# arkworks-rs/ripp

Hardware: AMD Instinct MI355X
Metric: SIPP prover pairing-products/sec at n=2^20 BLS12-381 (higher is better)
Workload: dtype u32

## Files before the change

### include/ripp_hip.h

```cpp
#ifndef RIPP_HIP_H
#define RIPP_HIP_H
#include <stddef.h>
#include <stdint.h>
#ifdef __cplusplus
extern "C" {
#endif

typedef struct { uint64_t l[6]; } ripp_fp;
typedef struct { uint64_t l[4]; } ripp_fr;
typedef struct { ripp_fp c0, c1; } ripp_fp2;
typedef struct { ripp_fp2 c[6]; } ripp_gt;
typedef struct { ripp_fp x, y; } ripp_g1a;
typedef struct { ripp_fp x, y, z; } ripp_g1j;
typedef struct { ripp_fp2 x, y; } ripp_g2a;
typedef struct { ripp_fp2 x, y, z; } ripp_g2j;

enum { RIPP_OK = 0, RIPP_ERR_LENGTH = 1, RIPP_ERR_POW2 = 2, RIPP_ERR_DEVICE = 3, RIPP_ERR_ARG = 4 };

typedef struct {
    double total_ms, upload_ms, scale_ms, miller_lines_ms, miller_products_ms, fold_ms, normalize_ms, host_ms, hash_ms;
    double kernel_miller_lines_ms_sum, kernel_line_products_ms_sum;
    uint64_t kernel_miller_lines_launches, kernel_line_products_launches;
    uint64_t pairs_lines, pairs_products;
    double exchange_ms;
    double look_ms;
    uint64_t look_items, look_pairs;
    double statement_hash_ms, statement_hash_wait_ms;
    uint64_t chains_lines;
    uint64_t mem_tier, device_bytes;
} ripp_stats;
#define RIPP_ABI_VERSION 7
int32_t ripp_abi_version(void);
size_t  ripp_stats_size(void);

int32_t ripp_init(int32_t device_ordinal);
void    ripp_shutdown(void);
int32_t ripp_device_count(void);
int32_t ripp_release_scratch(void);
size_t  ripp_device_bytes(void);
const char* ripp_last_error(void);

typedef struct {
    uint32_t struct_size;
    uint32_t no_vm, no_precompute, no_fold_tables, no_msm_glv, lp_one_lane, no_endo, no_fq, no_xscale, scale_no_fq, agg_sequential, look_static, quiet_waits, no_share, no_fuse, fuse_tables;
    int32_t  look_eighths;
    int32_t  ranks_per_device;
    int32_t  msm_c; uint32_t msm_ch, msm_gmin;
    uint32_t no_prebuild;
    uint64_t vm_lines_max, vm_fold_max, vm_tree_max, gls_split_max, msm_vm_merge_max, fold_tab_min, fq_min, lp_fq_min, vm_joint_max, vm_scale_max,
             tail_pipe_max, ml_fq_min, fq_min_g1,
             msm_lds_sort_min,
             msm_chunk_min;
    uint64_t mem_cap_bytes;
    uint32_t hot_workers;
    uint32_t no_job_cache;
    uint32_t no_lp_karatsuba;
    uint32_t comm_timeout_ms;
    uint32_t plan_derate_pct;
    uint32_t n_devices;
} ripp_config;
int32_t ripp_config_default(ripp_config* cfg);
int32_t ripp_configure(const ripp_config* cfg);
int32_t ripp_config_get(ripp_config* cfg);

int32_t ripp_pairing_product_j(const ripp_g1j* left, size_t n_left, const ripp_g2j* right, size_t n_right, ripp_gt* out);
int32_t ripp_pairing_product_a(const ripp_g1a* a, const ripp_g2a* b, size_t n, ripp_gt* out);
int32_t ripp_pairing_product_coeffs_a(const ripp_g1a* a, const ripp_g2a* b, const ripp_fr* r, size_t n, ripp_gt* out);
int32_t ripp_msm_g1_j(const ripp_g1j* bases, size_t n_left, const ripp_fr* scalars, size_t n_right, ripp_g1j* out);
int32_t ripp_msm_g2_j(const ripp_g2j* bases, size_t n_left, const ripp_fr* scalars, size_t n_right, ripp_g2j* out);
int32_t ripp_msm_g1_a(const ripp_g1a* bases, const ripp_fr* scalars, size_t n, ripp_g1j* out);
int32_t ripp_msm_g2_a(const ripp_g2a* bases, const ripp_fr* scalars, size_t n, ripp_g2j* out);
int32_t ripp_device_slots_used(void);
int32_t ripp_scalar_inner_product(const ripp_fr* left, size_t nl, const ripp_fr* right, size_t nr, ripp_fr* out);
int32_t ripp_pairing_miller_j(const ripp_g1j* left, size_t nl, const ripp_g2j* right, size_t nr, ripp_gt* miller_value);
int32_t ripp_sum_g1_j(const ripp_g1j* pts, size_t n, ripp_g1j* out);
int32_t ripp_sum_g2_j(const ripp_g2j* pts, size_t n, ripp_g2j* out);

int32_t ripp_fold_g1_a(const ripp_g1a* hi, const ripp_g1a* lo, size_t half, const ripp_fr* s, ripp_g1a* out);
int32_t ripp_fold_g2_a(const ripp_g2a* hi, const ripp_g2a* lo, size_t half, const ripp_fr* s, ripp_g2a* out);
int32_t ripp_fold_g1_j(const ripp_g1j* hi, const ripp_g1j* lo, size_t half, const ripp_fr* s, ripp_g1j* out);
int32_t ripp_fold_g2_j(const ripp_g2j* hi, const ripp_g2j* lo, size_t half, const ripp_fr* s, ripp_g2j* out);
int32_t ripp_fold_fr(const ripp_fr* hi, const ripp_fr* lo, size_t half, const ripp_fr* s, ripp_fr* out);
int32_t ripp_scale_g1_a(const ripp_g1a* a, const ripp_fr* r, size_t n, ripp_g1a* out);
int32_t ripp_normalize_g1(const ripp_g1j* in, size_t n, ripp_g1a* out);
int32_t ripp_normalize_g2(const ripp_g2j* in, size_t n, ripp_g2a* out);

typedef struct ripp_vec ripp_vec;
enum { RIPP_VEC_G1 = 1, RIPP_VEC_G2 = 2, RIPP_VEC_FR = 3 };
int32_t ripp_vec_upload_g1a(const ripp_g1a* p, size_t n, ripp_vec** out);
int32_t ripp_vec_upload_g2a(const ripp_g2a* p, size_t n, ripp_vec** out);
int32_t ripp_vec_upload_g1j(const ripp_g1j* p, size_t n, ripp_vec** out);
int32_t ripp_vec_upload_g2j(const ripp_g2j* p, size_t n, ripp_vec** out);
int32_t ripp_vec_upload_fr(const ripp_fr* p, size_t n, ripp_vec** out);
size_t  ripp_vec_len(const ripp_vec* v);
int32_t ripp_vec_kind(const ripp_vec* v);
int32_t ripp_vec_slice(const ripp_vec* v, size_t off, size_t len, ripp_vec** view);
int32_t ripp_vec_halves(const ripp_vec* v, ripp_vec** lo, ripp_vec** hi);
int32_t ripp_vec_download(const ripp_vec* v, void* out);
void    ripp_vec_free(ripp_vec* v);
int32_t ripp_vec_pairing_product(const ripp_vec* left_g1, const ripp_vec* right_g2, ripp_gt* out);
int32_t ripp_vec_msm(const ripp_vec* bases, const ripp_vec* scalars, void* out );
int32_t ripp_vec_scalar_inner_product(const ripp_vec* left, const ripp_vec* right, ripp_fr* out);
int32_t ripp_vec_fold(const ripp_vec* hi, const ripp_vec* lo, const ripp_fr* s, ripp_vec** out);

int32_t ripp_sipp_prove(const ripp_g1a* a, const ripp_g2a* b, const ripp_fr* r, size_t n, const ripp_gt* value,
                        ripp_gt* proof, ripp_fr* challenges, ripp_stats* stats);
int32_t ripp_sipp_verify(const ripp_g1a* a, const ripp_g2a* b, const ripp_fr* r, size_t n, const ripp_gt* claimed,
                         const ripp_gt* proof, size_t proof_rounds, int32_t* accept);

typedef struct ripp_sipp_job ripp_sipp_job;
int32_t ripp_sipp_job_create(const ripp_g1a* a, const ripp_g2a* b, const ripp_fr* r, size_t n_local,
                             int32_t rank, int32_t world, ripp_sipp_job** job);
void    ripp_sipp_job_destroy(ripp_sipp_job* job);
int32_t ripp_sipp_job_prove(ripp_sipp_job* job, const ripp_gt* value, ripp_gt* proof, ripp_fr* challenges, ripp_stats* stats);
int32_t ripp_sipp_job_begin(ripp_sipp_job* job);
size_t  ripp_sipp_job_rounds_left(const ripp_sipp_job* job);
int32_t ripp_sipp_job_round_partials(ripp_sipp_job* job, ripp_gt* partials );
int32_t ripp_sipp_job_round_finish(ripp_sipp_job* job, const ripp_gt* combined , const uint8_t seed_digest[32],
                                   ripp_gt* z_l, ripp_gt* z_r, ripp_fr* x);
int32_t ripp_sipp_job_stats(const ripp_sipp_job* job, ripp_stats* stats);
size_t  ripp_sipp_job_local_len(const ripp_sipp_job* job);
int32_t ripp_sipp_job_export(ripp_sipp_job* job, ripp_g1a* a_out, ripp_g2a* b_out);
// ... 189 lines not shown
```

### ripp_amd/csrc/engine.hip

```cpp
#include <hip/hip_runtime.h>
#include <atomic>
#include <csignal>
#include <sched.h>
#include <condition_variable>
#include <deque>
#include <functional>
#include <memory>
#include <future>
#include <chrono>
#include <cmath>
#include <cstdio>
#include <cstring>
#include <cstdlib>
#include <mutex>
#include <string>
#include <thread>
#include <vector>
#ifndef RIPP_BUILD_STAMP
#define RIPP_BUILD_STAMP __DATE__ " " __TIME__
#endif
#include "../../include/ripp_hip.h"
#include "kernels.hpp"
#include "line_products.hpp"
#include "msm.hpp"
// ... 129 lines not shown
struct Engine;
thread_local Engine* t_engine = nullptr;
size_t evict_idle_scratch(Engine* e);
struct DevBuf {
    void* p = nullptr; size_t cap = 0; uint64_t epoch = 0;
    int32_t reserve(size_t bytes) {
        epoch = g_call_epoch.load(std::memory_order_relaxed);
        if (bytes <= cap) return RIPP_OK;
        release();
        hipError_t err = hipMalloc(&p, bytes);
        if (err == hipErrorOutOfMemory && t_engine) {
            (void)hipGetLastError();
            const size_t freed = evict_idle_scratch(t_engine);
            if (trace_on()) fprintf(stderr, "[ripp] out of device memory for %zu bytes: %zu bytes of idle scratch freed, retrying\n", bytes, freed);
            err = freed ? hipMalloc(&p, bytes) : err;
        }
        if (err != hipSuccess) { p = nullptr; (void)hipGetLastError(); set_err(std::string("hipMalloc(&p, bytes): ") + hipGetErrorString(err) + " (" + std::to_string(bytes) + " bytes wanted, " + std::to_string(g_dev_bytes.load()) + " held by the library)"); return RIPP_ERR_DEVICE; }
        cap = bytes; g_dev_bytes.fetch_add(bytes, std::memory_order_relaxed); return RIPP_OK;
    }
    void release() { if (p) { (void)hipFree(p); g_dev_bytes.fetch_sub(cap, std::memory_order_relaxed); } p = nullptr; cap = 0; }
    template <class T> T* as() { return reinterpret_cast<T*>(p); }
};

struct PinBuf {
    void* p = nullptr; size_t cap = 0; hipEvent_t ev = nullptr; bool pending = false;
    bool blocking = false;
    bool ev_blocking = false;
    int32_t wait() { if (pending) { HIPCHK(hipEventSynchronize(ev)); pending = false; } return RIPP_OK; }
    int32_t reserve(size_t bytes) {
        int32_t rc = wait(); if (rc) return rc;
        if (ev && ev_blocking != blocking) { (void)hipEventDestroy(ev); ev = nullptr; }
        if (!ev) { HIPCHK(hipEventCreateWithFlags(&ev, hipEventDisableTiming | (blocking ? hipEventBlockingSync : 0))); ev_blocking = blocking; }
        if (bytes <= cap) return RIPP_OK;
        if (p) { (void)hipHostFree(p); p = nullptr; cap = 0; }
        HIPCHK(hipHostMalloc(&p, bytes, hipHostMallocDefault)); cap = bytes; return RIPP_OK;
    }
    int32_t send(void* dst, size_t bytes, hipStream_t st) {
        HIPCHK(hipMemcpyAsync(dst, p, bytes, hipMemcpyHostToDevice, st)); HIPCHK(hipEventRecord(ev, st)); pending = true; return RIPP_OK;
    }
    void release() { if (pending && ev) (void)hipEventSynchronize(ev); pending = false; if (p) (void)hipHostFree(p); p = nullptr; cap = 0; if (ev) (void)hipEventDestroy(ev); ev = nullptr; }
    template <class T> T* as() { return reinterpret_cast<T*>(p); }
};

struct MsmScratch {
    DevBuf digits, hist, offs, cursor, slotoffs, spw, sorted, slots, buckets, seg, seg2, win, out;
    DevBuf ext;
    DevBuf flags;
    DevBuf nflag;
    void* host_out = nullptr;
    void release() { for (DevBuf* b : {&digits, &hist, &offs, &cursor, &slotoffs, &spw, &sorted, &slots, &buckets, &seg, &seg2, &win, &out, &ext, &flags, &nflag}) b->release(); if (host_out) (void)hipHostFree(host_out); host_out = nullptr; }
};

struct Timer {
    hipEvent_t a{}, b{};
    int32_t init() { HIPCHK(hipEventCreate(&a)); HIPCHK(hipEventCreate(&b)); return RIPP_OK; }
    void destroy() { if (a) (void)hipEventDestroy(a); if (b) (void)hipEventDestroy(b); a = b = nullptr; }
};

struct Engine {
    int device = -1;
    hipStream_t stream = nullptr, stream2 = nullptr;
    hipEvent_t ev_fork = nullptr, ev_join = nullptr, ev_join3 = nullptr;
    hipEvent_t ev_t0 = nullptr, ev_t1 = nullptr;
    int n_simd = 1024;
    DevBuf lines, partA, partB, jacG1, jacG2, tmpA, tmpB, tmpR, affG1, affG2;
    DevBuf qtab;
    MsmScratch msm_scratch[2];
    MsmScratch msm_batch; DevBuf pc_coef, pc_out, pc_yev, pc_h, pc_cin, pc_q, pc_aff;
    DevBuf tpc_m, tpc_m2, tpc_b, tpc_b2, tpc_k, tpc_k2, tpc_jac, tpc_part, tpc_out;
    uint32_t msm_batch_chunks = 0;
    void pc_release() { msm_batch.release(); for (DevBuf* b : {&pc_coef, &pc_out, &pc_yev, &pc_h, &pc_cin, &pc_q, &pc_aff, &tpc_m, &tpc_m2, &tpc_b, &tpc_b2, &tpc_k, &tpc_k2, &tpc_jac, &tpc_part, &tpc_out}) b->release(); }
    DevBuf kzg_q[2];
    PinBuf stage[4];
    DevBuf kzg_bases[2];
    hipStream_t stream3 = nullptr;
    hipStream_t stream4 = nullptr;
    hipEvent_t ev_join4 = nullptr;
    DevBuf fold_tab1, fold_mult, fold_tab, fold_jac1, fold_jac2;
    DevBuf fix_flags, scale_flags;
    const void* tab_owner = nullptr;
    struct JobBufCache { DevBuf d[15]; PinBuf p[4]; bool full = false; void release() { for (DevBuf& b : d) b.release(); for (PinBuf& b : p) b.release(); full = false; } } job_cache;
    size_t msm_chunk_min = (size_t)1 << 20;
    size_t msm_lds_sort_min = 0;
    const void* g2tab_hi = nullptr; size_t g2tab_half = 0;
    size_t vm_scale_max = (size_t)1 << 14;
    size_t vm_joint_max = (size_t)1 << 13;
    size_t lp_fq_min = 0;
    size_t ml_fq_min = 0;
    size_t fq_min_g1 = (size_t)1 << 12;
    size_t fq_min = (size_t)1 << 15;
    size_t fold_tab_min = 32768;
    size_t msm_vm_merge_max = 16384;
    hipStream_t stream5 = nullptr;
    hipEvent_t ev_join5 = nullptr;
    Fp12* pinned_rows = nullptr;
    size_t pinned_rows_cap = 0;
    std::vector<std::pair<hipEvent_t, hipEvent_t>> ev_lines, ev_prod;
    std::vector<std::pair<hipEvent_t, hipEvent_t>> ev_fold_async;
    size_t tail_pipe_max = (size_t)1 << 11;
    size_t vm_tree_max = (size_t)1 << 16;
    size_t vm_fold_max = (size_t)1 << 11;
    DevBuf vm_flag;
    size_t vm_lines_max = (size_t)1 << 15;
    size_t gls_split_max = (size_t)1 << 14;
    size_t max_pairs_per_batch = (size_t)1 << 19;
    size_t mem_cap = 0;
    int mem_tier = 0;
    bool mem_fits(size_t need, size_t held) const {
        if (need <= held) return true;
        const size_t extra = need - held;
        if (mem_cap) return g_dev_bytes.load(std::memory_order_relaxed) + extra <= mem_cap;
        size_t fr = 0, tot = 0;
        if (hipMemGetInfo(&fr, &tot) != hipSuccess) return true;
        return extra + std::max<size_t>((size_t)2 << 30, tot / 50) <= fr;
    }
    size_t pairs_cap(size_t want) {
        want = std::max<size_t>(1, std::min(want, max_pairs_per_batch));
        const size_t per = (size_t)N_LINES * LINE_CHUNKS * sizeof(uint4);
        auto bytes = [per](size_t pairs) { return ((pairs + 63) & ~(size_t)63) * per + (size_t)MAX_PRODUCTS * 64 * per; };
        if (bytes(want) <= lines.cap) return want;
        size_t w = want;
        while (w > 4096 && !mem_fits(bytes(w), lines.cap)) w = (w + 1) / 2;
        if (w < want) mem_tier |= 8;
        return w;
    }
    ripp_stats stats{};
    std::vector<Engine*> peers; bool virtual_devices = false;
    Engine* aux = nullptr;
    Engine* aux_engine() {
        if (!aux) { Engine* a = new Engine(); if (a->init(device) != RIPP_OK) { delete a; return nullptr; } aux = a; }
        aux->refresh_switches(); aux->stats = ripp_stats{};
        return aux;
    }
    struct Switches { bool no_vm = false, no_precompute = false, no_fold_tables = false, no_msm_glv = false, lp_one_lane = false, no_endo = false, no_fq = false, no_xscale = false, no_share = false, no_fuse = false, no_prebuild = false, fuse_tables = false, no_job_cache = false, no_lp_kara = false, no_msm_batch = false; } sw;
    struct Sizes { size_t vm_lines_max, vm_fold_max, vm_tree_max, gls_split_max, msm_vm_merge_max, fold_tab_min, fq_min, lp_fq_min, vm_joint_max, vm_scale_max, tail_pipe_max, ml_fq_min, fq_min_g1, msm_lds_sort_min, msm_chunk_min; } defaults{};
    MsmTune msm_tune;
    static constexpr size_t TPC_CROSS_MIN = ~(size_t)0;
    size_t tpc_cross_min = TPC_CROSS_MIN;
    double cal_ms_per_pair = 0, cal_hash_bytes_per_ms = 0;
    int look_eighths = -1; double ranks_per_device = 1.0; bool look_static = false, quiet_waits_cfg = false, agg_sequential = false, scale_no_fq = false;
    int hot_workers_cfg = 0;
    uint32_t comm_timeout_ms = 0, plan_derate_pct = 0, n_devices_cfg = 0;
    void refresh_switches() {
        msm_tune = MsmTune();
        vm_lines_max = defaults.vm_lines_max; vm_fold_max = defaults.vm_fold_max; vm_tree_max = defaults.vm_tree_max; gls_split_max = defaults.gls_split_max;
        msm_vm_merge_max = defaults.msm_vm_merge_max; fold_tab_min = defaults.fold_tab_min; fq_min = defaults.fq_min; lp_fq_min = defaults.lp_fq_min; vm_joint_max = defaults.vm_joint_max;
        vm_scale_max = defaults.vm_scale_max; tail_pipe_max = defaults.tail_pipe_max; ml_fq_min = defaults.ml_fq_min; fq_min_g1 = defaults.fq_min_g1; msm_lds_sort_min = defaults.msm_lds_sort_min; msm_chunk_min = defaults.msm_chunk_min;
        sw = Switches(); look_eighths = -1; ranks_per_device = 1.0; look_static = quiet_waits_cfg = agg_sequential = scale_no_fq = false; mem_cap = 0; hot_workers_cfg = 0; comm_timeout_ms = plan_derate_pct = n_devices_cfg = 0;
        if (g_cfg_set) {
            const ripp_config& c = g_cfg;
            sw.no_vm = c.no_vm; sw.no_precompute = c.no_precompute; sw.no_fold_tables = c.no_fold_tables; sw.no_msm_glv = c.no_msm_glv; sw.lp_one_lane = c.lp_one_lane;
            sw.no_endo = c.no_endo; sw.no_fq = c.no_fq; sw.no_xscale = c.no_xscale; sw.no_share = c.no_share; sw.no_fuse = c.no_fuse; sw.fuse_tables = c.fuse_tables; scale_no_fq = c.scale_no_fq; agg_sequential = c.agg_sequential; look_static = c.look_static; quiet_waits_cfg = c.quiet_waits;
            look_eighths = c.look_eighths; ranks_per_device = c.ranks_per_device > 1 ? (double)c.ranks_per_device : 1.0;
            msm_tune.c = c.msm_c; msm_tune.ch = c.msm_ch; msm_tune.gmin = c.msm_gmin; sw.no_prebuild = c.no_prebuild;
            mem_cap = (size_t)c.mem_cap_bytes; hot_workers_cfg = (int)c.hot_workers; sw.no_job_cache = c.no_job_cache != 0;
            sw.no_lp_kara = c.no_lp_karatsuba != 0; comm_timeout_ms = c.comm_timeout_ms; plan_derate_pct = c.plan_derate_pct; n_devices_cfg = c.n_devices;
            vm_lines_max = c.vm_lines_max; vm_fold_max = c.vm_fold_max; vm_tree_max = c.vm_tree_max; gls_split_max = c.gls_split_max; msm_vm_merge_max = c.msm_vm_merge_max; fold_tab_min = c.fold_tab_min;
            fq_min = c.fq_min; lp_fq_min = c.lp_fq_min; vm_joint_max = c.vm_joint_max; vm_scale_max = c.vm_scale_max; tail_pipe_max = c.tail_pipe_max; ml_fq_min = c.ml_fq_min; fq_min_g1 = c.fq_min_g1; msm_lds_sort_min = c.msm_lds_sort_min; msm_chunk_min = c.msm_chunk_min;
        }
        { const char* s; if ((s = std::getenv("RIPP_MSM_C"))) msm_tune.c = std::atoi(s); if ((s = std::getenv("RIPP_MSM_CH"))) msm_tune.ch = (uint32_t)std::strtoul(s, nullptr, 10); if ((s = std::getenv("RIPP_MSM_GMIN"))) msm_tune.gmin = (uint32_t)std::strtoul(s, nullptr, 10); }
        auto env_sz = [](const char* k, size_t& v) { if (const char* s = std::getenv(k)) v = (size_t)std::strtoull(s, nullptr, 10); };
        env_sz("RIPP_VM_LINES_MAX", vm_lines_max); env_sz("RIPP_VM_FOLD_MAX", vm_fold_max); env_sz("RIPP_VM_TREE_MAX", vm_tree_max);
        env_sz("RIPP_GLS_SPLIT_MAX", gls_split_max); env_sz("RIPP_MSM_VM_MERGE_MAX", msm_vm_merge_max); env_sz("RIPP_FOLD_TAB_MIN", fold_tab_min);
        env_sz("RIPP_FQ_MIN", fq_min); env_sz("RIPP_LP_FQ_MIN", lp_fq_min); env_sz("RIPP_VM_JOINT_MAX", vm_joint_max);
        env_sz("RIPP_MSM_LDS_SORT_MIN", msm_lds_sort_min); env_sz("RIPP_MSM_CHUNK_MIN", msm_chunk_min);
        env_sz("RIPP_VM_SCALE_MAX", vm_scale_max); env_sz("RIPP_TAIL_PIPE_MAX", tail_pipe_max); env_sz("RIPP_ML_FQ_MIN", ml_fq_min); env_sz("RIPP_FQ_MIN_G1", fq_min_g1);
        auto env_on = [](const char* k, bool& v) { if (std::getenv(k)) v = true; };
        env_on("RIPP_NO_VM", sw.no_vm); env_on("RIPP_NO_PRECOMPUTE", sw.no_precompute); env_on("RIPP_NO_FOLD_TABLES", sw.no_fold_tables); env_on("RIPP_NO_MSM_GLV", sw.no_msm_glv);
        env_on("RIPP_LP_ONE_LANE", sw.lp_one_lane);
        env_on("RIPP_NO_ENDO", sw.no_endo);
        env_on("RIPP_NO_XSCALE", sw.no_xscale);
        env_on("RIPP_NO_LP_KARA", sw.no_lp_kara);
        env_on("RIPP_NO_FQ", sw.no_fq);
        env_on("RIPP_FUSE_TABLES", sw.fuse_tables);
        env_on("RIPP_NO_JOB_CACHE", sw.no_job_cache);
        env_sz("RIPP_MEM_CAP_BYTES", mem_cap);
        if (const char* s = std::getenv("RIPP_HOT_WORKERS")) hot_workers_cfg = std::atoi(s) ? 1 : 2;
        { auto env_u32 = [](const char* k, uint32_t& v) { if (const char* s = std::getenv(k)) v = (uint32_t)std::strtoul(s, nullptr, 10); };
          env_u32("RIPP_COMM_TIMEOUT_MS", comm_timeout_ms); env_u32("RIPP_PLAN_DERATE_PCT", plan_derate_pct); env_u32("RIPP_N_DEVICES", n_devices_cfg);
          virtual_devices = false; if (const char* s = std::getenv("RIPP_VIRTUAL_DEVICES")) { n_devices_cfg = (uint32_t)std::strtoul(s, nullptr, 10); virtual_devices = true; } }
        tpc_cross_min = TPC_CROSS_MIN; env_sz("RIPP_TPC_CROSS_MIN", tpc_cross_min);
        env_on("RIPP_NO_MSM_BATCH", sw.no_msm_batch);
        env_on("RIPP_NO_PREBUILD", sw.no_prebuild);
        env_on("RIPP_NO_FUSE", sw.no_fuse);
        env_on("RIPP_NO_SHARE", sw.no_share);
        env_on("RIPP_SCALE_NO_FQ", scale_no_fq); env_on("RIPP_AGG_SEQUENTIAL", agg_sequential); env_on("RIPP_LOOK_STATIC", look_static); env_on("RIPP_QUIET_WAITS", quiet_waits_cfg);
        if (const char* s = std::getenv("RIPP_LOOK_ITEMS")) look_eighths = 8 * std::max(0, std::atoi(s));
        if (const char* s = std::getenv("RIPP_LOOK_EIGHTHS")) look_eighths = std::max(0, std::atoi(s));
        if (const char* s = std::getenv("RIPP_RANKS_PER_DEVICE")) ranks_per_device = std::max(1.0, std::atof(s));
#if !defined(RIPP_AB_KERNELS) || defined(RIPP_BLS12_377)
        sw.lp_one_lane = false;
#endif
    }

    int32_t init(int dev) {
        int n = 0;
        if (hipGetDeviceCount(&n) != hipSuccess || n <= 0) { set_err("no HIP device available (libripp_hip has no CPU fallback)"); return RIPP_ERR_DEVICE; }
        if (dev < 0 || dev >= n) { set_err("device ordinal out of range"); return RIPP_ERR_ARG; }
        HIPCHK(hipSetDevice(dev));
        HIPCHK(hipStreamCreateWithFlags(&stream, hipStreamNonBlocking));
        HIPCHK(hipStreamCreateWithFlags(&stream2, hipStreamNonBlocking));
        HIPCHK(hipStreamCreateWithFlags(&stream3, hipStreamNonBlocking));
        HIPCHK(hipStreamCreateWithFlags(&stream4, hipStreamNonBlocking)); HIPCHK(hipEventCreateWithFlags(&ev_join4, hipEventDisableTiming));
        HIPCHK(hipStreamCreateWithFlags(&stream5, hipStreamNonBlocking)); HIPCHK(hipEventCreateWithFlags(&ev_join5, hipEventDisableTiming));
        HIPCHK(hipEventCreateWithFlags(&ev_fork, hipEventDisableTiming)); HIPCHK(hipEventCreateWithFlags(&ev_join, hipEventDisableTiming)); HIPCHK(hipEventCreateWithFlags(&ev_join3, hipEventDisableTiming));
        HIPCHK(hipEventCreate(&ev_t0)); HIPCHK(hipEventCreate(&ev_t1));
        { hipDeviceProp_t pr; if (hipGetDeviceProperties(&pr, dev) == hipSuccess) n_simd = pr.multiProcessorCount * 4; }
        defaults = Sizes{vm_lines_max, vm_fold_max, vm_tree_max, gls_split_max, msm_vm_merge_max, fold_tab_min, fq_min, lp_fq_min, vm_joint_max, vm_scale_max, tail_pipe_max, ml_fq_min, fq_min_g1, msm_lds_sort_min, msm_chunk_min};
        refresh_switches();
        device = dev;
        return RIPP_OK;
    }
    void destroy() {
        if (aux) { aux->destroy(); delete aux; aux = nullptr; }
        for (Engine* p : peers) { (void)hipSetDevice(p->device); p->destroy(); delete p; }
        if (!peers.empty()) { peers.clear(); (void)hipSetDevice(device); }
        for (DevBuf* b : {&lines, &partA, &partB, &jacG1, &jacG2, &tmpA, &tmpB, &tmpR, &affG1, &affG2, &qtab, &vm_flag, &scale_tab, &fold_tab1, &fold_mult, &fold_tab, &fold_jac1, &fold_jac2, &fix_flags, &scale_flags}) b->release();
        msm_scratch[0].release(); msm_scratch[1].release(); kzg_q[0].release(); kzg_q[1].release(); kzg_bases[0].release(); kzg_bases[1].release(); job_cache.release(); pc_release();
        if (stream3) (void)hipStreamDestroy(stream3);
        if (stream4) (void)hipStreamDestroy(stream4); if (ev_join4) (void)hipEventDestroy(ev_join4);
        if (stream5) (void)hipStreamDestroy(stream5); if (ev_join5) (void)hipEventDestroy(ev_join5);
        if (pinned_rows) (void)hipHostFree(pinned_rows);
        for (PinBuf& b : stage) b.release();
        for (auto& e : ev_lines) { (void)hipEventDestroy(e.first); (void)hipEventDestroy(e.second); }
        for (auto& e : ev_prod) { (void)hipEventDestroy(e.first); (void)hipEventDestroy(e.second); }
        for (auto& e : ev_fold_async) { (void)hipEventDestroy(e.first); (void)hipEventDestroy(e.second); }
        if (stream) (void)hipStreamDestroy(stream);
        if (stream2) (void)hipStreamDestroy(stream2);
        if (ev_fork) (void)hipEventDestroy(ev_fork); if (ev_join) (void)hipEventDestroy(ev_join); if (ev_join3) (void)hipEventDestroy(ev_join3);
        if (ev_t0) (void)hipEventDestroy(ev_t0); if (ev_t1) (void)hipEventDestroy(ev_t1);
        if (ev_quiet) (void)hipEventDestroy(ev_quiet);
    }
    int32_t ensure_pinned_rows(size_t rows) {
        if (rows <= pinned_rows_cap) return RIPP_OK;
        if (pinned_rows) (void)hipHostFree(pinned_rows);
        HIPCHK(hipHostMalloc((void**)&pinned_rows, rows * sizeof(Fp12), hipHostMallocDefault));
        pinned_rows_cap = rows; return RIPP_OK;
    }
    bool quiet_waits = false; hipEvent_t ev_quiet = nullptr;
    int32_t sync() {
        if (quiet_waits) {
            if (!ev_quiet) HIPCHK(hipEventCreateWithFlags(&ev_quiet, hipEventDisableTiming | hipEventBlockingSync));
            HIPCHK(hipEventRecord(ev_quiet, stream)); HIPCHK(hipEventSynchronize(ev_quiet)); return RIPP_OK;
        }
        HIPCHK(hipStreamSynchronize(stream)); return RIPP_OK;
    }

    int32_t mark(std::vector<std::pair<hipEvent_t, hipEvent_t>>& v, bool begin) {
        if (begin) { hipEvent_t a, b; HIPCHK(hipEventCreate(&a)); HIPCHK(hipEventCreate(&b)); v.emplace_back(a, b); HIPCHK(hipEventRecord(a, stream)); }
        else HIPCHK(hipEventRecord(v.back().second, stream));
        return RIPP_OK;
    }
    void collect_kernel_stats() {
        auto drain = [](std::vector<std::pair<hipEvent_t, hipEvent_t>>& v, double& sum, uint64_t& cnt) {
            for (auto& e : v) { float ms = 0; if (hipEventElapsedTime(&ms, e.first, e.second) == hipSuccess) { sum += ms; ++cnt; } (void)hipEventDestroy(e.first); (void)hipEventDestroy(e.second); }
            v.clear(); };
        drain(ev_lines, stats.kernel_miller_lines_ms_sum, stats.kernel_miller_lines_launches);
        drain(ev_prod, stats.kernel_line_products_ms_sum, stats.kernel_line_products_launches);
        uint64_t nf = 0; drain(ev_fold_async, stats.fold_ms, nf);
    }

    DevBuf scale_tab;
    int32_t scale_g1_dev(const G1A* base, uint32_t base_stride, const Fr* k, size_t n, G1J* out, hipStream_t st = nullptr) {
        if (n == 0) return RIPP_OK;
        if (!st) st = stream;
        if (sw.no_endo) {
            hipLaunchKernelGGL(HIP_KERNEL_NAME(k_scale_pts<Fp>), dim3(nblk(n, 256)), dim3(256), 0, st, base, base_stride, k, (uint32_t)n, out);
            HIPCHK(hipGetLastError());
            return RIPP_OK;
        }
        if (n <= vm_scale_max && !sw.no_vm) {
            hipLaunchKernelGGL(k_vm_scale_g1, dim3(nblk(n, 4 * VM_EPW)), dim3(256), 4 * VM_EPW * VM_SCALE_SLOTS * sizeof(VmSlot), st, base, base_stride, k, (uint32_t)n, out);
            HIPCHK(hipGetLastError());
            return RIPP_OK;
        }
        int32_t rc = scale_tab.reserve((size_t)SCALE_TAB * G1J_CHUNKS * n * sizeof(uint4)); if (rc) return rc;
        if (!sw.no_fq && !scale_no_fq)
        {
            if ((rc = scale_flags.reserve(n + 16))) return rc;
            hipLaunchKernelGGL(k_scale_g1_glv_q, dim3(nblk(n, 256)), dim3(256), 0, st, base, base_stride, k, (uint32_t)n, scale_tab.as<uint4>(), out, scale_flags.as<uint8_t>());
            hipLaunchKernelGGL(k_scale_g1_fix, dim3(FIX_GRID), dim3(64), 0, st, base, base_stride, k, (uint32_t)n, out, scale_flags.as<uint8_t>());
        }
        else
        hipLaunchKernelGGL(k_scale_g1_glv, dim3(nblk(n, 256)), dim3(256), 0, st, base, base_stride, k, (uint32_t)n, scale_tab.as<uint4>(), out);
        HIPCHK(hipGetLastError());
        return RIPP_OK;
    }

    template <class F> int32_t normalize_dev(const Jac<F>* in, size_t n, Affine<F>* out, hipStream_t st = nullptr) {
        if (n == 0) return RIPP_OK;
        if (!st) st = stream;
        uint32_t K = (uint32_t)std::min<size_t>(16, std::max<size_t>(1, n / 65536));
        uint32_t T = (uint32_t)((n + K - 1) / K);
        hipLaunchKernelGGL(HIP_KERNEL_NAME(k_normalize<F>), dim3(nblk(T, 256)), dim3(256), 0, st, in, (uint32_t)n, out, T);
        HIPCHK(hipGetLastError());
        return RIPP_OK;
    }


    template <class F> int32_t msm_launch(MsmScratch& ms, hipStream_t st, const Affine<F>* bases, const Fr* scalars, size_t n, const std::function<int32_t()>* bases_arrive = nullptr) {
        if (!ms.host_out) HIPCHK(hipHostMalloc(&ms.host_out, sizeof(G2J), hipHostMallocDefault));
        if (n == 0) { *reinterpret_cast<Jac<F>*>(ms.host_out) = jac_inf<F>(); return bases_arrive ? (*bases_arrive)() : RIPP_OK; }
        const bool no_glv = sw.no_msm_glv;
        const size_t nreal = n;
        const MsmPlan p = msm_plan(nreal, no_glv ? 1 : std::is_same<F, Fp>::value ? 2 : 4, msm_tune);
        n = p.n;
        const size_t nwb = (size_t)p.nwin * p.nb;
        const uint32_t max_slots = (uint32_t)(n / p.ch + std::min<size_t>(p.nb, n) + 1);
        uint32_t nseg = (p.nb + p.seg - 1) / p.seg;
        int32_t rc;
        if ((rc = ms.digits.reserve((size_t)p.nwin * n * sizeof(uint16_t))) || (rc = ms.hist.reserve(nwb * 4)) || (rc = ms.offs.reserve(nwb * 4)) ||
            (rc = ms.cursor.reserve(nwb * 4)) || (rc = ms.slotoffs.reserve(nwb * 4)) || (rc = ms.spw.reserve(p.nwin * 4)) ||
            (rc = ms.sorted.reserve((size_t)p.nwin * n * 4)) || (rc = ms.slots.reserve((size_t)p.nwin * max_slots * sizeof(Jac<F>))) ||
// ... 195 lines not shown
        const uint4* lrows = lines.as<uint4>() + (size_t)p_lo * N_LINES * LINE_CHUNKS * stride;
#if !defined(RIPP_BLS12_377)
        const bool lp_kara = !sw.no_fq && !sw.no_lp_kara && !sw.lp_one_lane && m * (size_t)np2 >= lp_fq_min;
#else
        const bool lp_kara = false;
#endif
        const uint32_t per_wave = sw.lp_one_lane ? 64 : lp_kara ? LK_GROUPS_PER_WAVE : LP_GROUPS_PER_WAVE;
        uint32_t T = (uint32_t)std::max<size_t>(per_wave, ((size_t)n_simd * RIPP_OCC_PROD / nrows) * per_wave);
        if (T > m) T = (uint32_t)m;
        if ((rc = partA.reserve(nrows * FP12_CHUNKS * (size_t)T * sizeof(uint4))) != RIPP_OK) return rc;
        if ((rc = partB.reserve(nrows * FP12_CHUNKS * (size_t)((T + 1) / 2) * sizeof(uint4))) != RIPP_OK) return rc;
        if ((rc = mark(ev_prod, true)) != RIPP_OK) return rc;
#if defined(RIPP_AB_KERNELS) && !defined(RIPP_BLS12_377)
        if (sw.lp_one_lane)
            hipLaunchKernelGGL(k_line_products1, dim3(nblk(T, 64), (unsigned)nrows), dim3(64), 0, stream, lrows, stride, (uint32_t)m, partA.as<uint4>(), T);
        else
#endif
#if !defined(RIPP_BLS12_377)
        if (lp_kara)
            hipLaunchKernelGGL(k_line_products_k, dim3(nblk(T, LK_GROUPS_PER_WAVE), (unsigned)nrows), dim3(64), 0, stream, lrows, stride, (uint32_t)m, partA.as<uint4>(), T);
        else
#endif
        if (!sw.no_fq && m * (size_t)np2 >= lp_fq_min)
            hipLaunchKernelGGL(k_line_products_q, dim3(nblk(T, LP_GROUPS_PER_WAVE), (unsigned)nrows), dim3(64), 0, stream, lrows, stride, (uint32_t)m, partA.as<uint4>(), T);
        else
            hipLaunchKernelGGL(k_line_products, dim3(nblk(T, LP_GROUPS_PER_WAVE), (unsigned)nrows), dim3(64), 0, stream, lrows, stride, (uint32_t)m, partA.as<uint4>(), T);
        HIPCHK(hipGetLastError());
        if ((rc = mark(ev_prod, false)) != RIPP_OK) return rc;
        stats.pairs_products += m * (size_t)np2;
        uint4* cur = partA.as<uint4>(); uint4* nxt = partB.as<uint4>();
        while (T > 1) {
            const int R = ((size_t)T * nrows > (size_t)n_simd * 64) ? 4 : 2;
            const uint32_t Tout = (T + R - 1) / R;
            if (R == 2 && (size_t)Tout * nrows <= vm_tree_max && !sw.no_vm)
                hipLaunchKernelGGL(k_vm_fp12_tree, dim3(nblk(Tout, 2 * VM_EPW), (unsigned)nrows), dim3(128), 2 * VM_EPW * VM_F12_SLOTS * sizeof(VmSlot), stream, cur, T, nxt, Tout);
            else
            hipLaunchKernelGGL(k_fp12_tree, dim3(nblk(Tout, 64), (unsigned)nrows), dim3(64), 0, stream, cur, T, nxt, Tout, R);
            HIPCHK(hipGetLastError());
            std::swap(cur, nxt); T = Tout;
        }
        HIPCHK(hipMemcpyAsync(dst_pinned + (size_t)p_lo * N_LINES, cur, nrows * sizeof(Fp12), hipMemcpyDeviceToHost, stream));
        return RIPP_OK;
    }
    int32_t step_products(const G1A* const* a, const G2A* const* b, int nprod, size_t M, Fp12* rows_out) {
        const size_t nrows = (size_t)nprod * N_LINES;
        for (size_t r = 0; r < nrows; ++r) rows_out[r] = Fp12::one();
        if (M == 0) return RIPP_OK;
        int32_t rc;
        if ((rc = ensure_pinned_rows(nrows)) != RIPP_OK) return rc;
        if (nprod > MAX_PRODUCTS) return RIPP_ERR_ARG;
        const size_t batch = std::min(M, std::max<size_t>(1, pairs_cap(std::min(max_pairs_per_batch, M * (size_t)nprod)) / nprod));
        for (size_t off = 0; off < M; off += batch) {
            const size_t m = std::min(batch, M - off);
            if ((rc = enqueue_products(a, b, nprod, off, m, pinned_rows)) != RIPP_OK) return rc;
            if ((rc = sync()) != RIPP_OK) return rc;
            for (size_t r = 0; r < nrows; ++r) rows_out[r] = (off == 0) ? pinned_rows[r] : mul(rows_out[r], pinned_rows[r]);
        }
        return RIPP_OK;
    }
};

int32_t get_engine(Engine** out) {
    if (!g_engine) {
        Engine* e = new Engine();
        int32_t rc = e->init(0);
        if (rc != RIPP_OK) { delete e; return rc; }
        g_engine = e;
    }
    if (hipSetDevice(g_engine->device) != hipSuccess) { set_err("hipSetDevice failed"); return RIPP_ERR_DEVICE; }
    g_engine->refresh_switches();
    g_call_epoch.fetch_add(1, std::memory_order_relaxed); t_engine = g_engine;
    *out = g_engine; return RIPP_OK;
}

bool trace_on() { static const bool on = std::getenv("RIPP_TRACE") != nullptr; return on; }
size_t evict_idle_scratch(Engine* e) {
    const uint64_t now = g_call_epoch.load(std::memory_order_relaxed);
    (void)hipDeviceSynchronize();
    const size_t before = g_dev_bytes.load();
    bool tables = false;
    for (DevBuf* b : {&e->lines, &e->partA, &e->partB, &e->qtab, &e->scale_tab, &e->jacG1, &e->jacG2, &e->affG1, &e->affG2, &e->tmpA, &e->tmpB, &e->tmpR}) if (b->p && b->epoch != now) b->release();
    for (DevBuf* b : {&e->fold_tab1, &e->fold_mult, &e->fold_tab, &e->fold_jac1, &e->fold_jac2}) if (b->p && b->epoch != now) { b->release(); tables = true; }
    if (tables) { e->tab_owner = nullptr; e->g2tab_hi = nullptr; }
    for (int k = 0; k < 2; ++k) {
        MsmScratch& ms = e->msm_scratch[k];
        for (DevBuf* b : {&ms.digits, &ms.hist, &ms.offs, &ms.cursor, &ms.slotoffs, &ms.spw, &ms.sorted, &ms.slots, &ms.buckets, &ms.seg, &ms.seg2, &ms.win, &ms.ext, &ms.flags}) if (b->p && b->epoch != now) b->release();
        for (DevBuf* b : {&e->kzg_q[k], &e->kzg_bases[k]}) if (b->p && b->epoch != now) b->release();
    }
    if (e->job_cache.full) e->job_cache.release();
    const size_t after = g_dev_bytes.load();
    return before > after ? before - after : 0;
}

ScalarBits scalar_bits(const Fr& s_mont) {
    const Fr c = from_mont(s_mont);
    ScalarBits sb; int top = -1;
    for (int i = 0; i < 8; ++i) { sb.w[i] = c.l[i]; }
    for (int i = 255; i >= 0; --i) if ((c.l[i >> 5] >> (i & 31)) & 1u) { top = i; break; }
    sb.nbits = top + 1; return sb;
}

int naf_recode(const uint32_t* words, int nwords, int8_t* digits, int maxd) {
    uint32_t w[10] = {0};
    for (int i = 0; i < nwords; ++i) w[i] = words[i];
    auto is_zero = [&]() { for (int i = 0; i <= nwords; ++i) if (w[i]) return false; return true; };
    int n = 0;
    while (!is_zero() && n < maxd) {
        int8_t d = 0;
        if (w[0] & 1u) {
            d = (int8_t)(2 - (int)(w[0] & 3u));
            if (d > 0) { w[0] &= ~1u; }
            else { for (int i = 0; i <= nwords; ++i) { if (++w[i] != 0) break; } }
        }
        digits[n++] = d;
        for (int i = 0; i < nwords; ++i) w[i] = (w[i] >> 1) | (w[i + 1] << 31);
        w[nwords] >>= 1;
    }
    return n;
}
NafDigits naf_digits(const Fr& s_mont) {
    const Fr c = from_mont(s_mont);
    NafDigits nd; std::memset(&nd, 0, sizeof nd);
    nd.len = naf_recode(c.l, 8, nd.d, 258);
    return nd;
}
GlsDigits gls_digits(const Fr& s_mont) {
    const Fr c = from_mont(s_mont);
    uint64_t v[4] = {(uint64_t)c.l[0] | ((uint64_t)c.l[1] << 32), (uint64_t)c.l[2] | ((uint64_t)c.l[3] << 32),
                     (uint64_t)c.l[4] | ((uint64_t)c.l[5] << 32), (uint64_t)c.l[6] | ((uint64_t)c.l[7] << 32)};
    GlsDigits g; std::memset(&g, 0, sizeof g);
    int maxlen = 0;
    for (int j = 0; j < 4; ++j) {
        unsigned __int128 rem = 0;
        for (int i = 3; i >= 0; --i) { const unsigned __int128 cur = (rem << 64) | v[i]; v[i] = (uint64_t)(cur / BLS_X_ABS); rem = cur % BLS_X_ABS; }
        const uint64_t dj = (uint64_t)rem;
        const uint32_t words[2] = {(uint32_t)dj, (uint32_t)(dj >> 32)};
        const int len = naf_recode(words, 2, g.d[j], 66);
        if (len > maxlen) maxlen = len;
    }
    g.len = maxlen;
    return g;
}

void glv_split(const Fr& s_mont, uint32_t rem[9], uint32_t quo[8]) {
    const Fr c = from_mont(s_mont);
    const uint32_t lam[8] = RIPP_GLV_LAMBDA;
    for (int i = 0; i < 9; ++i) rem[i] = 0; for (int i = 0; i < 8; ++i) quo[i] = 0;
    for (int bit = 255; bit >= 0; --bit) {
        for (int i = 8; i > 0; --i) rem[i] = (rem[i] << 1) | (rem[i - 1] >> 31);
        rem[0] = (rem[0] << 1) | ((c.l[bit >> 5] >> (bit & 31)) & 1u);
        bool ge = rem[8] != 0;
        if (!ge) { ge = true; for (int i = 7; i >= 0; --i) { if (rem[i] != lam[i]) { ge = rem[i] > lam[i]; break; } } }
        if (ge) { uint32_t borrow = 0; for (int i = 0; i < 8; ++i) rem[i] = subb32(rem[i], lam[i], borrow); rem[8] -= borrow; quo[bit >> 5] |= 1u << (bit & 31); }
    }
}
GlvDigits glv_digits(const Fr& s_mont) {
    uint32_t rem[9], quo[8]; glv_split(s_mont, rem, quo);
    GlvDigits g; std::memset(&g, 0, sizeof g);
    const int l1 = naf_recode(rem, 5, g.d1, 131), l2 = naf_recode(quo, 5, g.d2, 131);
    g.len = l1 > l2 ? l1 : l2;
    return g;
}

int wnaf4_recode(uint64_t v, int8_t* digits, int maxd, int W = RIPP_FOLD_W) {
    unsigned __int128 k = v; int len = 0;
    while (k != 0 && len < maxd) {
        int d = 0;
        if ((uint64_t)k & 1u) { d = (int)((uint64_t)k & ((1u << W) - 1)); if (d >= (1 << (W - 1))) d -= 1 << W; if (d >= 0) k -= (unsigned)d; else k += (unsigned)(-d); }
        digits[len++] = (int8_t)d;
        k >>= 1;
    }
    return len;
}
Wnaf4 split32_wnaf(const Fr& s_mont, int W = RIPP_FOLD_W) {
    const Fr c = from_mont(s_mont);
    Wnaf4 g; std::memset(&g, 0, sizeof g);
    for (int t = 0; t < 4; ++t) g.len = std::max(g.len, wnaf4_recode(c.l[t], g.d[t], 35, W));
    return g;
}
int tab_width(int M) { int w = 2; while ((1 << (w - 2)) < M) ++w; return w; }
void glv_split(const Fr& s_mont, uint32_t rem[9], uint32_t quo[8]);
WnafG1x4 fused_digits_g1(const Fr& x0, const Fr& x1, int W) {
    WnafG1x4 g; std::memset(&g, 0, sizeof g);
    const Fr c0 = from_mont(x0), c1 = from_mont(x1);
    uint32_t rem[9], quo[8]; glv_split(mul(x0, x1), rem, quo);
    const uint32_t* src[4] = {c0.l, rem, quo, c1.l};
    for (int u = 0; u < 4; ++u) for (int b = 0; b < 4; ++b) g.len = std::max(g.len, wnaf4_recode(src[u][b], g.d[4 * u + b], 35, W));
    return g;
}
GlvDigits split64_digits(const Fr& s_mont) {
    const Fr c = from_mont(s_mont);
    GlvDigits g; std::memset(&g, 0, sizeof g);
    const int l1 = naf_recode(&c.l[0], 2, g.d1, 131), l2 = naf_recode(&c.l[2], 2, g.d2, 131);
    g.len = l1 > l2 ? l1 : l2;
    return g;
}
bool fits_128(const Fr& s_mont) { const Fr c = from_mont(s_mont); return (c.l[4] | c.l[5] | c.l[6] | c.l[7]) == 0; }
Gls8Digits gls8_digits(const Fr& s_mont) {
    const Fr c = from_mont(s_mont);
    uint64_t v[4] = {(uint64_t)c.l[0] | ((uint64_t)c.l[1] << 32), (uint64_t)c.l[2] | ((uint64_t)c.l[3] << 32),
                     (uint64_t)c.l[4] | ((uint64_t)c.l[5] << 32), (uint64_t)c.l[6] | ((uint64_t)c.l[7] << 32)};
    Gls8Digits g; std::memset(&g, 0, sizeof g);
    int maxlen = 0;
    for (int j = 0; j < 4; ++j) {
        unsigned __int128 rem = 0;
        for (int i = 3; i >= 0; --i) { const unsigned __int128 cur = (rem << 64) | v[i]; v[i] = (uint64_t)(cur / BLS_X_ABS); rem = cur % BLS_X_ABS; }
        const uint64_t dj = (uint64_t)rem;
        const uint32_t lo = (uint32_t)dj, hi = (uint32_t)(dj >> 32);
        const int l1 = naf_recode(&lo, 1, g.d[j], 35), l2 = naf_recode(&hi, 1, g.d[4 + j], 35);
        maxlen = std::max(maxlen, std::max(l1, l2));
    }
    g.len = maxlen;
    return g;
}

Wnaf16 gls16_wnaf(const Fr& s_mont, int W = RIPP_FOLD_W) {
    const Fr c = from_mont(s_mont);
    uint64_t v[4] = {(uint64_t)c.l[0] | ((uint64_t)c.l[1] << 32), (uint64_t)c.l[2] | ((uint64_t)c.l[3] << 32),
                     (uint64_t)c.l[4] | ((uint64_t)c.l[5] << 32), (uint64_t)c.l[6] | ((uint64_t)c.l[7] << 32)};
    Wnaf16 g; std::memset(&g, 0, sizeof g);
    for (int j = 0; j < 4; ++j) {
        unsigned __int128 rem = 0;
        for (int i = 3; i >= 0; --i) { const unsigned __int128 cur = (rem << 64) | v[i]; v[i] = (uint64_t)(cur / BLS_X_ABS); rem = cur % BLS_X_ABS; }
        const uint64_t dj = (uint64_t)rem;
        for (int b = 0; b < 4; ++b) g.len = std::max(g.len, wnaf4_recode((dj >> (16 * b)) & 0xffffu, g.d[4 * b + j], 19, W));
    }
    return g;
}
Wnaf16x3 fused_digits_g2(const Fr& x0, const Fr& x1, int W) {
    Wnaf16x3 g; g.s[0] = gls16_wnaf(mul(x0, x1), W); g.s[1] = gls16_wnaf(x0, W); g.s[2] = gls16_wnaf(x1, W);
    g.len = std::max(g.s[0].len, std::max(g.s[1].len, g.s[2].len));
    return g;
}

GlsDigits gls_wnaf(const Fr& s_mont, int W) {
    const Fr c = from_mont(s_mont);
    uint64_t v[4] = {(uint64_t)c.l[0] | ((uint64_t)c.l[1] << 32), (uint64_t)c.l[2] | ((uint64_t)c.l[3] << 32),
                     (uint64_t)c.l[4] | ((uint64_t)c.l[5] << 32), (uint64_t)c.l[6] | ((uint64_t)c.l[7] << 32)};
    GlsDigits g; std::memset(&g, 0, sizeof g);
    for (int j = 0; j < 4; ++j) {
        unsigned __int128 rem = 0;
        for (int i = 3; i >= 0; --i) { const unsigned __int128 cur = (rem << 64) | v[i]; v[i] = (uint64_t)(cur / BLS_X_ABS); rem = cur % BLS_X_ABS; }
        g.len = std::max(g.len, wnaf4_recode((uint64_t)rem, g.d[j], 66, W));
    }
    return g;
}

SplitDigits split_digits_g1(const Fr& s_mont) {
    const GlvDigits g = split64_digits(s_mont);
    SplitDigits d; std::memset(&d, 0, sizeof d);
    for (int i = 0; i < g.len && i < 68; ++i) { d.d[0][i] = g.d1[i]; d.d[1][i] = g.d2[i]; }
    d.len = g.len; return d;
}
SplitDigits split_digits_g2(const Fr& s_mont) {
    const Gls8Digits g = gls8_digits(s_mont);
    SplitDigits d; std::memset(&d, 0, sizeof d);
    for (int t = 0; t < 8; ++t) for (int i = 0; i < g.len; ++i) d.d[t][i] = g.d[t][i];
    d.len = g.len; return d;
}

SplitDigits split_digits_g1_glv(const Fr& s_mont) {
    uint32_t rem[9], quo[8]; glv_split(s_mont, rem, quo);
    SplitDigits d; std::memset(&d, 0, sizeof d);
    const int l0 = naf_recode(&rem[0], 2, d.d[0], 67), l1 = naf_recode(&quo[0], 2, d.d[1], 67), l2 = naf_recode(&rem[2], 2, d.d[2], 67), l3 = naf_recode(&quo[2], 2, d.d[3], 67);
    d.len = std::max(std::max(l0, l1), std::max(l2, l3)); return d;
}

template <class T> int32_t upload(Engine* e, DevBuf& buf, const void* host, size_t n, T** dev) {
    int32_t rc = buf.reserve(std::max<size_t>(n, 1) * sizeof(T)); if (rc != RIPP_OK) return rc;
    if (n) HIPCHK(hipMemcpyAsync(buf.p, host, n * sizeof(T), hipMemcpyHostToDevice, e->stream));
    *dev = buf.as<T>(); return RIPP_OK;
}


double g_digest_hash_ms = 0, g_digest_wait_ms = 0;
void statement_digest(const G1A* a, const G2A* b, const Fr* r, size_t n, const Fp12& value, uint8_t digest[32], std::atomic<uint64_t>* progress = nullptr) {
    fs::Blake2s h;
    g_digest_hash_ms = g_digest_wait_ms = 0;
    const uint64_t len = (uint64_t)n;
    constexpr size_t BLK = 1 << 13; constexpr int RING = 6;
    const size_t item[3] = {96, 192, 32};
    struct Seg { int kind; size_t s, e; };
    std::vector<Seg> segs;
    for (int kind = 0; kind < 3; ++kind) for (size_t s0 = 0; s0 < n; s0 += BLK) segs.push_back({kind, s0, std::min(n, s0 + BLK)});
    struct Ring { std::vector<uint8_t> b[RING]; };
    static std::mutex pool_mu; static std::vector<std::unique_ptr<Ring>> pool;
    std::unique_ptr<Ring> ring;
    { std::lock_guard<std::mutex> lk(pool_mu); if (!pool.empty()) { ring = std::move(pool.back()); pool.pop_back(); } }
    if (!ring) { ring.reset(new Ring()); for (auto& v : ring->b) v.resize(BLK * 192); }
    struct Return { std::unique_ptr<Ring>& r; std::mutex& m; std::vector<std::unique_ptr<Ring>>& p; ~Return() { std::lock_guard<std::mutex> lk(m); p.emplace_back(std::move(r)); } } give_back{ring, pool_mu, pool};
    std::vector<uint8_t>* const buf = ring->b;
    std::vector<std::future<void>> fut(segs.size());
    auto launch = [&](size_t j) {
        const Seg sg = segs[j]; uint8_t* out = buf[j % RING].data();
        fut[j] = host_pool().submit([a, b, r, sg, out]() {
            for (size_t i = sg.s; i < sg.e; ++i) {
                if (sg.kind == 0) fs::ser_g1(a[i], out + (i - sg.s) * 96);
                else if (sg.kind == 1) fs::ser_g2(b[i], out + (i - sg.s) * 192);
                else fs::ser_fr(r[i], out + (i - sg.s) * 32);
            } });
    };
    for (size_t j = 0; j < segs.size() && j < (size_t)RING - 1; ++j) launch(j);
    int cur_kind = -1;
    for (size_t j = 0; j < segs.size(); ++j) {
        if (segs[j].kind != cur_kind) {
            for (int k = cur_kind + 1; k <= segs[j].kind; ++k) h.update(reinterpret_cast<const uint8_t*>(&len), 8);
            cur_kind = segs[j].kind;
        }
        const double t0 = now_ms();
        fut[j].get();
        const double t1 = now_ms();
        h.update(buf[j % RING].data(), (segs[j].e - segs[j].s) * item[segs[j].kind]);
        if (progress) progress->fetch_add((segs[j].e - segs[j].s) * item[segs[j].kind], std::memory_order_relaxed);
        g_digest_wait_ms += t1 - t0; g_digest_hash_ms += now_ms() - t1;
        if (j + RING - 1 < segs.size()) launch(j + RING - 1);
    }
    for (int k = cur_kind + 1; k < 3; ++k) h.update(reinterpret_cast<const uint8_t*>(&len), 8);
    uint8_t gt[576]; fs::ser_gt(value, gt); h.update(gt, 576);
    h.finish(digest);
}

}

struct ripp_sipp_job {
    size_t n_local = 0, len = 0;
    int rank = 0, world = 1, world0 = 1;
    DevBuf a0, b0, r0;
    DevBuf a, b, a_next, b_next, jac1, jac2;
    size_t tab2_stride = 0; bool tab_ready = false;
    size_t tab_cnt = 0; int tab_M = FOLD_TAB_M; bool tab_fused = false;
    Fr bs = Fr::one(); bool bs_on = false; bool tab_on_lo = false; bool xs_enabled = false;
    DevBuf a_pow, b_pow; bool pre_ready = false;
    struct LookItem {
        int R = 0, side = 0, level = 0;
        size_t npairs = 0, q = 0;
        std::vector<Fp12> Z;
        std::vector<std::future<Fp12>> fe, pend;
    };
    std::vector<LookItem> look; PinBuf look_rows[2];
    double look_deadline = 0;
    std::atomic<uint64_t> hash_done{0}; uint64_t hash_total = 0; double hash_t0 = 0;
    bool no_window = false;
    size_t hash_n = 0;
    DevBuf a_pow_h, b_pow_h, parts1, parts2; bool pre_vm_ready = false, pre_vm_side = false;
    PinBuf tp_rows[2]; size_t tp_round[2] = {~(size_t)0, ~(size_t)0};
    std::vector<G1A> ha; std::vector<G2A> hb; std::vector<Fr> hr;
    const G1A* ha_ext = nullptr; const G2A* hb_ext = nullptr; const Fr* hr_ext = nullptr;
    bool hash_prestarted = false;
    fs::FiatShamirRng rng; bool seeded = false;
    std::thread hash_thread; uint8_t digest[32]; std::atomic<bool> digest_ready{false};
    double t_begin = 0;
};

namespace {

int32_t job_begin(Engine* e, ripp_sipp_job* j) {
    const size_t n = j->n_local;
    int32_t rc;
    if ((rc = j->a.reserve(n * sizeof(G1A))) != RIPP_OK) return rc;
    if ((rc = j->b.reserve(n * sizeof(G2A))) != RIPP_OK) return rc;
    if ((rc = j->a_next.reserve(std::max<size_t>(n / 2, 1) * sizeof(G1A))) != RIPP_OK) return rc;
    if ((rc = j->b_next.reserve(std::max<size_t>(n / 2, 1) * sizeof(G2A))) != RIPP_OK) return rc;
    if ((rc = j->jac1.reserve(n * sizeof(G1J))) != RIPP_OK) return rc;
    if ((rc = j->jac2.reserve(std::max<size_t>(n / 2, 1) * sizeof(G2J))) != RIPP_OK) return rc;
    e->stats = ripp_stats{};
    j->t_begin = now_ms();
    hipEvent_t t0 = e->ev_t0, t1 = e->ev_t1;
    HIPCHK(hipEventRecord(t0, e->stream));
    if ((rc = e->scale_g1_dev(j->a0.as<G1A>(), 1u, j->r0.as<Fr>(), n, j->jac1.as<G1J>())) != RIPP_OK) return rc;
    if ((rc = e->normalize_dev<Fp>(j->jac1.as<G1J>(), n, j->a.as<G1A>())) != RIPP_OK) return rc;
    HIPCHK(hipMemcpyAsync(j->b.p, j->b0.p, n * sizeof(G2A), hipMemcpyDeviceToDevice, e->stream));
    HIPCHK(hipEventRecord(t1, e->stream));
    if ((rc = e->sync()) != RIPP_OK) return rc;
    float ms = 0; (void)hipEventElapsedTime(&ms, t0, t1); e->stats.scale_ms += ms;
    j->len = n; j->seeded = false; j->world = j->world0;
    j->bs = Fr::one(); j->bs_on = false;
    j->pre_vm_ready = false; j->pre_vm_side = false; j->pre_ready = false; j->look.clear(); j->tp_round[0] = j->tp_round[1] = ~(size_t)0;
    return RIPP_OK;
}

int32_t job_round_partials(Engine* e, ripp_sipp_job* j, Fp12* rows ) {
    const size_t half = j->len / 2;
    const G1A* a = j->a.as<G1A>(); const G2A* b = j->b.as<G2A>();
    const G1A* as[2] = {a + half, a};
    const G2A* bs[2] = {b, b + half};
    const double t0 = now_ms();
    int32_t rc = e->step_products(as, bs, 2, half, rows);
    e->stats.miller_products_ms += now_ms() - t0;
    return rc;
}

bool fold_g2_table_pays(const Engine* e, size_t half) { return half >= e->fold_tab_min && half > e->gls_split_max && !e->sw.no_fold_tables; }
bool fold_g2_table_fits(const Engine* e, size_t half) {
    const size_t need = half * (5 * 4 * sizeof(G2A) + 3 * sizeof(G2J)) + 65536, held = e->fold_mult.cap + e->fold_tab.cap + e->fold_jac2.cap;
    return need <= held || e->mem_fits(need, held);
}
bool xscale_round(const Engine* e, const ripp_sipp_job* j, size_t half) {
    if (!j->xs_enabled || e->sw.no_endo || e->sw.no_xscale) return false;
    if (fold_g2_table_pays(e, half)) return true;
    return j->bs_on && half <= e->gls_split_max && 2 * half > e->vm_joint_max && half > e->vm_fold_max;
}
int32_t job_precompute_vm(Engine* e, ripp_sipp_job* j, bool side = false) {
    const size_t half = j->len / 2;
    if (half == 0 || half > e->vm_fold_max || e->sw.no_vm || e->sw.no_precompute) return RIPP_OK;
    int32_t rc;
    if ((rc = j->a_pow_h.reserve(half * sizeof(G1J))) || (rc = j->b_pow_h.reserve(half * sizeof(G2J))) || (rc = j->parts1.reserve(2 * half * sizeof(G1J))) || (rc = j->parts2.reserve(8 * half * sizeof(G2J)))) return rc;
    hipLaunchKernelGGL(HIP_KERNEL_NAME(k_vm_pow2<Fp>), dim3(nblk(half, 4 * VM_EPW)), dim3(256), 4 * VM_EPW * VmCurve<Fp>::SLOTS * sizeof(VmSlot), e->stream2, j->a.as<G1A>() + half, (uint32_t)half, 64, j->a_pow_h.as<G1J>());
    hipStream_t s2 = e->stream;
    if (side) { HIPCHK(hipStreamWaitEvent(e->stream3, e->ev_t1, 0)); s2 = e->stream3; }
    hipLaunchKernelGGL(HIP_KERNEL_NAME(k_vm_pow2<Fp2>), dim3(nblk(half, 4 * VM_EPW)), dim3(256), 4 * VM_EPW * VmCurve<Fp2>::SLOTS * sizeof(VmSlot), s2, j->b.as<G2A>() + half, (uint32_t)half, 32, j->b_pow_h.as<G2J>());
    HIPCHK(hipGetLastError());
    if (side) HIPCHK(hipEventRecord(e->ev_join3, e->stream3));
    j->pre_vm_side = side;
    j->pre_vm_ready = true;
    return RIPP_OK;
}

int32_t job_precompute_round0(Engine* e, ripp_sipp_job* j, bool fuse = false) {
    const size_t half = j->len / 2, q = j->len / 4;
    if (half < ((size_t)1 << 16) || j->digest_ready.load() || j->no_window || e->sw.no_precompute) return RIPP_OK;
    int32_t rc;
    bool tables = !e->sw.no_fold_tables;
    j->tab_ready = false; j->tab_fused = false;
    auto tab_bytes = [](size_t M, size_t cnt) { return cnt * (4 * M * (sizeof(G1A) + sizeof(G2A)) + 16 * M * sizeof(G2A) + (M - 1) * (sizeof(G1J) + sizeof(G2J)) + 4) + 65536; };
    const size_t tab_held = e->fold_tab1.cap + e->fold_mult.cap + e->fold_tab.cap + e->fold_jac1.cap + e->fold_jac2.cap + e->fix_flags.cap;
    size_t M_half = FOLD_TAB_M;
    if (tables) {
        const bool want_fuse = fuse && xscale_round(e, j, half) && !e->sw.no_fq && !e->sw.no_fuse && q >= e->fq_min;
        if (want_fuse && !e->mem_fits(tab_bytes(4, 3 * q), tab_held)) { fuse = false; e->mem_tier = std::max(e->mem_tier & 7, 1) | (e->mem_tier & 8); }
        if (!(want_fuse && fuse)) {
            if (!e->mem_fits(tab_bytes(M_half, half), tab_held)) { M_half = 4; e->mem_tier = std::max(e->mem_tier & 7, 1) | (e->mem_tier & 8); }
            if (!e->mem_fits(tab_bytes(M_half, half), tab_held)) { tables = false; e->mem_tier = std::max(e->mem_tier & 7, 2) | (e->mem_tier & 8); }
        }
        if (!tables) e->sw.no_fold_tables = true;
    }
    if (!tables && !e->mem_fits(half * (sizeof(G1A) + sizeof(G2A) + sizeof(G1J) + sizeof(G2J)), j->a_pow.cap + j->b_pow.cap + j->jac1.cap + j->jac2.cap)) {
        e->mem_tier = 3 | (e->mem_tier & 8);
        if (trace_on()) fprintf(stderr, "[ripp] round-0 precomputation skipped: the device is short of memory\n");
        return RIPP_OK;
    }
    if (trace_on() && (e->mem_tier & 7)) fprintf(stderr, "[ripp] round-0 tables: memory tier %d (%s)\n", e->mem_tier & 7, tables ? "half-vector tables" : "pre-doubled bases only");
    if ((rc = j->a_pow.reserve(half * sizeof(G1A))) || (rc = j->b_pow.reserve(half * sizeof(G2A))) || (rc = j->jac1.reserve(half * sizeof(G1J))) || (rc = j->jac2.reserve(half * sizeof(G2J)))) return rc;
    if (!tables) {
        if (!e->sw.no_fq) hipLaunchKernelGGL(k_pow2_mul_g1_q, dim3(nblk(half, 256)), dim3(256), 0, e->stream, j->a.as<G1A>() + half, (uint32_t)half, 64, j->jac1.as<G1J>());
        else hipLaunchKernelGGL(HIP_KERNEL_NAME(k_pow2_mul<Fp>), dim3(nblk(half, 256)), dim3(256), 0, e->stream, j->a.as<G1A>() + half, (uint32_t)half, 64, j->jac1.as<G1J>());
        HIPCHK(hipGetLastError());
        if ((rc = e->normalize_dev<Fp>(j->jac1.as<G1J>(), half, j->a_pow.as<G1A>()))) return rc;
        if (!e->sw.no_fq) hipLaunchKernelGGL(k_pow2_mul_g2_q, dim3(nblk(half, 64)), dim3(64), 0, e->stream, j->b.as<G2A>() + half, (uint32_t)half, 32, j->jac2.as<G2J>());
        else hipLaunchKernelGGL(HIP_KERNEL_NAME(k_pow2_mul<Fp2>), dim3(nblk(half, 256)), dim3(256), 0, e->stream, j->b.as<G2A>() + half, (uint32_t)half, 32, j->jac2.as<G2J>());
        HIPCHK(hipGetLastError());
        if ((rc = e->normalize_dev<Fp2>(j->jac2.as<G2J>(), half, j->b_pow.as<G2A>()))) return rc;
        j->pre_ready = true;
        return RIPP_OK;
    }
    j->tab_on_lo = xscale_round(e, j, half);
    fuse = fuse && j->tab_on_lo && !e->sw.no_fq && !e->sw.no_fuse && q >= e->fq_min;
    const size_t M = fuse ? 4 : M_half;
    const size_t cnt = fuse ? 3 * q : half;
    const size_t qstride = (cnt + 63) & ~(size_t)63;
    const size_t njt = (M - 1) * cnt;
    if ((rc = e->fold_tab1.reserve(4 * M * cnt * sizeof(G1A))) || (rc = e->fold_mult.reserve(4 * M * cnt * sizeof(G2A))) || (rc = e->fold_tab.reserve(16 * M * G2A_CHUNKS * qstride * sizeof(uint4))) ||
        (rc = e->fold_jac1.reserve(njt * sizeof(G1J))) || (rc = e->fold_jac2.reserve(njt * sizeof(G2J))) || (rc = e->fix_flags.reserve(4 * cnt + 16))) return rc;
    e->tab_owner = j;
    G1A* t1 = e->fold_tab1.as<G1A>(); G2A* t2 = e->fold_mult.as<G2A>();
    G1J* sj1 = e->fold_jac1.as<G1J>(); G2J* sj2 = e->fold_jac2.as<G2J>();
    HIPCHK(hipMemcpyAsync(t1, j->a.as<G1A>() + (fuse ? q : half), cnt * sizeof(G1A), hipMemcpyDeviceToDevice, e->stream));
    HIPCHK(hipMemcpyAsync(t2, j->b.as<G2A>() + (j->tab_on_lo ? 0 : half), cnt * sizeof(G2A), hipMemcpyDeviceToDevice, e->stream));
    for (int b = 0; b < 4; ++b) {
        G1A* base1 = t1 + M * b * cnt; G2A* base2 = t2 + M * b * cnt;
        if (b > 0) {
            if (!e->sw.no_fq) hipLaunchKernelGGL(k_pow2_mul_g1_q, dim3(nblk(cnt, 256)), dim3(256), 0, e->stream, base1 - M * cnt, (uint32_t)cnt, 32, sj1);
            else hipLaunchKernelGGL(HIP_KERNEL_NAME(k_pow2_mul<Fp>), dim3(nblk(cnt, 256)), dim3(256), 0, e->stream, base1 - M * cnt, (uint32_t)cnt, 32, sj1);
            HIPCHK(hipGetLastError());
            if ((rc = e->normalize_dev<Fp>(sj1, cnt, base1))) return rc;
            if (!e->sw.no_fq) hipLaunchKernelGGL(k_pow2_mul_g2_q, dim3(nblk(cnt, 64)), dim3(64), 0, e->stream, base2 - M * cnt, (uint32_t)cnt, 16, sj2);
            else hipLaunchKernelGGL(HIP_KERNEL_NAME(k_pow2_mul<Fp2>), dim3(nblk(cnt, 256)), dim3(256), 0, e->stream, base2 - M * cnt, (uint32_t)cnt, 16, sj2);
            HIPCHK(hipGetLastError());
            if ((rc = e->normalize_dev<Fp2>(sj2, cnt, base2))) return rc;
        }
        hipLaunchKernelGGL(HIP_KERNEL_NAME(k_odd_multiples<Fp>), dim3(nblk(cnt, 64)), dim3(64), 0, e->stream, base1, (uint32_t)cnt, (int)M, sj1);
        HIPCHK(hipGetLastError());
        if ((rc = e->normalize_dev<Fp>(sj1, njt, base1 + cnt))) return rc;
        if (!e->sw.no_fq) {
            hipLaunchKernelGGL(k_odd_multiples_q, dim3(nblk(cnt, 64)), dim3(64), 0, e->stream, base2, (uint32_t)cnt, (int)M, sj2, e->fix_flags.as<uint8_t>());
#if !defined(RIPP_INLINE_FALLBACK)
            hipLaunchKernelGGL(k_odd_multiples_fix, dim3(FIX_GRID), dim3(64), 0, e->stream, base2, (uint32_t)cnt, (int)M, sj2, e->fix_flags.as<uint8_t>());
#endif
        }
        else hipLaunchKernelGGL(HIP_KERNEL_NAME(k_odd_multiples<Fp2>), dim3(nblk(cnt, 64)), dim3(64), 0, e->stream, base2, (uint32_t)cnt, (int)M, sj2);
        HIPCHK(hipGetLastError());
        if ((rc = e->normalize_dev<Fp2>(sj2, njt, base2 + cnt))) return rc;
    }
    hipLaunchKernelGGL(k_g2_tab_images, dim3(nblk(cnt, 64), 4 * M), dim3(64), 0, e->stream, e->fold_mult.as<G2A>(), (uint32_t)cnt, (int)M, e->fold_tab.as<uint4>(), qstride);
    HIPCHK(hipGetLastError());
    j->tab2_stride = qstride; j->tab_cnt = cnt; j->tab_M = (int)M; j->tab_fused = fuse; j->tab_ready = true;
    return RIPP_OK;
}

int32_t fold_g2_table_build(Engine* e, hipStream_t st, const G2A* hi, size_t half) {
    constexpr int M = 4;
    const size_t qstride = (half + 63) & ~(size_t)63;
    int32_t rc;
    e->g2tab_hi = nullptr;
    if ((rc = e->fold_mult.reserve((size_t)M * half * sizeof(G2A))) || (rc = e->fold_tab.reserve((size_t)4 * M * G2A_CHUNKS * qstride * sizeof(uint4))) ||
        (rc = e->fold_jac2.reserve((size_t)(M - 1) * half * sizeof(G2J))) || (rc = e->fix_flags.reserve(4 * half + 16))) return rc;
    e->tab_owner = nullptr;
    G2A* mult = e->fold_mult.as<G2A>();
    HIPCHK(hipMemcpyAsync(mult, hi, half * sizeof(G2A), hipMemcpyDeviceToDevice, st));
    if (!e->sw.no_fq) {
        hipLaunchKernelGGL(k_odd_multiples_q, dim3(nblk(half, 64)), dim3(64), 0, st, hi, (uint32_t)half, M, e->fold_jac2.as<G2J>(), e->fix_flags.as<uint8_t>());
#if !defined(RIPP_INLINE_FALLBACK)
        hipLaunchKernelGGL(k_odd_multiples_fix, dim3(FIX_GRID), dim3(64), 0, st, hi, (uint32_t)half, M, e->fold_jac2.as<G2J>(), e->fix_flags.as<uint8_t>());
#endif
    }
    else hipLaunchKernelGGL(HIP_KERNEL_NAME(k_odd_multiples<Fp2>), dim3(nblk(half, 64)), dim3(64), 0, st, hi, (uint32_t)half, M, e->fold_jac2.as<G2J>());
    HIPCHK(hipGetLastError());
    if ((rc = e->normalize_dev<Fp2>(e->fold_jac2.as<G2J>(), (size_t)(M - 1) * half, mult + half, st)) != RIPP_OK) return rc;
    hipLaunchKernelGGL(k_g2_tab_images, dim3(nblk(half, 64), M), dim3(64), 0, st, mult, (uint32_t)half, M, e->fold_tab.as<uint4>(), qstride);
    HIPCHK(hipGetLastError());
    e->g2tab_hi = hi; e->g2tab_half = half;
    return RIPP_OK;
}
int32_t fold_g2_table(Engine* e, hipStream_t st, const G2A* hi, const G2A* lo, size_t half, const Fr& s, DevBuf& jac) {
    constexpr int M = 4;
    const size_t qstride = (half + 63) & ~(size_t)63;
    int32_t rc;
    const bool built = e->g2tab_hi == hi && e->g2tab_half == half && e->tab_owner == nullptr;
    if (!built && (rc = fold_g2_table_build(e, st, hi, half))) return rc;
    e->g2tab_hi = nullptr;
    if ((rc = jac.reserve(half * sizeof(G2J))) || (rc = e->fix_flags.reserve(4 * half + 16))) return rc;
    if (!e->sw.no_fq && half >= e->fq_min)
    {
        hipLaunchKernelGGL(HIP_KERNEL_NAME(k_fold_g2_tab_q<GlsDigits, 4>), dim3(nblk(half, 64)), dim3(64), 0, st, e->fold_tab.as<uint4>(), qstride, M, lo, (uint32_t)half, gls_wnaf(s, 4), jac.as<G2J>(), e->fix_flags.as<uint8_t>());
#if !defined(RIPP_INLINE_FALLBACK)
        hipLaunchKernelGGL(HIP_KERNEL_NAME(k_fold_g2_tab_fix<GlsDigits, 4>), dim3(FIX_GRID), dim3(64), 0, st, e->fold_tab.as<uint4>(), qstride, M, lo, (uint32_t)half, gls_wnaf(s, 4), jac.as<G2J>(), e->fix_flags.as<uint8_t>());
#endif
    }
    else
        hipLaunchKernelGGL(HIP_KERNEL_NAME(k_fold_g2_tab<GlsDigits, 4>), dim3(nblk(half, 64)), dim3(64), 0, st, e->fold_tab.as<uint4>(), qstride, M, lo, (uint32_t)half, gls_wnaf(s, 4), jac.as<G2J>());
    HIPCHK(hipGetLastError());
    return RIPP_OK;
}

int32_t job_prebuild_g2_tables(Engine* e, ripp_sipp_job* j) {
    const size_t half = j->len / 2;
    e->g2tab_hi = nullptr;
    if (e->sw.no_prebuild || e->sw.no_endo || half < 1) return RIPP_OK;
    const bool vm_form = (half <= e->vm_fold_max || half <= e->vm_joint_max) && !e->sw.no_vm;
    if (vm_form || j->pre_ready || j->pre_vm_ready || (j->tab_ready && e->tab_owner == j) || !fold_g2_table_pays(e, half)) return RIPP_OK;
    const bool xs = xscale_round(e, j, half);
    if (j->bs_on && !xs) return RIPP_OK;
    if (!fold_g2_table_fits(e, half)) return RIPP_OK;
    const G2A* b = j->b.as<G2A>();
    return fold_g2_table_build(e, e->stream, xs ? b : b + half, half);
}

int32_t job_fold(Engine* e, ripp_sipp_job* j, const Fr& x, bool allow_vm = true, bool async = false) {
    const size_t half = j->len / 2;
    int32_t rc;
    const Fr x_inv = inv(x);
    hipEvent_t t0 = e->ev_t0, t1 = e->ev_t1;
    HIPCHK(hipEventRecord(t0, e->stream));
    if (async) { hipEvent_t fa, fb; HIPCHK(hipEventCreate(&fa)); HIPCHK(hipEventCreate(&fb)); e->ev_fold_async.emplace_back(fa, fb); HIPCHK(hipEventRecord(fa, e->stream)); }
    G1A* a = j->a.as<G1A>(); G2A* b = j->b.as<G2A>();
    const size_t qstride = (half + 63) & ~(size_t)63;
    if ((rc = e->qtab.reserve(4 * G2A_CHUNKS * qstride * sizeof(uint4))) != RIPP_OK) return rc;
    const bool use_vm = allow_vm && half <= e->vm_fold_max && !e->sw.no_vm;
    const bool mid_vm = allow_vm && !use_vm && half <= e->vm_joint_max && !e->sw.no_vm && !e->sw.no_endo;
    if ((rc = e->vm_flag.reserve(sizeof(uint32_t))) != RIPP_OK) return rc;
    const bool pre = j->pre_ready && fits_128(x); j->pre_ready = false;
    const bool pre_vm = j->pre_vm_ready && fits_128(x) && allow_vm; j->pre_vm_ready = false;
    const hipStream_t g1s = e->stream2;
    HIPCHK(hipEventRecord(e->ev_fork, e->stream));
    HIPCHK(hipStreamWaitEvent(e->stream2, e->ev_fork, 0));
    const bool tab = j->tab_ready && e->tab_owner == j && fits_128(x); j->tab_ready = false;
    const int tabW = tab_width(j->tab_M);
    const G1A* tab1 = e->fold_tab1.as<G1A>() + (j->tab_fused ? half / 2 : 0);
    if (tab && !e->sw.no_fq && half >= e->fq_min)
        hipLaunchKernelGGL(k_fold_g1_tab_q, dim3(nblk(half, 256)), dim3(256), 0, g1s, tab1, j->tab_cnt, j->tab_M, a, (uint32_t)half, split32_wnaf(x, tabW), j->jac1.as<G1J>());
    else if (tab)
        hipLaunchKernelGGL(k_fold_g1_tab, dim3(nblk(half, 256)), dim3(256), 0, g1s, tab1, j->tab_cnt, j->tab_M, a, (uint32_t)half, split32_wnaf(x, tabW), j->jac1.as<G1J>());
    else if (pre)
        hipLaunchKernelGGL(k_fold_g1_two, dim3(nblk(half, 256)), dim3(256), 0, g1s, a + half, j->a_pow.as<G1A>(), a, (uint32_t)half, split64_digits(x), j->jac1.as<G1J>());
    else if (pre_vm) {
        hipLaunchKernelGGL(HIP_KERNEL_NAME(k_vm_fold_split2<Fp>), dim3(nblk(half, 4 * VM_EPW), 2), dim3(256), 4 * VM_EPW * VmCurve<Fp>::SLOTS * sizeof(VmSlot), g1s, a + half, j->a_pow_h.as<G1J>(), (uint32_t)half, split_digits_g1(x), 1, j->parts1.as<G1J>());
        hipLaunchKernelGGL(HIP_KERNEL_NAME(k_vm_combine<Fp>), dim3(nblk(half, 4 * VM_EPW)), dim3(256), 4 * VM_EPW * VmCurve<Fp>::SLOTS * sizeof(VmSlot), g1s, j->parts1.as<G1J>(), 2, a, (uint32_t)half, j->jac1.as<G1J>());
    }
    else if (use_vm || mid_vm)
        hipLaunchKernelGGL(k_vm_fold_g1, dim3(nblk(half, 4 * VM_EPW)), dim3(256), 4 * VM_EPW * VM_G1_SLOTS * sizeof(VmSlot), g1s, a + half, a, (uint32_t)half, naf_digits(x), j->jac1.as<G1J>(), e->vm_flag.as<uint32_t>());
    else if (!e->sw.no_fq && half >= e->fq_min_g1)
        hipLaunchKernelGGL(k_fold_g1_naf_q, dim3(nblk(half, 256)), dim3(256), 0, g1s, a + half, a, (uint32_t)half, naf_digits(x), j->jac1.as<G1J>());
    else
        hipLaunchKernelGGL(HIP_KERNEL_NAME(k_fold_affine_naf<Fp>), dim3(nblk(half, 256)), dim3(256), 0, g1s, a + half, a, (uint32_t)half, naf_digits(x), j->jac1.as<G1J>());
    HIPCHK(hipGetLastError());
    if ((rc = e->normalize_dev<Fp>(j->jac1.as<G1J>(), half, j->a_next.as<G1A>(), g1s)) != RIPP_OK) return rc;
    HIPCHK(hipEventRecord(e->ev_join, g1s));
    const bool xs = xscale_round(e, j, half) && fits_128(x) && (!tab || j->tab_on_lo);
    const bool unscale = j->bs_on && !xs;
    if (tab && j->tab_on_lo != xs) return (set_err("fold tables were built for the other half"), RIPP_ERR_ARG);
    const G2A* g2_hi = xs ? b : b + half; const G2A* g2_lo = xs ? b + half : b;
    const Fr g2_s = xs ? x : x_inv;
    if (unscale) {
        const Fr s_inv = inv(j->bs), sx_inv = mul(s_inv, x_inv);
        if (mid_vm) {
            GlsDigits2 d2; d2.a = gls_digits(s_inv); d2.b = gls_digits(sx_inv);
            hipLaunchKernelGGL(k_vm_fold_g2_joint2, dim3(nblk(half, 4 * VM_EPW)), dim3(256), 4 * VM_EPW * VM_G2_SLOTS * sizeof(VmSlot), e->stream, b, b + half, (uint32_t)half, d2, j->jac2.as<G2J>());
        } else {
        if ((rc = e->qtab.reserve(8 * half * sizeof(G2J))) != RIPP_OK || (rc = e->fix_flags.reserve(8 * half + 32)) != RIPP_OK) return rc;
        HIPCHK(hipStreamWaitEvent(e->stream3, e->ev_fork, 0));
        for (int t = 0; t < 2; ++t) {
            hipStream_t st2 = t ? e->stream3 : e->stream; const G2A* src = t ? b + half : b; const GlsDigits dg2 = gls_digits(t ? sx_inv : s_inv);
            G2J* parts = e->qtab.as<G2J>() + (size_t)t * 4 * half; uint8_t* flags = e->fix_flags.as<uint8_t>() + (size_t)t * ((4 * half + 15) & ~(size_t)15);
            if (!e->sw.no_fq) {
                hipLaunchKernelGGL(k_fold_g2_gls_split_q, dim3(nblk(half, 64), 4), dim3(64), 0, st2, src, (uint32_t)half, dg2, parts, flags);
#if !defined(RIPP_INLINE_FALLBACK)
                hipLaunchKernelGGL(k_fold_g2_gls_split_fix, dim3(FIX_GRID), dim3(64), 0, st2, src, (uint32_t)half, dg2, parts, flags);
#endif
            } else hipLaunchKernelGGL(k_fold_g2_gls_split, dim3(nblk(half, 64), 4), dim3(64), 0, st2, src, (uint32_t)half, dg2, parts);
        }
        HIPCHK(hipEventRecord(e->ev_join3, e->stream3)); HIPCHK(hipStreamWaitEvent(e->stream, e->ev_join3, 0));
        hipLaunchKernelGGL(k_fold_g2_combine8, dim3(nblk(half, 64)), dim3(64), 0, e->stream, e->qtab.as<G2J>(), (uint32_t)half, j->jac2.as<G2J>());
        }
        j->bs = Fr::one(); j->bs_on = false;
    } else
    if (pre_vm) {
        if (j->pre_vm_side) { HIPCHK(hipStreamWaitEvent(e->stream, e->ev_join3, 0)); j->pre_vm_side = false; }
        hipLaunchKernelGGL(HIP_KERNEL_NAME(k_vm_fold_split2<Fp2>), dim3(nblk(half, 4 * VM_EPW), 8), dim3(256), 4 * VM_EPW * VmCurve<Fp2>::SLOTS * sizeof(VmSlot), e->stream, b + half, j->b_pow_h.as<G2J>(), (uint32_t)half, split_digits_g2(x_inv), 4, j->parts2.as<G2J>());
        hipLaunchKernelGGL(HIP_KERNEL_NAME(k_vm_combine<Fp2>), dim3(nblk(half, 4 * VM_EPW)), dim3(256), 4 * VM_EPW * VmCurve<Fp2>::SLOTS * sizeof(VmSlot), e->stream, j->parts2.as<G2J>(), 8, b, (uint32_t)half, j->jac2.as<G2J>());
    } else
    if (tab && !e->sw.no_fq && half >= e->fq_min) {
        if ((rc = e->fix_flags.reserve(4 * half + 16))) return rc;
        hipLaunchKernelGGL(HIP_KERNEL_NAME(k_fold_g2_tab_q<Wnaf16, 16>), dim3(nblk(half, 64)), dim3(64), 0, e->stream, e->fold_tab.as<uint4>(), j->tab2_stride, j->tab_M, g2_lo, (uint32_t)half, gls16_wnaf(g2_s, tabW), j->jac2.as<G2J>(), e->fix_flags.as<uint8_t>());
#if !defined(RIPP_INLINE_FALLBACK)
        hipLaunchKernelGGL(HIP_KERNEL_NAME(k_fold_g2_tab_fix<Wnaf16, 16>), dim3(FIX_GRID), dim3(64), 0, e->stream, e->fold_tab.as<uint4>(), j->tab2_stride, j->tab_M, g2_lo, (uint32_t)half, gls16_wnaf(g2_s, tabW), j->jac2.as<G2J>(), e->fix_flags.as<uint8_t>());
#endif
    } else
    if (tab) {
        hipLaunchKernelGGL(HIP_KERNEL_NAME(k_fold_g2_tab<Wnaf16, 16>), dim3(nblk(half, 64)), dim3(64), 0, e->stream, e->fold_tab.as<uint4>(), j->tab2_stride, j->tab_M, g2_lo, (uint32_t)half, gls16_wnaf(g2_s, tabW), j->jac2.as<G2J>());
    } else
    if (pre) {
        if ((rc = e->qtab.reserve(8 * G2A_CHUNKS * qstride * sizeof(uint4))) != RIPP_OK) return rc;
        hipLaunchKernelGGL(k_fold_g2_gls8, dim3(nblk(half, 64)), dim3(64), 0, e->stream, b + half, j->b_pow.as<G2A>(), b, (uint32_t)half, gls8_digits(x_inv), e->qtab.as<uint4>(), qstride, j->jac2.as<G2J>());
    } else
    if (mid_vm) {
        hipLaunchKernelGGL(k_vm_fold_g2_joint, dim3(nblk(half, 4 * VM_EPW)), dim3(256), 4 * VM_EPW * VM_G2_SLOTS * sizeof(VmSlot), e->stream, g2_hi, g2_lo, (uint32_t)half, gls_digits(g2_s), j->jac2.as<G2J>());
    } else
    if (use_vm) {
        if ((rc = e->qtab.reserve(std::max<size_t>(4 * G2A_CHUNKS * qstride * sizeof(uint4), 4 * half * sizeof(G2J)))) != RIPP_OK) return rc;
        hipLaunchKernelGGL(k_vm_fold_g2_split, dim3(nblk(half, 4 * VM_EPW), 4), dim3(256), 4 * VM_EPW * VM_G2_SLOTS * sizeof(VmSlot), e->stream, b + half, (uint32_t)half, gls_digits(x_inv), e->qtab.as<G2J>(), e->vm_flag.as<uint32_t>());
        hipLaunchKernelGGL(k_vm_combine_g2, dim3(nblk(half, 4 * VM_EPW)), dim3(256), 4 * VM_EPW * VM_G2_SLOTS * sizeof(VmSlot), e->stream, e->qtab.as<G2J>(), b, (uint32_t)half, j->jac2.as<G2J>());
    } else
    if (e->sw.no_endo) {
        hipLaunchKernelGGL(HIP_KERNEL_NAME(k_fold_affine_naf<Fp2>), dim3(nblk(half, 256)), dim3(256), 0, e->stream, b + half, b, (uint32_t)half, naf_digits(x_inv), j->jac2.as<G2J>());
    } else
    if (half <= e->gls_split_max || (fold_g2_table_pays(e, half) && !(e->g2tab_hi && e->g2tab_half == half) && !fold_g2_table_fits(e, half) && ((e->mem_tier |= 16), true))) {
        if ((rc = e->qtab.reserve(std::max<size_t>(4 * G2A_CHUNKS * qstride * sizeof(uint4), 4 * half * sizeof(G2J)))) != RIPP_OK) return rc;
        if (!e->sw.no_fq) {
            if ((rc = e->fix_flags.reserve(4 * half + 16))) return rc;
            hipLaunchKernelGGL(k_fold_g2_gls_split_q, dim3(nblk(half, 64), 4), dim3(64), 0, e->stream, g2_hi, (uint32_t)half, gls_digits(g2_s), e->qtab.as<G2J>(), e->fix_flags.as<uint8_t>());
#if !defined(RIPP_INLINE_FALLBACK)
            hipLaunchKernelGGL(k_fold_g2_gls_split_fix, dim3(FIX_GRID), dim3(64), 0, e->stream, g2_hi, (uint32_t)half, gls_digits(g2_s), e->qtab.as<G2J>(), e->fix_flags.as<uint8_t>());
#endif
        }
        else hipLaunchKernelGGL(k_fold_g2_gls_split, dim3(nblk(half, 64), 4), dim3(64), 0, e->stream, g2_hi, (uint32_t)half, gls_digits(g2_s), e->qtab.as<G2J>());
        hipLaunchKernelGGL(k_fold_g2_combine, dim3(nblk(half, 64)), dim3(64), 0, e->stream, e->qtab.as<G2J>(), g2_lo, (uint32_t)half, j->jac2.as<G2J>());
    } else if (fold_g2_table_pays(e, half)) {
        if ((rc = fold_g2_table(e, e->stream, g2_hi, g2_lo, half, g2_s, j->jac2)) != RIPP_OK) return rc;
    } else {
        hipLaunchKernelGGL(k_fold_g2_gls, dim3(nblk(half, 64)), dim3(64), 0, e->stream, b + half, b, (uint32_t)half, gls_digits(x_inv), e->qtab.as<uint4>(), qstride, j->jac2.as<G2J>());
    }
    HIPCHK(hipGetLastError());
    if (xs) { j->bs = j->bs_on ? mul(j->bs, x) : x; j->bs_on = true; }
    if ((rc = e->normalize_dev<Fp2>(j->jac2.as<G2J>(), half, j->b_next.as<G2A>())) != RIPP_OK) return rc;
    HIPCHK(hipStreamWaitEvent(e->stream, e->ev_join, 0));
    HIPCHK(hipEventRecord(t1, e->stream));
    if (!async) {
        if ((rc = e->sync()) != RIPP_OK) return rc;
        float ms = 0; (void)hipEventElapsedTime(&ms, t0, t1); e->stats.fold_ms += ms;
    } else HIPCHK(hipEventRecord(e->ev_fold_async.back().second, e->stream));
    std::swap(j->a, j->a_next); std::swap(j->b, j->b_next);
    j->len = half;
    return RIPP_OK;
}

int32_t job_fold_fused(Engine* e, ripp_sipp_job* j, const Fr& x0, const Fr& x1, bool async) {
    const size_t q = j->len / 4;
    int32_t rc;
    if (!(j->tab_ready && j->tab_fused && e->tab_owner == j && j->tab_on_lo && !j->bs_on && fits_128(x0) && fits_128(x1))) { set_err("fused fold: the three-quarter tables of this job are not in place"); return RIPP_ERR_ARG; }
    j->tab_ready = false; j->pre_ready = false; j->pre_vm_ready = false;
    hipEvent_t t0 = e->ev_t0, t1 = e->ev_t1;
    HIPCHK(hipEventRecord(t0, e->stream));
    if (async) { hipEvent_t fa, fb; HIPCHK(hipEventCreate(&fa)); HIPCHK(hipEventCreate(&fb)); e->ev_fold_async.emplace_back(fa, fb); HIPCHK(hipEventRecord(fa, e->stream)); }
    if ((rc = j->jac1.reserve(q * sizeof(G1J))) || (rc = j->jac2.reserve(q * sizeof(G2J))) || (rc = e->fix_flags.reserve(2 * ((q + 15) & ~(size_t)15) + 32))) return rc;
    const int W = tab_width(j->tab_M);
    G1A* a = j->a.as<G1A>(); G2A* b = j->b.as<G2A>();
    uint8_t* flag1 = e->fix_flags.as<uint8_t>(); uint8_t* flag2 = flag1 + ((q + 15) & ~(size_t)15) + 16;
    HIPCHK(hipEventRecord(e->ev_fork, e->stream));
    HIPCHK(hipStreamWaitEvent(e->stream2, e->ev_fork, 0));
    const hipStream_t g1s = e->stream2;
    const WnafG1x4 d1 = fused_digits_g1(x0, x1, W);
    hipLaunchKernelGGL(k_fold_g1_fused_q, dim3(nblk(q, 256)), dim3(256), 0, g1s, e->fold_tab1.as<G1A>(), j->tab_cnt, j->tab_M, a, (uint32_t)q, d1, j->jac1.as<G1J>(), flag1);
    hipLaunchKernelGGL(k_fold_g1_fused_fix, dim3(FIX_GRID), dim3(64), 0, g1s, e->fold_tab1.as<G1A>(), j->tab_cnt, j->tab_M, a, (uint32_t)q, d1, j->jac1.as<G1J>(), flag1);
    HIPCHK(hipGetLastError());
    if ((rc = e->normalize_dev<Fp>(j->jac1.as<G1J>(), q, j->a_next.as<G1A>(), g1s)) != RIPP_OK) return rc;
    HIPCHK(hipEventRecord(e->ev_join, g1s));
    const Wnaf16x3 d2 = fused_digits_g2(x0, x1, W);
    hipLaunchKernelGGL(k_fold_g2_fused_q, dim3(nblk(q, 64)), dim3(64), 0, e->stream, e->fold_tab.as<uint4>(), j->tab2_stride, j->tab_M, b + 3 * q, (uint32_t)q, d2, j->jac2.as<G2J>(), flag2);
    hipLaunchKernelGGL(k_fold_g2_fused_fix, dim3(FIX_GRID), dim3(64), 0, e->stream, e->fold_tab.as<uint4>(), j->tab2_stride, j->tab_M, b + 3 * q, (uint32_t)q, d2, j->jac2.as<G2J>(), flag2);
    HIPCHK(hipGetLastError());
    j->bs = mul(x0, x1); j->bs_on = true;
    if ((rc = e->normalize_dev<Fp2>(j->jac2.as<G2J>(), q, j->b_next.as<G2A>())) != RIPP_OK) return rc;
    HIPCHK(hipStreamWaitEvent(e->stream, e->ev_join, 0));
    HIPCHK(hipEventRecord(t1, e->stream));
    if (!async) {
        if ((rc = e->sync()) != RIPP_OK) return rc;
        float ms = 0; (void)hipEventElapsedTime(&ms, t0, t1); e->stats.fold_ms += ms;
    } else HIPCHK(hipEventRecord(e->ev_fold_async.back().second, e->stream));
    std::swap(j->a, j->a_next); std::swap(j->b, j->b_next);
    j->len = q;
    return RIPP_OK;
}

void job_start_hash(ripp_sipp_job* j, const Fp12& value) {
    if (j->hash_prestarted) { j->hash_prestarted = false; return; }
    if (j->hash_thread.joinable()) j->hash_thread.join();
    j->digest_ready = false;
    const G1A* pa = j->ha_ext ? j->ha_ext : j->ha.data(); const G2A* pb = j->ha_ext ? j->hb_ext : j->hb.data(); const Fr* pr = j->ha_ext ? j->hr_ext : j->hr.data();
    const size_t pn = j->ha_ext ? j->hash_n : j->ha.size();
    j->hash_done = 0; j->hash_total = (uint64_t)pn * (96 + 192 + 32); j->hash_t0 = now_ms();
    j->hash_thread = std::thread([j, value, pa, pb, pr, pn]() { statement_digest(pa, pb, pr, pn, value, j->digest, &j->hash_done); j->digest_ready = true; });
}

}

extern "C" {

#define API __attribute__((visibility("default")))
#define LOCK std::lock_guard<std::mutex> lk_(g_mu)
#define ENGINE Engine* e; { int32_t rc_ = get_engine(&e); if (rc_ != RIPP_OK) return rc_; }

API const char* ripp_last_error(void) { return g_err.c_str(); }
static_assert(sizeof(ripp_stats) == 24 * 8, "ripp_stats changed: bump RIPP_ABI_VERSION (include/ripp_hip.h) and the bindings (ripp_amd/_lib.py, rust/ripp-hip/src/ffi.rs)");
API int32_t ripp_abi_version(void) { return RIPP_ABI_VERSION; }
API size_t ripp_stats_size(void) { return sizeof(ripp_stats); }
API void ripp_statement_hash_times(double* hash_ms, double* wait_ms) { if (hash_ms) *hash_ms = g_digest_hash_ms; if (wait_ms) *wait_ms = g_digest_wait_ms; }
API int32_t ripp_device_count(void) { int n = 0; if (hipGetDeviceCount(&n) != hipSuccess) return 0; return n; }
extern "C++" { static void vec_caches_release(); }
API int32_t ripp_init(int32_t dev) {
    LOCK;
    if (g_engine) {
        if (g_engine->device == dev) return RIPP_OK;
        if (g_live_handles.load() > 0) { set_err("ripp_init: " + std::to_string(g_live_handles.load()) + " job / SRS handle(s) are alive on device " + std::to_string(g_engine->device) + "; destroy them before re-binding the engine"); return RIPP_ERR_ARG; }
        vec_caches_release();
        g_engine->destroy(); delete g_engine; g_engine = nullptr;
    }
    Engine* e = new Engine(); int32_t rc = e->init(dev);
    if (rc != RIPP_OK) { delete e; return rc; }
    g_engine = e; return RIPP_OK;
}
API void ripp_shutdown(void) {
    LOCK; if (!g_engine) return;
    if (g_live_handles.load() > 0) { set_err("ripp_shutdown: " + std::to_string(g_live_handles.load()) + " job / SRS / vector handle(s) are still alive; destroy them first"); fprintf(stderr, "[ripp] %s\n", g_err.c_str()); return; }
    vec_caches_release();
    g_engine->destroy(); delete g_engine; g_engine = nullptr;
}
API int32_t ripp_release_scratch(void) {
    LOCK; if (!g_engine) return RIPP_OK;
    Engine* e = g_engine;
    if (hipSetDevice(e->device) != hipSuccess || hipDeviceSynchronize() != hipSuccess) { set_err("ripp_release_scratch: device synchronisation failed"); return RIPP_ERR_DEVICE; }
    for (DevBuf* b : {&e->lines, &e->partA, &e->partB, &e->jacG1, &e->jacG2, &e->tmpA, &e->tmpB, &e->tmpR, &e->affG1, &e->affG2, &e->qtab, &e->scale_tab, &e->fold_tab1, &e->fold_mult, &e->fold_tab, &e->fold_jac1, &e->fold_jac2, &e->fix_flags, &e->scale_flags}) b->release();
    e->msm_scratch[0].release(); e->msm_scratch[1].release(); e->kzg_q[0].release(); e->kzg_q[1].release(); e->kzg_bases[0].release(); e->kzg_bases[1].release(); e->pc_release();
    for (PinBuf& pb : e->stage) pb.release();
    e->tab_owner = nullptr; e->g2tab_hi = nullptr; e->job_cache.release(); vec_caches_release();
    if (e->aux) { e->aux->destroy(); delete e->aux; e->aux = nullptr; }
    for (Engine* p : e->peers) { (void)hipSetDevice(p->device); p->destroy(); delete p; }
    if (!e->peers.empty()) { e->peers.clear(); (void)hipSetDevice(e->device); }
    return RIPP_OK;
}

API size_t ripp_device_bytes(void) { return g_dev_bytes.load(std::memory_order_relaxed); }

API int32_t ripp_normalize_g1(const ripp_g1j* in, size_t n, ripp_g1a* out) {
    LOCK; ENGINE; if (n == 0) return RIPP_OK; if (!in || !out) return RIPP_ERR_ARG;
    G1J* d; int32_t rc = upload<G1J>(e, e->jacG1, in, n, &d); if (rc) return rc;
    if ((rc = e->affG1.reserve(n * sizeof(G1A)))) return rc;
    if ((rc = e->normalize_dev<Fp>(d, n, e->affG1.as<G1A>()))) return rc;
    HIPCHK(hipMemcpyAsync(out, e->affG1.p, n * sizeof(G1A), hipMemcpyDeviceToHost, e->stream));
    return e->sync();
}
API int32_t ripp_normalize_g2(const ripp_g2j* in, size_t n, ripp_g2a* out) {
    LOCK; ENGINE; if (n == 0) return RIPP_OK; if (!in || !out) return RIPP_ERR_ARG;
    G2J* d; int32_t rc = upload<G2J>(e, e->jacG2, in, n, &d); if (rc) return rc;
    if ((rc = e->affG2.reserve(n * sizeof(G2A)))) return rc;
    if ((rc = e->normalize_dev<Fp2>(d, n, e->affG2.as<G2A>()))) return rc;
    HIPCHK(hipMemcpyAsync(out, e->affG2.p, n * sizeof(G2A), hipMemcpyDeviceToHost, e->stream));
    return e->sync();
}
API int32_t ripp_scale_g1_a(const ripp_g1a* a, const ripp_fr* r, size_t n, ripp_g1a* out) {
    LOCK; ENGINE; if (n == 0) return RIPP_OK; if (!a || !r || !out) return RIPP_ERR_ARG;
    G1A* da; Fr* dr; int32_t rc;
    if ((rc = upload<G1A>(e, e->tmpA, a, n, &da))) return rc;
    if ((rc = upload<Fr>(e, e->tmpR, r, n, &dr))) return rc;
    if ((rc = e->jacG1.reserve(n * sizeof(G1J)))) return rc;
    if ((rc = e->affG1.reserve(n * sizeof(G1A)))) return rc;
    if ((rc = e->scale_g1_dev(da, 1u, dr, n, e->jacG1.as<G1J>()))) return rc;
    if ((rc = e->normalize_dev<Fp>(e->jacG1.as<G1J>(), n, e->affG1.as<G1A>()))) return rc;
    HIPCHK(hipMemcpyAsync(out, e->affG1.p, n * sizeof(G1A), hipMemcpyDeviceToHost, e->stream));
    return e->sync();
}

extern "C++" {
template <class F, bool JAC_IN, bool AFF_OUT, class IN, class OUT>
static int32_t fold_impl(const IN* hi, const IN* lo, size_t half, const ripp_fr* s, OUT* out) {
    LOCK; ENGINE; if (half == 0) return RIPP_OK; if (!hi || !lo || !s || !out) return RIPP_ERR_ARG;
    Fr sm; std::memcpy(&sm, s, sizeof(Fr));
    const ScalarBits sb = scalar_bits(sm);
    int32_t rc;
    DevBuf& jac = std::is_same<F, Fp>::value ? e->jacG1 : e->jacG2;
    DevBuf& aff = std::is_same<F, Fp>::value ? e->affG1 : e->affG2;
    if ((rc = jac.reserve(half * sizeof(Jac<F>)))) return rc;
    if (JAC_IN) {
        Jac<F>*dh, *dl;
        if ((rc = upload<Jac<F>>(e, e->tmpA, hi, half, &dh))) return rc;
        if ((rc = upload<Jac<F>>(e, e->tmpB, lo, half, &dl))) return rc;
        hipLaunchKernelGGL(HIP_KERNEL_NAME(k_fold_jac<F>), dim3(nblk(half, 64)), dim3(64), 0, e->stream, dh, dl, (uint32_t)half, sb, jac.as<Jac<F>>());
    } else {
        Affine<F>*dh, *dl;
        if ((rc = upload<Affine<F>>(e, e->tmpA, hi, half, &dh))) return rc;
        if ((rc = upload<Affine<F>>(e, e->tmpB, lo, half, &dl))) return rc;
        if (std::is_same<F, Fp2>::value && !e->sw.no_endo) {
            const size_t qstride = (half + 63) & ~(size_t)63;
            if ((rc = e->qtab.reserve(4 * G2A_CHUNKS * qstride * sizeof(uint4)))) return rc;
            hipLaunchKernelGGL(k_fold_g2_gls, dim3(nblk(half, 64)), dim3(64), 0, e->stream, reinterpret_cast<const G2A*>(dh), reinterpret_cast<const G2A*>(dl), (uint32_t)half,
                               gls_digits(sm), e->qtab.as<uint4>(), qstride, reinterpret_cast<G2J*>(jac.p));
        } else {
            hipLaunchKernelGGL(HIP_KERNEL_NAME(k_fold_affine_naf<F>), dim3(nblk(half, 256)), dim3(256), 0, e->stream, dh, dl, (uint32_t)half, naf_digits(sm), jac.as<Jac<F>>());
        }
    }
    HIPCHK(hipGetLastError());
    if (AFF_OUT) {
        if ((rc = aff.reserve(half * sizeof(Affine<F>)))) return rc;
        if ((rc = e->normalize_dev<F>(jac.as<Jac<F>>(), half, aff.as<Affine<F>>()))) return rc;
        HIPCHK(hipMemcpyAsync(out, aff.p, half * sizeof(Affine<F>), hipMemcpyDeviceToHost, e->stream));
    } else {
        HIPCHK(hipMemcpyAsync(out, jac.p, half * sizeof(Jac<F>), hipMemcpyDeviceToHost, e->stream));
    }
    return e->sync();
}
}
API int32_t ripp_fold_g1_a(const ripp_g1a* hi, const ripp_g1a* lo, size_t half, const ripp_fr* s, ripp_g1a* out) { return fold_impl<Fp, false, true>(hi, lo, half, s, out); }
API int32_t ripp_fold_g2_a(const ripp_g2a* hi, const ripp_g2a* lo, size_t half, const ripp_fr* s, ripp_g2a* out) { return fold_impl<Fp2, false, true>(hi, lo, half, s, out); }
API int32_t ripp_fold_g1_j(const ripp_g1j* hi, const ripp_g1j* lo, size_t half, const ripp_fr* s, ripp_g1j* out) { return fold_impl<Fp, true, false>(hi, lo, half, s, out); }
API int32_t ripp_fold_g2_j(const ripp_g2j* hi, const ripp_g2j* lo, size_t half, const ripp_fr* s, ripp_g2j* out) { return fold_impl<Fp2, true, false>(hi, lo, half, s, out); }

API int32_t ripp_fold_fr(const ripp_fr* hi, const ripp_fr* lo, size_t half, const ripp_fr* s, ripp_fr* out) {
    LOCK; ENGINE; if (half == 0) return RIPP_OK; if (!hi || !lo || !s || !out) return RIPP_ERR_ARG;
    Fr sm; std::memcpy(&sm, s, sizeof sm);
    Fr *dh, *dl; int32_t rc;
    if ((rc = upload<Fr>(e, e->tmpA, hi, half, &dh)) || (rc = upload<Fr>(e, e->tmpB, lo, half, &dl)) || (rc = e->tmpR.reserve(half * sizeof(Fr)))) return rc;
    hipLaunchKernelGGL(k_fold_fr, dim3(nblk(half, 256)), dim3(256), 0, e->stream, dh, dl, (uint32_t)half, sm, e->tmpR.as<Fr>());
    HIPCHK(hipGetLastError());
    HIPCHK(hipMemcpyAsync(out, e->tmpR.p, half * sizeof(Fr), hipMemcpyDeviceToHost, e->stream));
    return e->sync();
}

extern "C++" {
static std::atomic<int32_t> g_last_slots{1};
struct DevSlot { Engine* e; size_t off, cnt; };
static int32_t device_slots(Engine* e, size_t n, size_t min_units, std::vector<DevSlot>* out) {
    size_t D = e->n_devices_cfg > 1 ? e->n_devices_cfg : 1;
    if (min_units && D > n / min_units) D = std::max<size_t>(1, n / min_units);
    out->clear();
    if (D > 1) {
        int count = 0; (void)hipGetDeviceCount(&count);
        for (size_t d = 1; d < D; ++d) {
            const int phys = e->virtual_devices ? e->device : e->device + (int)d;
            if (phys >= count) { set_err("n_devices = " + std::to_string(e->n_devices_cfg) + ": device " + std::to_string(phys) + " does not exist (" + std::to_string(count) + " visible)"); (void)hipSetDevice(e->device); return RIPP_ERR_ARG; }
            if (e->peers.size() < d) {
                Engine* p = new Engine(); const int32_t rc = p->init(phys);
                (void)hipSetDevice(e->device);
                if (rc != RIPP_OK) { delete p; return rc; }
                e->peers.push_back(p);
            } else if (e->peers[d - 1]->device != phys) { set_err("n_devices: the device mapping changed under live peer engines (ripp_release_scratch first)"); return RIPP_ERR_ARG; }
            e->peers[d - 1]->refresh_switches(); e->peers[d - 1]->stats = ripp_stats{};
        }
    }
    for (size_t d = 0; d < D; ++d) { const size_t lo = n * d / D, hi = n * (d + 1) / D; out->push_back({d == 0 ? e : e->peers[d - 1], lo, hi - lo}); }
    g_last_slots = (int32_t)D;
    return RIPP_OK;
}
template <class FN> static int32_t run_on_devices(Engine* e, const std::vector<DevSlot>& sl, FN fn) {
    if (sl.size() == 1) return fn(sl[0].e, sl[0].off, sl[0].cnt, 0);
    std::vector<int32_t> rcs(sl.size(), RIPP_OK); std::vector<std::string> errs(sl.size());
    std::vector<std::thread> th;
    for (size_t d = 1; d < sl.size(); ++d)
        th.emplace_back([&, d]() {
            if (hipSetDevice(sl[d].e->device) != hipSuccess) { rcs[d] = RIPP_ERR_DEVICE; errs[d] = "hipSetDevice failed"; return; }
            t_engine = sl[d].e;
            rcs[d] = fn(sl[d].e, sl[d].off, sl[d].cnt, (int)d);
            if (rcs[d]) errs[d] = g_err;
        });
    rcs[0] = fn(sl[0].e, sl[0].off, sl[0].cnt, 0); if (rcs[0]) errs[0] = g_err;
    for (std::thread& t : th) t.join();
    (void)hipSetDevice(e->device);
    for (size_t d = 0; d < sl.size(); ++d) if (rcs[d]) { set_err("device slot " + std::to_string(d) + " of " + std::to_string(sl.size()) + ": " + errs[d]); return rcs[d]; }
    return RIPP_OK;
}
constexpr size_t PAIRS_PER_DEVICE_MIN = 4096, MSM_TERMS_PER_DEVICE_MIN = (size_t)1 << 15;
}
API int32_t ripp_device_slots_used(void) { return g_last_slots.load(); }

static int32_t pairing_product_dev(Engine* e, const G1A* da, const G2A* db, size_t n, ripp_gt* out) {
// ... 559 lines not shown
            auto rows = std::make_shared<std::vector<Fp12>>(grows.begin() + (size_t)g * N_LINES, grows.begin() + (size_t)(g + 1) * N_LINES);
            li.fe.push_back(look_pool().submit([rows]() { return final_exponentiation(miller_combine(rows->data())); }));
        }
        ++e->stats.look_items;
    }
    e->stats.look_ms += now_ms() - t0;
    if (trace_on()) fprintf(stderr, "[ripp] look-ahead: %zu of %d (round, side) values pre-evaluated in the hash window, %.1f ms (hash %s)\n", j->look.size(), items, now_ms() - t0, j->digest_ready.load() ? "already done" : "still running");
    return RIPP_OK;
}
static void look_finish_level(ripp_sipp_job::LookItem& it) {
    if (it.pend.empty()) return;
    const size_t S = it.Z.size() / 3;
    std::vector<Fp12> Zn(S);
    for (size_t r = 0; r < S; ++r) { const Fp12 lo = mul(it.pend[3 * r].get(), it.pend[3 * r + 1].get()); Zn[r] = mul(mul(lo, it.Z[S + r]), it.pend[3 * r + 2].get()); }
    it.pend.clear(); it.Z.swap(Zn); ++it.level;
}
static void look_start_level(ripp_sipp_job::LookItem& it, const GlsDigits& gx, const GlsDigits& gxi) {
    if (!it.fe.empty()) { it.Z.resize(it.fe.size()); for (size_t i = 0; i < it.fe.size(); ++i) it.Z[i] = it.fe[i].get(); it.fe.clear(); }
    const size_t S = it.Z.size() / 3;
    for (size_t r = 0; r < S; ++r) {
        const Fp12 zm = it.Z[r], zp = it.Z[2 * S + r];
        it.pend.push_back(host_pool().submit([zm, gxi]() { return gt_pow_gls_strings(zm, gxi, 3u); }));
        it.pend.push_back(host_pool().submit([zm, gxi]() { return gt_pow_gls_strings(zm, gxi, 12u); }));
        it.pend.push_back(host_pool().submit([zp, gx]() { return gt_pow_gls_strings(zp, gx, 15u); }));
    }
}
static void look_apply(ripp_sipp_job* j, size_t t, const Fr& x) {
    bool any = false; for (auto& it : j->look) any = any || (size_t)it.R > t;
    if (!any) return;
    const GlsDigits gx = gls_digits(x), gxi = gls_digits(inv(x));
    for (int pass = 0; pass < 2; ++pass) for (auto& it : j->look) {
        if ((size_t)it.R <= t || ((size_t)it.R == t + 1) != (pass == 0)) continue;
        look_finish_level(it);
        look_start_level(it, gx, gxi);
    }
}
static ripp_sipp_job::LookItem* look_find(ripp_sipp_job* j, size_t round, int side) { for (auto& it : j->look) if ((size_t)it.R == round && it.side == side) return &it; return nullptr; }
static bool look_full(ripp_sipp_job* j, size_t round) { const auto* l = look_find(j, round, 0); const auto* r = look_find(j, round, 1); return l && r && l->npairs == l->q && r->npairs == r->q; }

static int32_t job_round0_shared(Engine* e, ripp_sipp_job* j, Fp12* rows) {
    const size_t q = j->len / 4;
    const G1A* a = j->a.as<G1A>(); const G2A* b = j->b.as<G2A>();
    const G1A* as[8] = {a + 2 * q, a + q, a + 3 * q,   a, a + q, a + 3 * q,   a + 3 * q,   a + q};
    const G2A* bs[8] = {b, b, b,   b + 2 * q, b + 2 * q, b + 2 * q,   b + q,   b + 3 * q};
    std::vector<Fp12> all((size_t)8 * N_LINES);
    const double t0 = now_ms();
    int32_t rc = e->step_products(as, bs, 8, q, all.data());
    e->stats.miller_products_ms += now_ms() - t0;
    if (rc) return rc;
    auto row = [&](int p) { return all.data() + (size_t)p * N_LINES; };
    for (int s2 = 0; s2 < N_LINES; ++s2) { rows[s2] = mul(row(0)[s2], row(6)[s2]); rows[N_LINES + s2] = mul(row(3)[s2], row(7)[s2]); }
    j->look.clear();
    j->look.emplace_back();
    ripp_sipp_job::LookItem& li = j->look.back();
    li.R = 1; li.side = 0; li.level = 0; li.npairs = q; li.q = q;
    for (int g = 0; g < 3; ++g) {
        auto grows = std::make_shared<std::vector<Fp12>>((size_t)N_LINES);
        for (int s2 = 0; s2 < N_LINES; ++s2) (*grows)[s2] = g == 0 ? row(4)[s2] : g == 1 ? mul(row(1)[s2], row(5)[s2]) : row(2)[s2];
        li.fe.push_back(look_pool().submit([grows]() { return final_exponentiation(miller_combine(grows->data())); }));
    }
    ++e->stats.look_items; e->stats.look_pairs += 4 * q;
    return RIPP_OK;
}

static std::atomic<int> g_fail_rank{-1}, g_fail_round{-1};
static bool test_fail_hit(int rank, size_t round) {
    if (g_fail_rank.load(std::memory_order_relaxed) == rank && g_fail_round.load(std::memory_order_relaxed) == 1000 + (int)round) raise(SIGKILL);
    if (g_fail_rank.load(std::memory_order_relaxed) != rank || g_fail_round.load(std::memory_order_relaxed) != (int)round) return false;
    g_fail_rank = -1; g_fail_round = -1;
    set_err("injected failure (ripp_test_inject_failure) in the fold of round " + std::to_string(round) + " on rank " + std::to_string(rank));
    return true;
}
struct SippPlanMsg { uint64_t n_local; int32_t world, rank, look_items, window, rc, pad; double hash_left_ms; };
struct SippRoundMsg { Fp12 z[2]; uint8_t digest[32]; int32_t rc, pad[3]; };
struct SippTailMsg { G1A a; G2A b; int32_t rc, pad[3]; };
static int32_t sipp_prove_core(Engine* e, ripp_sipp_job* j, const Fp12& val, const uint8_t* seed_digest, ripp_gt* proof, ripp_fr* challenges, ripp_stats* st) {
    const int world0 = j->world0, rank = j->rank;
    const double t_start = now_ms();
    double exchange_ms = 0;
    comm_mark_proof();
    e->mem_tier = 0;
    struct Quiesce { Engine* e; ripp_sipp_job* j; ~Quiesce() {
        (void)hipStreamSynchronize(e->stream); (void)hipStreamSynchronize(e->stream2); (void)hipStreamSynchronize(e->stream3);
        j->tp_round[0] = j->tp_round[1] = ~(size_t)0; j->pre_vm_ready = false; j->pre_vm_side = false; j->pre_ready = false; j->tab_ready = false; j->look.clear();
        e->g2tab_hi = nullptr;
        if (j->hash_thread.joinable()) j->hash_thread.join();
        j->ha_ext = nullptr; j->hb_ext = nullptr; j->hr_ext = nullptr; j->hash_prestarted = false; } } quiesce{e, j};
    const bool window = rank == 0 && !seed_digest;
    if (rank == 0) {
        if (seed_digest) { if (j->hash_thread.joinable()) j->hash_thread.join(); std::memcpy(j->digest, seed_digest, 32); j->digest_ready = true; j->hash_prestarted = false; }
        else job_start_hash(j, val);
    }
    const bool look_forced = e->look_eighths >= 0;
    int look_items = (rank == 0 || look_forced) ? look_plan(e, j->n_local, world0, window || look_forced) : 0;
    j->no_window = !window; j->look_deadline = 0;
    if (world0 > 1) {
        double hash_left = 0;
        if (window && j->hash_total > 0) hash_left = std::max(0.0, (double)j->hash_total / (e->cal_hash_bytes_per_ms > 0 ? e->cal_hash_bytes_per_ms : 1.17e6) - (now_ms() - j->hash_t0));
        SippPlanMsg mine{(uint64_t)j->n_local, world0, rank, look_items, window ? 1 : 0, RIPP_OK, 0, hash_left};
        std::vector<SippPlanMsg> all((size_t)world0);
        const double tx = now_ms();
        t_ex_kind = EX_PLAN;
        int32_t rc = comm_allgather(e, &mine, all.data(), sizeof mine); if (rc) return rc;
        exchange_ms += now_ms() - tx;
        for (int w = 0; w < world0; ++w) {
            if (all[w].rc) { set_err("sharded SIPP proof: rank " + std::to_string(w) + " failed before the proof started (status " + std::to_string(all[w].rc) + ")"); return RIPP_ERR_DEVICE; }
            if (all[w].n_local != (uint64_t)j->n_local || all[w].world != world0 || all[w].rank != w) { set_err("sharded SIPP proof: the ranks disagree on the shard size / world size / rank order"); return RIPP_ERR_ARG; }
        }
        look_items = all[0].look_items; j->no_window = !all[0].window;
        if (rank != 0 && all[0].window && all[0].hash_left_ms > 0) j->look_deadline = now_ms() + all[0].hash_left_ms;
    }
    struct HotOff { ~HotOff() { host_pool().set_hot(false); } } hot_off;
    struct QuietOff { Engine* e; ~QuietOff() { e->quiet_waits = false; } } quiet_off{e};
    e->quiet_waits = window && e->quiet_waits_cfg;
    j->look_rows[0].blocking = j->look_rows[1].blocking = e->quiet_waits;
    struct XsOff { ripp_sipp_job* j; ~XsOff() { j->xs_enabled = false; } } xs_off{j};
    j->xs_enabled = true; j->seeded = false;
    int32_t lrc = job_begin(e, j);
    if (lrc && world0 == 1) return lrc;
    e->stats.look_items = 0; e->stats.look_pairs = 0; e->stats.look_ms = 0;
    if (trace_on()) fprintf(stderr, "[ripp] scale+normalize done at t=%.1f ms\n", now_ms() - t_start);
    size_t len = j->n_local;
    bool sharded = world0 > 1, digest_sent = world0 == 1;
    size_t round = 0;
    Fr x_prev = Fr::zero();
    bool fuse_pending = false; Fr x0_saved = Fr::zero();
    j->tp_round[0] = j->tp_round[1] = ~(size_t)0;
    while ((sharded ? len * (size_t)world0 : len) > 1) {
        if (sharded && len == 1) {
            SippTailMsg mine; std::memset((void*)&mine, 0, sizeof mine);
            if (!lrc) {
                auto grab = [&]() -> int32_t {
                    HIPCHK(hipStreamSynchronize(e->stream2)); HIPCHK(hipStreamSynchronize(e->stream3));
                    HIPCHK(hipMemcpyAsync(&mine.a, j->a.p, sizeof(G1A), hipMemcpyDeviceToHost, e->stream));
                    HIPCHK(hipMemcpyAsync(&mine.b, j->b.p, sizeof(G2A), hipMemcpyDeviceToHost, e->stream));
                    return e->sync(); };
                lrc = grab();
            }
            mine.rc = lrc;
            std::vector<SippTailMsg> all((size_t)world0);
            const double tx = now_ms();
            int32_t rc = comm_allgather(e, &mine, all.data(), sizeof mine); if (rc) return rc;
            exchange_ms += now_ms() - tx;
            for (int w = 0; w < world0; ++w) if (all[w].rc) { if (!lrc) set_err("sharded SIPP proof: rank " + std::to_string(w) + " failed (status " + std::to_string(all[w].rc) + ")"); return lrc ? lrc : RIPP_ERR_DEVICE; }
            const size_t L = (size_t)world0;
            if ((rc = j->a.reserve(L * sizeof(G1A))) || (rc = j->b.reserve(L * sizeof(G2A))) || (rc = j->a_next.reserve(L * sizeof(G1A))) ||
                (rc = j->b_next.reserve(L * sizeof(G2A))) || (rc = j->jac1.reserve(L * sizeof(G1J))) || (rc = j->jac2.reserve(L * sizeof(G2J))) || (rc = e->stage[3].reserve(L * (sizeof(G1A) + sizeof(G2A))))) return rc;
            G1A* ha = e->stage[3].as<G1A>(); G2A* hb = reinterpret_cast<G2A*>(ha + L);
            for (size_t w = 0; w < L; ++w) { ha[w] = all[w].a; hb[w] = all[w].b; }
            if (j->bs_on) { set_err("sharded SIPP proof: the G2 vector is still x-scaled at the tail gather"); return RIPP_ERR_ARG; }
            HIPCHK(hipMemcpyAsync(j->a.p, ha, L * sizeof(G1A), hipMemcpyHostToDevice, e->stream));
            HIPCHK(hipMemcpyAsync(j->b.p, hb, L * sizeof(G2A), hipMemcpyHostToDevice, e->stream));
            if ((rc = e->sync())) return rc;
            j->len = len = L; j->world = 1; sharded = false;
            j->pre_vm_ready = false;
            continue;
        }
        Fp12 rows[2 * N_LINES];
        const double tr0 = now_ms();
        ripp_sipp_job::LookItem* lk_l = lrc ? nullptr : look_find(j, round, 0);
        ripp_sipp_job::LookItem* lk_r = lrc ? nullptr : look_find(j, round, 1);
        const bool tp_round = !lrc && j->tp_round[round & 1] == round;
        double t0 = tr0;
        double round0_ms_per_pair = 7.7e-5;
        bool shared_r0 = false;
        Fp12 zl = Fp12::one(), zr = Fp12::one();
        auto local_values = [&]() -> int32_t {
            int32_t rc;
            const size_t half = fuse_pending ? j->len / 4 : j->len / 2;
            const size_t start[2] = {lk_l ? std::min(lk_l->npairs, half) : 0, lk_r ? std::min(lk_r->npairs, half) : 0};
            const bool dev[2] = {!tp_round && start[0] < half, !tp_round && start[1] < half};
            if (dev[0] && dev[1] && start[0] == 0 && start[1] == 0) {
                const double tp = now_ms();
                shared_r0 = round == 0 && !j->seeded && look_items >= 8 && j->len >= 4 && !e->sw.no_share && !e->sw.no_precompute && (look_forced || !j->digest_ready.load());
                if (shared_r0) { if ((rc = job_round0_shared(e, j, rows))) return rc; }
                else if ((rc = job_round_partials(e, j, rows))) return rc;
                if (round == 0 && j->len >= ((size_t)1 << 16)) {
                    round0_ms_per_pair = (now_ms() - tp) / (double)(shared_r0 ? 2 * j->len : j->len);
                    if (e->ranks_per_device <= 1.0) e->cal_ms_per_pair = round0_ms_per_pair;
                }
            }
            else for (int sd = 0; sd < 2; ++sd) {
                if (!dev[sd]) continue;
                const G1A* as[1] = {j->a.as<G1A>() + (sd == 0 ? half : 0) + start[sd]}; const G2A* bs[1] = {j->b.as<G2A>() + (sd == 0 ? 0 : half) + start[sd]};
                const double tp = now_ms();
                if ((rc = e->step_products(as, bs, 1, half - start[sd], rows + sd * N_LINES))) return rc;
                e->stats.miller_products_ms += now_ms() - tp;
            }
            if (round >= 1 && !fuse_pending && !tp_round && (rc = job_prebuild_g2_tables(e, j))) return rc;
            const bool plan_fuse = look_forced ? look_items >= 16 : look_items >= 12;
            if (round == 0 && !j->seeded && (rc = job_precompute_round0(e, j, (plan_fuse || e->sw.fuse_tables) && j->len >= 4))) return rc;
            if (!j->pre_vm_ready && (rc = job_precompute_vm(e, j))) return rc;
            const bool next_known = round == 0 ? (plan_fuse && j->len >= 4 && (look_forced || !j->digest_ready.load())) : look_full(j, round + 1);
            if (!tp_round && !next_known && tail_pipe_ok(e, j) && (rc = job_tail_enqueue(e, j, round + 1))) return rc;
            t0 = now_ms();
            if (tp_round) { if ((rc = job_tail_values(j, round, x_prev, &zl, &zr))) return rc; }
            else {
                Fp12 zd[2] = {Fp12::one(), Fp12::one()};
                if (dev[0] && dev[1]) pairing_values(rows, 2, zd);
                else if (dev[0]) pairing_values(rows, 1, &zd[0]);
                else if (dev[1]) pairing_values(rows + N_LINES, 1, &zd[1]);
                if (j->bs_on && (dev[0] || dev[1])) {
                    const GlsDigits gsi = gls_digits(inv(j->bs));
                    if (host_pool().size() >= 11) {
                        Fp12 part[8];
                        host_pool().parallel(8, [&](int t) { if (!dev[t >> 2]) return; part[t] = gt_pow_gls_strings(zd[t >> 2], gsi, 1u << (t & 3)); });
                        for (int k = 0; k < 2; ++k) if (dev[k]) zd[k] = mul(mul(part[4 * k], part[4 * k + 1]), mul(part[4 * k + 2], part[4 * k + 3]));
                    } else {
                    Fp12 part[4];
                    host_pool().parallel(4, [&](int t) { if (!dev[t >> 1]) return; part[t] = gt_pow_gls_strings(zd[t >> 1], gsi, (t & 1) ? 12u : 3u); });
                    for (int k = 0; k < 2; ++k) if (dev[k]) zd[k] = mul(part[2 * k], part[2 * k + 1]);
                    }
                }
                zl = zd[0]; zr = zd[1];
                if (lk_l) { look_finish_level(*lk_l); zl = dev[0] ? mul(lk_l->Z[0], zd[0]) : lk_l->Z[0]; }
                if (lk_r) { look_finish_level(*lk_r); zr = dev[1] ? mul(lk_r->Z[0], zd[1]) : lk_r->Z[0]; }
            }
            if (round == 0 && !j->seeded && (rc = job_lookahead(e, j, look_items, look_forced, round0_ms_per_pair, shared_r0 ? 1 : 0))) return rc;
            return RIPP_OK;
        };
        if (!lrc) lrc = local_values();
        if (lrc && !sharded) return lrc;
        if (!j->seeded && rank == 0) {
            const double th = now_ms();
            if (j->hash_thread.joinable()) j->hash_thread.join();
            e->stats.hash_ms += now_ms() - th;
        }
        if (sharded || !digest_sent) {
            SippRoundMsg mine; std::memset((void*)&mine, 0, sizeof mine);
            mine.z[0] = zl; mine.z[1] = zr; mine.rc = lrc;
            if (rank == 0) std::memcpy(mine.digest, j->digest, 32);
            std::vector<SippRoundMsg> all((size_t)world0);
            const double tx = now_ms();
            int32_t rc = comm_allgather(e, &mine, all.data(), sizeof mine); if (rc) return rc;
            exchange_ms += now_ms() - tx;
            for (int w = 0; w < world0; ++w) if (all[w].rc) { if (!lrc) set_err("sharded SIPP proof: rank " + std::to_string(w) + " failed (status " + std::to_string(all[w].rc) + ")"); return lrc ? lrc : RIPP_ERR_DEVICE; }
            if (sharded) { zl = all[0].z[0]; zr = all[0].z[1]; for (int w = 1; w < world0; ++w) { zl = mul(zl, all[w].z[0]); zr = mul(zr, all[w].z[1]); } }
            if (!digest_sent) { std::memcpy(j->digest, all[0].digest, 32); digest_sent = true; }
        }
        if (!j->seeded) {
            j->rng.from_digest(j->digest); j->seeded = true;
            e->quiet_waits = false;
            host_pool().set_hot(e->hot_workers_cfg ? (e->hot_workers_cfg == 1 && effective_cpus() >= (int)host_pool().size() + 2) : hot_workers_pay(world0));
        }
        const Fr x = fs::sipp_challenge(j->rng, zl, zr);
        x_prev = x;
        look_apply(j, round, x);
        e->stats.host_ms += now_ms() - t0;
        std::memcpy(&proof[2 * round], &zl, sizeof(Fp12)); std::memcpy(&proof[2 * round + 1], &zr, sizeof(Fp12));
        if (challenges) std::memcpy(&challenges[round], &x, sizeof(Fr));
        const double tf0 = now_ms();
        const bool pipelined = j->tp_round[(round + 1) & 1] == round + 1;
        const bool known = look_full(j, round + 1);
        if (!sharded && len == 2) { j->len = 0; j->pre_vm_ready = false; }
        else {
            if (!lrc && test_fail_hit(rank, round)) lrc = RIPP_ERR_DEVICE;
            if (!lrc && fuse_pending) { lrc = job_fold_fused(e, j, x0_saved, x, pipelined || known); fuse_pending = false; }
            else if (!lrc && round == 0 && known && j->tab_ready && j->tab_fused && e->tab_owner == j && !j->bs_on) { fuse_pending = true; x0_saved = x; }
            else
            if (!lrc) lrc = job_fold(e, j, x, true, pipelined || known);
            if (!lrc && pipelined) {
                if (!j->pre_vm_ready) lrc = job_precompute_vm(e, j, true);
                if (!lrc && tail_pipe_ok(e, j)) lrc = job_tail_enqueue(e, j, round + 2);
            }
            if (lrc && !sharded) return lrc;
        }
        len /= 2;
        if (trace_on()) fprintf(stderr, "[ripp] round %2zu len %8zu: products %.2f ms, host %.2f ms, fold %.2f ms%s (t=%.1f)\n", round, len * 2, t0 - tr0, tf0 - t0, now_ms() - tf0, (pipelined || known) ? " (enqueued)" : "", now_ms() - t_start);
        ++round;
    }
    if (j->hash_thread.joinable()) j->hash_thread.join();
    host_pool().set_hot(false);
    if (lrc) return lrc;
    int32_t rc;
    if ((rc = e->sync())) return rc; HIPCHK(hipStreamSynchronize(e->stream2)); HIPCHK(hipStreamSynchronize(e->stream3));
    e->collect_kernel_stats();
    e->stats.exchange_ms = exchange_ms;
    e->stats.mem_tier = (uint64_t)e->mem_tier; e->stats.device_bytes = g_dev_bytes.load();
    e->stats.statement_hash_ms = window ? g_digest_hash_ms : 0; e->stats.statement_hash_wait_ms = window ? g_digest_wait_ms : 0;
    if (window && j->hash_total >= ((uint64_t)336 << 16) && g_digest_hash_ms + g_digest_wait_ms > 1.0) e->cal_hash_bytes_per_ms = (double)j->hash_total / (g_digest_hash_ms + g_digest_wait_ms);
    e->stats.total_ms = now_ms() - t_start;
    if (st) *st = e->stats;
    return RIPP_OK;
}

static void config_from_engine(const Engine* e, ripp_config* c) {
    std::memset(c, 0, sizeof *c); c->struct_size = (uint32_t)sizeof *c;
    c->no_vm = e->sw.no_vm; c->no_precompute = e->sw.no_precompute; c->no_fold_tables = e->sw.no_fold_tables; c->no_msm_glv = e->sw.no_msm_glv; c->lp_one_lane = e->sw.lp_one_lane;
    c->no_endo = e->sw.no_endo; c->no_fq = e->sw.no_fq; c->no_xscale = e->sw.no_xscale; c->no_share = e->sw.no_share; c->no_fuse = e->sw.no_fuse; c->fuse_tables = e->sw.fuse_tables; c->scale_no_fq = e->scale_no_fq; c->agg_sequential = e->agg_sequential; c->look_static = e->look_static; c->quiet_waits = e->quiet_waits_cfg;
    c->look_eighths = e->look_eighths; c->ranks_per_device = (int32_t)e->ranks_per_device; c->msm_c = e->msm_tune.c; c->msm_ch = e->msm_tune.ch; c->msm_gmin = e->msm_tune.gmin; c->no_prebuild = e->sw.no_prebuild;
    c->vm_lines_max = e->vm_lines_max; c->vm_fold_max = e->vm_fold_max; c->vm_tree_max = e->vm_tree_max; c->gls_split_max = e->gls_split_max; c->msm_vm_merge_max = e->msm_vm_merge_max; c->fold_tab_min = e->fold_tab_min;
    c->fq_min = e->fq_min; c->lp_fq_min = e->lp_fq_min; c->vm_joint_max = e->vm_joint_max; c->vm_scale_max = e->vm_scale_max; c->tail_pipe_max = e->tail_pipe_max; c->ml_fq_min = e->ml_fq_min; c->fq_min_g1 = e->fq_min_g1; c->msm_lds_sort_min = e->msm_lds_sort_min; c->msm_chunk_min = e->msm_chunk_min;
    c->mem_cap_bytes = e->mem_cap; c->hot_workers = (uint32_t)e->hot_workers_cfg; c->no_job_cache = e->sw.no_job_cache;
    c->no_lp_karatsuba = e->sw.no_lp_kara; c->comm_timeout_ms = e->comm_timeout_ms; c->plan_derate_pct = e->plan_derate_pct; c->n_devices = e->n_devices_cfg;
}
API int32_t ripp_config_default(ripp_config* cfg) {
    if (!cfg) return RIPP_ERR_ARG;
    Engine tmp; tmp.defaults = Engine::Sizes{tmp.vm_lines_max, tmp.vm_fold_max, tmp.vm_tree_max, tmp.gls_split_max, tmp.msm_vm_merge_max, tmp.fold_tab_min, tmp.fq_min, tmp.lp_fq_min, tmp.vm_joint_max, tmp.vm_scale_max, tmp.tail_pipe_max, tmp.ml_fq_min, tmp.fq_min_g1, tmp.msm_lds_sort_min, tmp.msm_chunk_min};
    config_from_engine(&tmp, cfg); cfg->look_eighths = -1; cfg->ranks_per_device = 1;
    return RIPP_OK;
}
API int32_t ripp_configure(const ripp_config* cfg) {
    LOCK;
    if (!cfg) { g_cfg_set = false; return RIPP_OK; }
    if (cfg->struct_size != sizeof(ripp_config)) { set_err("ripp_configure: struct_size does not match this library's ripp_config (fill the struct with ripp_config_default first)"); return RIPP_ERR_ARG; }
    g_cfg = *cfg; g_cfg_set = true;
    return RIPP_OK;
}
API int32_t ripp_config_get(ripp_config* cfg) {
    if (!cfg) return RIPP_ERR_ARG;
    LOCK; ENGINE;
    config_from_engine(e, cfg);
    return RIPP_OK;
}

API void ripp_test_inject_failure(int32_t rank, int32_t round) { g_fail_rank = rank; g_fail_round = round; }

API int32_t ripp_sipp_job_prove(ripp_sipp_job* j, const ripp_gt* value, ripp_gt* proof, ripp_fr* challenges, ripp_stats* st) {
    LOCK; ENGINE; if (!j || !value || !proof || j->world0 != 1) return RIPP_ERR_ARG;
    Fp12 val; std::memcpy(&val, value, sizeof(Fp12));
    return sipp_prove_core(e, j, val, nullptr, proof, challenges, st);
}

extern "C++" {
static int32_t sipp_prove_devices(Engine* e, std::vector<DevSlot>& sl, const ripp_g1a* a, const ripp_g2a* b, const ripp_fr* r, size_t n, const ripp_gt* value,
                                  ripp_gt* proof, ripp_fr* challenges, ripp_stats* st) {
    const size_t D = sl.size(), nl = n / D; size_t rounds = 0; while (((size_t)1 << rounds) < n) ++rounds;
    LocalComm lc; lc.world = (int)D;
    Fp12 val; std::memcpy(&val, value, sizeof val);
    struct Out { std::vector<ripp_gt> proof; std::vector<ripp_fr> ch; ripp_stats st; };
    std::vector<Out> outs(D);
    const bool virt = e->virtual_devices;
    int32_t rc = run_on_devices(e, sl, [&](Engine* ee, size_t, size_t, int d) -> int32_t {
        t_lcomm = &lc; t_lrank = d;
        struct Unbind { ~Unbind() { t_lcomm = nullptr; t_lrank = 0; } } unbind;
        if (virt) ee->ranks_per_device = (double)D;
        std::vector<G1A> sa(nl); std::vector<G2A> sb(nl); std::vector<Fr> sr(nl);
        for (size_t i = 0; i < nl; ++i) { std::memcpy(&sa[i], &a[i * D + (size_t)d], sizeof(G1A)); std::memcpy(&sb[i], &b[i * D + (size_t)d], sizeof(G2A)); std::memcpy(&sr[i], &r[i * D + (size_t)d], sizeof(Fr)); }
        ripp_sipp_job* j = nullptr;
        int32_t r2 = sipp_job_create_on(ee, reinterpret_cast<const ripp_g1a*>(sa.data()), reinterpret_cast<const ripp_g2a*>(sb.data()), reinterpret_cast<const ripp_fr*>(sr.data()), nl, d, (int32_t)D,
                                        d == 0 ? value : nullptr, &j, d == 0 ? a : nullptr, d == 0 ? b : nullptr, d == 0 ? r : nullptr, n, true);
        if (r2) { lc.fail(); return r2; }
        if (d == 0 && !j->hash_prestarted) {
// ... 119 lines not shown
```

### ripp_amd/csrc/fq_curve.hpp

```cpp
#pragma once
#include "fq28.hpp"
#include "kernels.hpp"

namespace ripp {

#if defined(__HIP_DEVICE_COMPILE__)
using FqC = Fq<FQ_LN, 4>;

template <uint64_t LM, int VB>
__device__ __forceinline__ Fqn fq_reduce(const Fq<LM, VB>& a) {
    using namespace fq28;
    static_assert((uint64_t)VB * (P_TOP + 1) < ((uint64_t)1 << 31), "top limb must stay a positive int");
    const Fq<FQ_LN, VB> n = fq_norm(a);
    constexpr float INV = (1.0f - 1.0f / 1048576.0f) / (float)(P_TOP + 1);
    const int q = (int)((float)n.l[NL - 1] * INV);
    Fqn r; int64_t carry = 0;
#pragma unroll
    for (int i = 0; i < NL - 1; ++i) { const int64_t t = (int64_t)n.l[i] - (int64_t)q * (int32_t)P28.l[i] + carry; r.l[i] = (uint32_t)t & MASK; carry = t >> W; }
    r.l[NL - 1] = (uint32_t)((int64_t)n.l[NL - 1] - (int64_t)q * (int32_t)P28.l[NL - 1] + carry);
    return r;
}
__device__ __forceinline__ bool fq_is_zero(const Fqn& a) {
    uint32_t z = 0, e = 0;
#pragma unroll
// ... 174 lines not shown
            a2 = dbl(a2);
#pragma unroll 1
            for (int t = 0; t < 4; ++t) { const int d = dg.d[t][pos]; if (d != 0) { G1A q = tab[(size_t)(M * t + ((d < 0 ? -d : d) >> 1)) * tstride + i]; if (d < 0) q.y = neg(q.y); a2 = add_mixed(a2, q); } }
        }
        out[i] = add_mixed(a2, l);
    } else out[i] = jacq_to_g1j(acc);
#endif
}

struct WnafG1x4 { int8_t d[16][36]; int len; };
__device__ __noinline__ inline G1J fold_g1_fused_complete(const G1A* __restrict__ tab, size_t tstride, int M, const G1A& l, uint32_t q, uint32_t i, const WnafG1x4& dg) {
    G1J a2 = jac_inf<Fp>();
#pragma unroll 1
    for (int pos = dg.len - 1; pos >= 0; --pos) {
        a2 = dbl(a2);
#pragma unroll 1
        for (int t = 0; t < 16; ++t) {
            const int d = dg.d[t][pos]; if (d == 0) continue;
            const int u = t >> 2; const uint32_t el = (u == 0 ? q : u == 3 ? 0u : 2 * q) + i;
            G1A p = tab[(size_t)(M * (t & 3) + ((d < 0 ? -d : d) >> 1)) * tstride + el];
            if (u == 2) p.x = fmul(p.x, fp_const(RIPP_GLV_BETA));
            if (d < 0) p.y = neg(p.y);
            a2 = add_mixed(a2, p);
        }
    }
    return add_mixed(a2, l);
}
__global__ void __launch_bounds__(256, 2) k_fold_g1_fused_q(const G1A* __restrict__ tab, size_t tstride, int M, const G1A* __restrict__ lo, uint32_t q, WnafG1x4 dg, G1J* __restrict__ out, uint8_t* __restrict__ flag) {
    const uint32_t i = blockIdx.x * blockDim.x + threadIdx.x;
    if (i >= q) return;
#if defined(__HIP_DEVICE_COMPILE__)
    constexpr uint32_t betaw[12] = RIPP_GLV_BETA; constexpr fq28::Limbs BETA = fq28::from_mont384(betaw);
    JacQ acc; jq_set_identity(acc);
    bool inf = true, bad = false;
#pragma unroll 1
    for (int pos = dg.len - 1; pos >= 0; --pos) {
        if (!inf) jdbl_q(acc);
#pragma unroll 1
        for (int t = 0; t < 16; ++t) {
            const int d = dg.d[t][pos];
            if (d == 0) continue;
            const int u = t >> 2;
            uint32_t el = i; asm volatile("" : "+v"(el));
            el += u == 0 ? q : u == 3 ? 0u : 2 * q;
            const G1A qa = tab[(size_t)(M * (t & 3) + ((d < 0 ? -d : d) >> 1)) * tstride + el];
            bad |= is_inf(qa);
            if (inf) {
                AffQ p = affq_from(qa);
                if (u == 2) p.x = fq_mul(p.x, fq_const<FQ_LN, 1>(BETA));
                if (d < 0) p.y = fq_reduce(fq_neg(p.y));
                jq_set(acc, p.x, p.y, fq_one()); inf = false;
            } else {
                FqTab px = fq_tab(qa.x);
                if (u == 2) px = fq_widen<FQ_LN, 256>(fq_mul(px, fq_const<FQ_LN, 1>(BETA)));
                bad |= jmadd_q(acc, px, fq_tab_y(qa.y, d < 0));
            }
        }
    }
    const G1A l = lo[i];
    if (inf) { out[i] = to_jac(l); flag[i] = 0; return; }
    if (!is_inf(l)) { const AffQ lq = affq_from(l); bad |= jmadd_q(acc, lq.x, lq.y); }
    flag[i] = bad;
    if (!bad) out[i] = jacq_to_g1j(acc);
#endif
}
__global__ void __launch_bounds__(64) k_fold_g1_fused_fix(const G1A* __restrict__ tab, size_t tstride, int M, const G1A* __restrict__ lo, uint32_t q, WnafG1x4 dg, G1J* __restrict__ out, const uint8_t* __restrict__ flag) {
    for_flagged(flag, q, [&](uint32_t i) { out[i] = fold_g1_fused_complete(tab, tstride, M, lo[i], q, i, dg); });
}

__global__ void __launch_bounds__(256, 2) k_pow2_mul_g1_q(const G1A* __restrict__ in, uint32_t n, int k, G1J* __restrict__ out) {
    const uint32_t i = blockIdx.x * blockDim.x + threadIdx.x;
    if (i >= n) return;
#if defined(__HIP_DEVICE_COMPILE__)
    const G1A p = in[i];
    if (is_inf(p)) { out[i] = jac_inf<Fp>(); return; }
    const AffQ q = affq_from(p);
    JacQ acc; jq_set(acc, q.x, q.y, fq_one());
#pragma unroll 1
    for (int t = 0; t < k; ++t) jdbl_q(acc);
    out[i] = jacq_to_g1j(acc);
#endif
}

}
```

### ripp_amd/csrc/fq_curve2.hpp

```cpp
#pragma once
#include "fq_curve.hpp"

namespace ripp {

#if defined(__HIP_DEVICE_COMPILE__)
#if defined(RIPP_BLS12_377)
constexpr int FQ2_BETA = 5;
#else
constexpr int FQ2_BETA = 1;
#endif
template <uint64_t L1, int V1> __device__ __forceinline__ auto fq_mul_beta(const Fq<L1, V1>& a) {
    if constexpr (FQ2_BETA == 1) return a;
    else { static_assert(FQ2_BETA == 5, "FQ2_BETA"); return fq_add(fq_dbl(fq_dbl(a)), a); }
}
template <uint64_t LM = FQ_LN, int VB = 2> struct Fq2T { Fq<LM, VB> c0, c1; };
using Fq2n = Fq2T<FQ_LN, 2>;
using Fq2C = Fq2T<FQ_LN, 4>;

template <uint64_t L1, int V1, uint64_t L2, int V2> __device__ __forceinline__ auto f2_add(const Fq2T<L1, V1>& a, const Fq2T<L2, V2>& b) { return Fq2T<L1 + L2 - 1, V1 + V2>{fq_add(a.c0, b.c0), fq_add(a.c1, b.c1)}; }
template <uint64_t L1, int V1, uint64_t L2, int V2> __device__ __forceinline__ auto f2_sub(const Fq2T<L1, V1>& a, const Fq2T<L2, V2>& b) { return Fq2T<fq28::sub_lm(L1, L2), V1 + V2 + 1>{fq_sub(a.c0, b.c0), fq_sub(a.c1, b.c1)}; }
template <uint64_t L1, int V1> __device__ __forceinline__ auto f2_dbl(const Fq2T<L1, V1>& a) { return Fq2T<2 * L1 - 1, 2 * V1>{fq_dbl(a.c0), fq_dbl(a.c1)}; }
template <uint64_t L1, int V1> __device__ __forceinline__ auto f2_norm(const Fq2T<L1, V1>& a) { return Fq2T<FQ_LN, V1>{fq_norm(a.c0), fq_norm(a.c1)}; }
template <uint64_t L1, int V1> __device__ __forceinline__ Fq2n f2_reduce(const Fq2T<L1, V1>& a) { return {fq_reduce(a.c0), fq_reduce(a.c1)}; }
template <uint64_t L1, int V1> __device__ __forceinline__ Fq2C f2_coord(const Fq2T<L1, V1>& a) { return {fq_coord(a.c0), fq_coord(a.c1)}; }
// ... 320 lines not shown
    if (M < 2) return;
    for_flagged(flag, n, [&](uint32_t i) { odd_multiples_complete<Fp2>(base, n, M, i, out); });
}

__device__ __noinline__ inline G2J fold_g2_gls_split_complete(const G2A& q, const GlsDigits& dg, int j) {
    G2J acc = jac_inf<Fp2>();
#pragma unroll 1
    for (int pos = dg.len - 1; pos >= 0; --pos) {
        acc = dbl(acc);
        const int d = dg.d[j][pos];
        if (d != 0) { G2A t = q; if (d < 0) t.y = neg(t.y); acc = add_mixed(acc, t); }
    }
    return acc;
}
__global__ void __launch_bounds__(64, 2) k_fold_g2_gls_split_q(const G2A* __restrict__ hi, uint32_t half, GlsDigits dg, G2J* __restrict__ parts , uint8_t* __restrict__ flag ) {
    __shared__ uint4 park_[21 * 64];
    const uint32_t i = blockIdx.x * blockDim.x + threadIdx.x;
    if (i >= half) return;
    const int j = blockIdx.y;
#if defined(__HIP_DEVICE_COMPILE__)
    uint4* park = park_ + threadIdx.x;
    uint4* qpark = park + 7 * 64;
    auto st7 = [](uint4* dst, const Fq2n& v) { uint32_t w[28];
#pragma unroll
        for (int k = 0; k < 14; ++k) { w[k] = v.c0.l[k]; w[14 + k] = v.c1.l[k]; }
        const uint4* src = reinterpret_cast<const uint4*>(w);
#pragma unroll
        for (int k = 0; k < 7; ++k) dst[k * 64] = src[k]; };
    auto ld7 = [](const uint4* src) { uint4 q[7];
#pragma unroll
        for (int k = 0; k < 7; ++k) q[k] = src[k * 64];
        const uint32_t* w = reinterpret_cast<const uint32_t*>(q);
        Fq2n v;
#pragma unroll
        for (int k = 0; k < 14; ++k) { v.c0.l[k] = w[k]; v.c1.l[k] = w[14 + k]; }
        return v; };
    bool bad;
    {
        const G2A q = gls_image(hi[i], j);
        bad = is_inf(q);
        st7(qpark, f2_from(q.x)); st7(qpark + 7 * 64, f2_from(q.y));
    }
    JacQ2 acc; j2_set_identity(acc);
    bool inf = true;
#pragma unroll 1
    for (int pos = dg.len - 1; pos >= 0; --pos) {
        if (!inf) jdbl2_q(acc);
        const int d = dg.d[j][pos];
        if (d == 0) continue;
        auto loadx = [&]() { return ld7(qpark); };
        auto loady = [&]() { const Fq2n y = ld7(qpark + 7 * 64); if (d > 0) return y; return Fq2n{fq_reduce(fq_neg(y.c0)), fq_reduce(fq_neg(y.c1))}; };
        if (inf) { j2_set(acc, loadx(), loady(), Fq2n{fq_one(), fq_zero()}); f2_pin(acc.z); inf = false; }
        else bad |= jmadd2_q(acc, loadx, loady, park);
    }
#if !defined(RIPP_INLINE_FALLBACK)
    flag[(size_t)j * half + i] = bad;
    if (bad) return;
#else
    if (bad) { parts[(size_t)j * half + i] = fold_g2_gls_split_complete(gls_image(hi[i], j), dg, j); return; }
#endif
    if (inf) parts[(size_t)j * half + i] = jac_inf<Fp2>();
    else parts[(size_t)j * half + i] = G2J{f2_to(acc.x), f2_to(acc.y), f2_to(acc.z)};
#endif
}
__global__ void __launch_bounds__(64) k_fold_g2_gls_split_fix(const G2A* __restrict__ hi, uint32_t half, GlsDigits dg, G2J* __restrict__ parts, const uint8_t* __restrict__ flag) {
    for_flagged(flag, 4 * half, [&](uint32_t f) { const int j = (int)(f / half); const uint32_t i = f - (uint32_t)j * half; parts[f] = fold_g2_gls_split_complete(gls_image(hi[i], j), dg, j); });
}

__global__ void __launch_bounds__(64, 2) k_pow2_mul_g2_q(const G2A* __restrict__ in, uint32_t n, int k, G2J* __restrict__ out) {
    const uint32_t i = blockIdx.x * blockDim.x + threadIdx.x;
    if (i >= n) return;
#if defined(__HIP_DEVICE_COMPILE__)
    const G2A* bp = in + i;
    bool inf; { const G2A b = *bp; inf = is_inf(b); }
    if (inf) { out[i] = jac_inf<Fp2>(); return; }
    JacQ2 d; j2_set(d, f2_from(opaque(bp)->x), f2_from(opaque(bp)->y), Fq2n{fq_one(), fq_zero()});
    f2_pin(d.z);
#pragma unroll 1
    for (int t = 0; t < k; ++t) jdbl2_q(d);
    out[i] = G2J{f2_to(d.x), f2_to(d.y), f2_to(d.z)};
#endif
}

}
```

### rust/ripp-hip/src/ffi.rs

```rust
#![allow(non_camel_case_types)]
use core::ffi::c_void;

#[repr(C)] #[derive(Copy, Clone, Default)] pub struct RippFp { pub l: [u64; 6] }
#[repr(C)] #[derive(Copy, Clone, Default)] pub struct RippFr { pub l: [u64; 4] }
#[repr(C)] #[derive(Copy, Clone, Default)] pub struct RippFp2 { pub c0: RippFp, pub c1: RippFp }
#[repr(C)] #[derive(Copy, Clone, Default)] pub struct RippGt { pub c: [RippFp2; 6] }
#[repr(C)] #[derive(Copy, Clone, Default)] pub struct RippG1A { pub x: RippFp, pub y: RippFp }
#[repr(C)] #[derive(Copy, Clone, Default)] pub struct RippG1J { pub x: RippFp, pub y: RippFp, pub z: RippFp }
#[repr(C)] #[derive(Copy, Clone, Default)] pub struct RippG2A { pub x: RippFp2, pub y: RippFp2 }
#[repr(C)] #[derive(Copy, Clone, Default)] pub struct RippG2J { pub x: RippFp2, pub y: RippFp2, pub z: RippFp2 }

#[repr(C)] pub struct RippVec { _private: [u8; 0] }
#[repr(C)] pub struct RippSippJob { _private: [u8; 0] }
#[repr(C)] pub struct RippSrs { _private: [u8; 0] }
#[repr(C)] pub struct RippPcSrs { _private: [u8; 0] }
#[repr(C)] pub struct RippTpcCk { _private: [u8; 0] }
pub type RippAllgatherFn = Option<unsafe extern "C" fn(user: *mut c_void, send: *const c_void, recv: *mut c_void, bytes: usize) -> i32>;
#[repr(C)] #[derive(Copy, Clone)]
pub struct RippAggregateProof {
    pub com_a: RippGt, pub com_b: RippGt, pub com_c: RippGt, pub ip_ab: RippGt,
    pub agg_c: RippG1J,
    pub r: RippFr,
    pub ab_com_steps: *mut RippGt,
    pub ab_transcript: *mut RippFr,
    pub ab_base_a: RippG1J, pub ab_base_b: RippG2J,
    pub ab_final_ck_a: RippG2J, pub ab_final_ck_b: RippG1J,
    pub ab_opening_a: RippG2J, pub ab_opening_b: RippG1J,
    pub ab_kzg_c: RippFr,
    pub c_com_gt: *mut RippGt,
    pub c_com_g1: *mut RippG1J,
    pub c_transcript: *mut RippFr,
    pub c_base_a: RippG1J, pub c_base_b: RippFr,
    pub c_final_ck_a: RippG2J, pub c_opening_a: RippG2J,
    pub c_kzg_c: RippFr,
}
#[repr(C)] #[derive(Copy, Clone)]
pub struct RippPcOpening {
    pub com_gt: *mut RippGt,
    pub com_g1: *mut RippG1J,
    pub transcript: *mut RippFr,
    pub base_a: RippG1J, pub base_b: RippFr,
    pub final_ck_a: RippG2J, pub opening_a: RippG2J,
    pub kzg_challenge: RippFr,
    pub y_eval_comm: RippG1J, pub kzg_proof: RippG1J,
}
#[repr(C)] #[derive(Copy, Clone)]
pub struct RippTpcOpening {
    pub s_com_gt: *mut RippGt,
    pub s_com_g1: *mut RippG1J,
    pub s_transcript: *mut RippFr,
    pub s_base_a: RippG1J, pub s_base_b: RippFr,
    pub y_eval_comm: RippG1J,
    pub f_com_g1: *mut RippG1J,
    pub f_com_fr: *mut RippFr,
    pub f_transcript: *mut RippFr,
    pub f_base_a: RippFr, pub f_base_b: RippFr,
}
#[repr(C)] #[derive(Copy, Clone, Default)]
pub struct RippVerifierSrs { pub g: RippG1J, pub h: RippG2J, pub g_beta: RippG1J, pub h_alpha: RippG2J }
#[repr(C)] #[derive(Copy, Clone)]
pub struct RippGroth16Vk { pub alpha_g1: RippG1A, pub beta_g2: RippG2A, pub gamma_g2: RippG2A, pub delta_g2: RippG2A, pub gamma_abc_g1: *const RippG1A, pub gamma_abc_len: usize }

pub const RIPP_OK: i32 = 0;
pub const RIPP_ERR_LENGTH: i32 = 1;
pub const RIPP_ERR_POW2: i32 = 2;
pub const RIPP_ERR_DEVICE: i32 = 3;
pub const RIPP_ERR_ARG: i32 = 4;
pub const RIPP_VEC_G1: i32 = 1;
pub const RIPP_VEC_G2: i32 = 2;
pub const RIPP_VEC_FR: i32 = 3;

#[repr(C)] #[derive(Copy, Clone, Default, Debug)]
pub struct RippStats {
    pub total_ms: f64, pub upload_ms: f64, pub scale_ms: f64, pub miller_lines_ms: f64, pub miller_products_ms: f64,
    pub fold_ms: f64, pub normalize_ms: f64, pub host_ms: f64, pub hash_ms: f64,
    pub kernel_miller_lines_ms_sum: f64, pub kernel_line_products_ms_sum: f64,
    pub kernel_miller_lines_launches: u64, pub kernel_line_products_launches: u64,
    pub pairs_lines: u64, pub pairs_products: u64,
    pub exchange_ms: f64, pub look_ms: f64, pub look_items: u64, pub look_pairs: u64,
    pub statement_hash_ms: f64, pub statement_hash_wait_ms: f64,
    pub chains_lines: u64,
    pub mem_tier: u64, pub device_bytes: u64,
}
#[repr(C)] #[derive(Copy, Clone, Default, Debug)]
pub struct RippConfig {
    pub struct_size: u32,
    pub no_vm: u32, pub no_precompute: u32, pub no_fold_tables: u32, pub no_msm_glv: u32, pub lp_one_lane: u32, pub no_endo: u32, pub no_fq: u32,
    pub no_xscale: u32, pub scale_no_fq: u32, pub agg_sequential: u32, pub look_static: u32, pub quiet_waits: u32, pub no_share: u32, pub no_fuse: u32, pub fuse_tables: u32,
    pub look_eighths: i32, pub ranks_per_device: i32, pub msm_c: i32, pub msm_ch: u32, pub msm_gmin: u32, pub no_prebuild: u32,
    pub vm_lines_max: u64, pub vm_fold_max: u64, pub vm_tree_max: u64, pub gls_split_max: u64, pub msm_vm_merge_max: u64, pub fold_tab_min: u64,
    pub fq_min: u64, pub lp_fq_min: u64, pub vm_joint_max: u64, pub vm_scale_max: u64, pub tail_pipe_max: u64, pub ml_fq_min: u64, pub fq_min_g1: u64, pub msm_lds_sort_min: u64, pub msm_chunk_min: u64,
    pub mem_cap_bytes: u64, pub hot_workers: u32, pub no_job_cache: u32,
    pub no_lp_karatsuba: u32, pub comm_timeout_ms: u32, pub plan_derate_pct: u32, pub n_devices: u32,
}
pub const RIPP_ABI_VERSION: i32 = 7;
#[cfg(feature = "ffi")]
pub fn abi_check() -> bool { unsafe { ripp_abi_version() == RIPP_ABI_VERSION && ripp_stats_size() == core::mem::size_of::<RippStats>() } }

#[cfg(feature = "ffi")]
extern "C" {
    pub fn ripp_abi_version() -> i32;
    pub fn ripp_stats_size() -> usize;
    pub fn ripp_init(device_ordinal: i32) -> i32;
    pub fn ripp_shutdown();
    pub fn ripp_device_count() -> i32;
    pub fn ripp_release_scratch() -> i32;
    pub fn ripp_device_bytes() -> usize;
    pub fn ripp_last_error() -> *const core::ffi::c_char;
    pub fn ripp_config_default(cfg: *mut RippConfig) -> i32;
    pub fn ripp_configure(cfg: *const RippConfig) -> i32;
    pub fn ripp_config_get(cfg: *mut RippConfig) -> i32;
    pub fn ripp_pairing_product_j(left: *const RippG1J, n_left: usize, right: *const RippG2J, n_right: usize, out: *mut RippGt) -> i32;
    pub fn ripp_pairing_product_a(a: *const RippG1A, b: *const RippG2A, n: usize, out: *mut RippGt) -> i32;
    pub fn ripp_pairing_product_coeffs_a(a: *const RippG1A, b: *const RippG2A, r: *const RippFr, n: usize, out: *mut RippGt) -> i32;
    pub fn ripp_msm_g1_j(bases: *const RippG1J, n_left: usize, scalars: *const RippFr, n_right: usize, out: *mut RippG1J) -> i32;
    pub fn ripp_msm_g2_j(bases: *const RippG2J, n_left: usize, scalars: *const RippFr, n_right: usize, out: *mut RippG2J) -> i32;
    pub fn ripp_msm_g1_a(bases: *const RippG1A, scalars: *const RippFr, n: usize, out: *mut RippG1J) -> i32;
    pub fn ripp_msm_g2_a(bases: *const RippG2A, scalars: *const RippFr, n: usize, out: *mut RippG2J) -> i32;
    pub fn ripp_device_slots_used() -> i32;
    pub fn ripp_scalar_inner_product(left: *const RippFr, nl: usize, right: *const RippFr, nr: usize, out: *mut RippFr) -> i32;
    pub fn ripp_pairing_miller_j(left: *const RippG1J, nl: usize, right: *const RippG2J, nr: usize, miller_value: *mut RippGt) -> i32;
    pub fn ripp_sum_g1_j(pts: *const RippG1J, n: usize, out: *mut RippG1J) -> i32;
    pub fn ripp_sum_g2_j(pts: *const RippG2J, n: usize, out: *mut RippG2J) -> i32;
    pub fn ripp_fold_g1_a(hi: *const RippG1A, lo: *const RippG1A, half: usize, s: *const RippFr, out: *mut RippG1A) -> i32;
    pub fn ripp_fold_g2_a(hi: *const RippG2A, lo: *const RippG2A, half: usize, s: *const RippFr, out: *mut RippG2A) -> i32;
    pub fn ripp_fold_g1_j(hi: *const RippG1J, lo: *const RippG1J, half: usize, s: *const RippFr, out: *mut RippG1J) -> i32;
    pub fn ripp_fold_g2_j(hi: *const RippG2J, lo: *const RippG2J, half: usize, s: *const RippFr, out: *mut RippG2J) -> i32;
    pub fn ripp_fold_fr(hi: *const RippFr, lo: *const RippFr, half: usize, s: *const RippFr, out: *mut RippFr) -> i32;
    pub fn ripp_scale_g1_a(a: *const RippG1A, r: *const RippFr, n: usize, out: *mut RippG1A) -> i32;
    pub fn ripp_normalize_g1(in_: *const RippG1J, n: usize, out: *mut RippG1A) -> i32;
    pub fn ripp_normalize_g2(in_: *const RippG2J, n: usize, out: *mut RippG2A) -> i32;
    pub fn ripp_vec_upload_g1a(p: *const RippG1A, n: usize, out: *mut *mut RippVec) -> i32;
    pub fn ripp_vec_upload_g2a(p: *const RippG2A, n: usize, out: *mut *mut RippVec) -> i32;
    pub fn ripp_vec_upload_g1j(p: *const RippG1J, n: usize, out: *mut *mut RippVec) -> i32;
    pub fn ripp_vec_upload_g2j(p: *const RippG2J, n: usize, out: *mut *mut RippVec) -> i32;
    pub fn ripp_vec_upload_fr(p: *const RippFr, n: usize, out: *mut *mut RippVec) -> i32;
    pub fn ripp_vec_len(v: *const RippVec) -> usize;
    pub fn ripp_vec_kind(v: *const RippVec) -> i32;
    pub fn ripp_vec_slice(v: *const RippVec, off: usize, len: usize, view: *mut *mut RippVec) -> i32;
    pub fn ripp_vec_halves(v: *const RippVec, lo: *mut *mut RippVec, hi: *mut *mut RippVec) -> i32;
    pub fn ripp_vec_download(v: *const RippVec, out: *mut c_void) -> i32;
    pub fn ripp_vec_free(v: *mut RippVec);
    pub fn ripp_vec_pairing_product(left_g1: *const RippVec, right_g2: *const RippVec, out: *mut RippGt) -> i32;
    pub fn ripp_vec_msm(bases: *const RippVec, scalars: *const RippVec, out: *mut c_void) -> i32;
    pub fn ripp_vec_scalar_inner_product(left: *const RippVec, right: *const RippVec, out: *mut RippFr) -> i32;
    pub fn ripp_vec_fold(hi: *const RippVec, lo: *const RippVec, s: *const RippFr, out: *mut *mut RippVec) -> i32;
    pub fn ripp_sipp_prove(a: *const RippG1A, b: *const RippG2A, r: *const RippFr, n: usize, value: *const RippGt, proof: *mut RippGt, challenges: *mut RippFr, stats: *mut RippStats) -> i32;
    pub fn ripp_sipp_verify(a: *const RippG1A, b: *const RippG2A, r: *const RippFr, n: usize, claimed: *const RippGt, proof: *const RippGt, proof_rounds: usize, accept: *mut i32) -> i32;
    pub fn ripp_sipp_job_create(a: *const RippG1A, b: *const RippG2A, r: *const RippFr, n_local: usize, rank: i32, world: i32, job: *mut *mut RippSippJob) -> i32;
    pub fn ripp_sipp_job_destroy(job: *mut RippSippJob);
    pub fn ripp_sipp_job_prove(job: *mut RippSippJob, value: *const RippGt, proof: *mut RippGt, challenges: *mut RippFr, stats: *mut RippStats) -> i32;
    pub fn ripp_sipp_job_begin(job: *mut RippSippJob) -> i32;
    pub fn ripp_sipp_job_rounds_left(job: *const RippSippJob) -> usize;
    pub fn ripp_sipp_job_round_partials(job: *mut RippSippJob, partials: *mut RippGt) -> i32;
    pub fn ripp_sipp_job_round_finish(job: *mut RippSippJob, combined: *const RippGt, seed_digest: *const u8, z_l: *mut RippGt, z_r: *mut RippGt, x: *mut RippFr) -> i32;
    pub fn ripp_sipp_job_stats(job: *const RippSippJob, stats: *mut RippStats) -> i32;
    pub fn ripp_sipp_job_local_len(job: *const RippSippJob) -> usize;
    pub fn ripp_sipp_job_export(job: *mut RippSippJob, a_out: *mut RippG1A, b_out: *mut RippG2A) -> i32;
    pub fn ripp_sipp_job_import(job: *mut RippSippJob, a: *const RippG1A, b: *const RippG2A, len: usize) -> i32;
    pub fn ripp_combine_partials(gathered: *const RippGt, world: i32, count: usize, out: *mut RippGt) -> i32;
    pub fn ripp_sipp_seed_digest(a: *const RippG1A, b: *const RippG2A, r: *const RippFr, n: usize, value: *const RippGt, digest: *mut u8) -> i32;
    pub fn ripp_statement_hash_times(hash_ms: *mut f64, wait_ms: *mut f64);
    pub fn ripp_comm_unique_id(id: *mut u8) -> i32;
    pub fn ripp_comm_init(id: *const u8, rank: i32, world: i32) -> i32;
    pub fn ripp_comm_init_callback(rank: i32, world: i32, allgather: RippAllgatherFn, user: *mut c_void) -> i32;
    pub fn ripp_comm_destroy();
    pub fn ripp_comm_rank() -> i32;
    pub fn ripp_comm_world() -> i32;
    pub fn ripp_comm_allgather(send: *const c_void, recv: *mut c_void, bytes: usize) -> i32;
    pub fn ripp_comm_record(on: i32) -> i32;
    pub fn ripp_comm_recording_save(path: *const core::ffi::c_char) -> i32;
    pub fn ripp_comm_init_replay(rank: i32, world: i32, path: *const core::ffi::c_char, latency_us: f64) -> i32;
    pub fn ripp_comm_replay_info(served: *mut u64, own_differs: *mut u64, waited_ms: *mut f64) -> i32;
    pub fn ripp_comm_replay_check(differing: *mut u64, mismatches: *mut u64) -> i32;
    pub fn ripp_pairing_product_sharded_j(left: *const RippG1J, nl: usize, right: *const RippG2J, nr: usize, out: *mut RippGt) -> i32;
    pub fn ripp_msm_g1_sharded_j(bases: *const RippG1J, nl: usize, scalars: *const RippFr, nr: usize, out: *mut RippG1J) -> i32;
    pub fn ripp_msm_g2_sharded_j(bases: *const RippG2J, nl: usize, scalars: *const RippFr, nr: usize, out: *mut RippG2J) -> i32;
    pub fn ripp_sipp_prove_sharded(a: *const RippG1A, b: *const RippG2A, r: *const RippFr, n_local: usize, value: *const RippGt, full_a: *const RippG1A, full_b: *const RippG2A, full_r: *const RippFr, seed_digest: *const u8, proof: *mut RippGt, challenges: *mut RippFr, stats: *mut RippStats) -> i32;
    pub fn ripp_sipp_job_prove_sharded(job: *mut RippSippJob, value: *const RippGt, full_a: *const RippG1A, full_b: *const RippG2A, full_r: *const RippFr, seed_digest: *const u8, proof: *mut RippGt, challenges: *mut RippFr, stats: *mut RippStats) -> i32;
    pub fn ripp_test_inject_failure(rank: i32, round: i32);
    pub fn ripp_gipa_tipp_prove(m_a: *const RippG1J, m_b: *const RippG2J, ck_a: *const RippG2J, ck_b: *const RippG1J, n: usize, com_steps: *mut RippGt, transcript: *mut RippFr, base_a: *mut RippG1J, base_b: *mut RippG2J, ck_base_a: *mut RippG2J, ck_base_b: *mut RippG1J, stats: *mut RippStats) -> i32;
    pub fn ripp_srs_create(g_alpha_powers: *const RippG1J, h_beta_powers: *const RippG2J, num: usize, srs: *mut *mut RippSrs) -> i32;
    pub fn ripp_srs_destroy(srs: *mut RippSrs);
    pub fn ripp_srs_powers_g1(s: *const RippFr, num: usize, out: *mut RippG1J) -> i32;
    pub fn ripp_srs_powers_g2(s: *const RippFr, num: usize, out: *mut RippG2J) -> i32;
    pub fn ripp_srs_commitment_keys(srs: *const RippSrs, ck_1: *mut RippG2J, ck_2: *mut RippG1J) -> i32;
    pub fn ripp_tipa_tipp_prove(srs: *const RippSrs, m_a: *const RippG1J, m_b: *const RippG2J, ck_a: *const RippG2J, ck_b: *const RippG1J, n: usize, r_shift: *const RippFr, com_steps: *mut RippGt, transcript: *mut RippFr, base_a: *mut RippG1J, base_b: *mut RippG2J, final_ck_a: *mut RippG2J, final_ck_b: *mut RippG1J, opening_a: *mut RippG2J, opening_b: *mut RippG1J, kzg_challenge: *mut RippFr, stats: *mut RippStats) -> i32;
    pub fn ripp_tipa_ssm_prove(srs: *const RippSrs, m_a: *const RippG1J, m_b: *const RippFr, ck_a: *const RippG2J, n: usize, com_gt: *mut RippGt, com_g1: *mut RippG1J, transcript: *mut RippFr, base_a: *mut RippG1J, base_b: *mut RippFr, final_ck_a: *mut RippG2J, opening_a: *mut RippG2J, kzg_challenge: *mut RippFr, stats: *mut RippStats) -> i32;
    pub fn ripp_aggregate_proofs(srs: *const RippSrs, a: *const RippG1A, b: *const RippG2A, c: *const RippG1A, n: usize, out: *mut RippAggregateProof, stats: *mut RippStats) -> i32;
    pub fn ripp_aggregate_proofs_sharded(srs: *const RippSrs, a: *const RippG1A, b: *const RippG2A, c: *const RippG1A, n_local: usize, out: *mut RippAggregateProof, stats: *mut RippStats) -> i32;
// ... 63 lines not shown
```

Measured before the change: 2.644 million.

## Add precomputed doubling-ladder fold path for mid-sized SIPP rounds

```diff
diff --git a/include/ripp_hip.h b/include/ripp_hip.h
--- a/include/ripp_hip.h
+++ b/include/ripp_hip.h
@@ -38,6 +38,7 @@
 int32_t ripp_device_count(void);
 int32_t ripp_release_scratch(void);
 size_t  ripp_device_bytes(void);
+int32_t ripp_fold_ladder_terms(const ripp_fr* s, int32_t group, uint32_t* terms, size_t cap, int32_t* n_terms);
 const char* ripp_last_error(void);
 
 typedef struct {
diff --git a/ripp_amd/csrc/engine.hip b/ripp_amd/csrc/engine.hip
--- a/ripp_amd/csrc/engine.hip
+++ b/ripp_amd/csrc/engine.hip
@@ -235,6 +235,11 @@
     struct JobBufCache { DevBuf d[15]; PinBuf p[4]; bool full = false; void release() { for (DevBuf& b : d) b.release(); for (PinBuf& b : p) b.release(); full = false; } } job_cache;
     size_t msm_chunk_min = (size_t)1 << 20;
     size_t msm_lds_sort_min = 0;
+    DevBuf lad_jac1, lad_aff1, lad_jac2, lad_aff2, lad_parts1, lad_parts2, lad_flags;
+    hipEvent_t ev_lad = nullptr, ev_lad1 = nullptr, ev_lad2 = nullptr;
+    static constexpr size_t FOLD_LADDER_MIN = ((size_t)1 << 12) + 1, FOLD_LADDER_MAX = (size_t)1 << 15;
+    size_t fold_ladder_min = FOLD_LADDER_MIN, fold_ladder_max = FOLD_LADDER_MAX;
+    int fold_ladder_L = 8;
     const void* g2tab_hi = nullptr; size_t g2tab_half = 0;
     size_t vm_scale_max = (size_t)1 << 14;
     size_t vm_joint_max = (size_t)1 << 13;
@@ -285,7 +290,7 @@
         aux->refresh_switches(); aux->stats = ripp_stats{};
         return aux;
     }
-    struct Switches { bool no_vm = false, no_precompute = false, no_fold_tables = false, no_msm_glv = false, lp_one_lane = false, no_endo = false, no_fq = false, no_xscale = false, no_share = false, no_fuse = false, no_prebuild = false, fuse_tables = false, no_job_cache = false, no_lp_kara = false, no_msm_batch = false; } sw;
+    struct Switches { bool no_vm = false, no_precompute = false, no_fold_tables = false, no_msm_glv = false, lp_one_lane = false, no_endo = false, no_fq = false, no_xscale = false, no_share = false, no_fuse = false, no_prebuild = false, fuse_tables = false, no_job_cache = false, no_lp_kara = false, no_msm_batch = false, no_fold_ladder = false; } sw;
     struct Sizes { size_t vm_lines_max, vm_fold_max, vm_tree_max, gls_split_max, msm_vm_merge_max, fold_tab_min, fq_min, lp_fq_min, vm_joint_max, vm_scale_max, tail_pipe_max, ml_fq_min, fq_min_g1, msm_lds_sort_min, msm_chunk_min; } defaults{};
     MsmTune msm_tune;
     static constexpr size_t TPC_CROSS_MIN = ~(size_t)0;
@@ -299,6 +304,7 @@
         vm_lines_max = defaults.vm_lines_max; vm_fold_max = defaults.vm_fold_max; vm_tree_max = defaults.vm_tree_max; gls_split_max = defaults.gls_split_max;
         msm_vm_merge_max = defaults.msm_vm_merge_max; fold_tab_min = defaults.fold_tab_min; fq_min = defaults.fq_min; lp_fq_min = defaults.lp_fq_min; vm_joint_max = defaults.vm_joint_max;
         vm_scale_max = defaults.vm_scale_max; tail_pipe_max = defaults.tail_pipe_max; ml_fq_min = defaults.ml_fq_min; fq_min_g1 = defaults.fq_min_g1; msm_lds_sort_min = defaults.msm_lds_sort_min; msm_chunk_min = defaults.msm_chunk_min;
+        fold_ladder_min = FOLD_LADDER_MIN; fold_ladder_max = FOLD_LADDER_MAX; fold_ladder_L = 8;
         sw = Switches(); look_eighths = -1; ranks_per_device = 1.0; look_static = quiet_waits_cfg = agg_sequential = scale_no_fq = false; mem_cap = 0; hot_workers_cfg = 0; comm_timeout_ms = plan_derate_pct = n_devices_cfg = 0;
         if (g_cfg_set) {
             const ripp_config& c = g_cfg;
@@ -334,6 +340,9 @@
           virtual_devices = false; if (const char* s = std::getenv("RIPP_VIRTUAL_DEVICES")) { n_devices_cfg = (uint32_t)std::strtoul(s, nullptr, 10); virtual_devices = true; } }
         tpc_cross_min = TPC_CROSS_MIN; env_sz("RIPP_TPC_CROSS_MIN", tpc_cross_min);
         env_on("RIPP_NO_MSM_BATCH", sw.no_msm_batch);
+        env_on("RIPP_NO_FOLD_LADDER", sw.no_fold_ladder);
+        env_sz("RIPP_FOLD_LADDER_MIN", fold_ladder_min); env_sz("RIPP_FOLD_LADDER_MAX", fold_ladder_max);
+        if (const char* s = std::getenv("RIPP_FOLD_LADDER_L")) fold_ladder_L = std::min(16, std::max(1, std::atoi(s)));
         env_on("RIPP_NO_PREBUILD", sw.no_prebuild);
         env_on("RIPP_NO_FUSE", sw.no_fuse);
         env_on("RIPP_NO_SHARE", sw.no_share);
@@ -358,6 +367,7 @@
         HIPCHK(hipStreamCreateWithFlags(&stream5, hipStreamNonBlocking)); HIPCHK(hipEventCreateWithFlags(&ev_join5, hipEventDisableTiming));
         HIPCHK(hipEventCreateWithFlags(&ev_fork, hipEventDisableTiming)); HIPCHK(hipEventCreateWithFlags(&ev_join, hipEventDisableTiming)); HIPCHK(hipEventCreateWithFlags(&ev_join3, hipEventDisableTiming));
         HIPCHK(hipEventCreate(&ev_t0)); HIPCHK(hipEventCreate(&ev_t1));
+        HIPCHK(hipEventCreateWithFlags(&ev_lad, hipEventDisableTiming)); HIPCHK(hipEventCreateWithFlags(&ev_lad1, hipEventDisableTiming)); HIPCHK(hipEventCreateWithFlags(&ev_lad2, hipEventDisableTiming));
         { hipDeviceProp_t pr; if (hipGetDeviceProperties(&pr, dev) == hipSuccess) n_simd = pr.multiProcessorCount * 4; }
         defaults = Sizes{vm_lines_max, vm_fold_max, vm_tree_max, gls_split_max, msm_vm_merge_max, fold_tab_min, fq_min, lp_fq_min, vm_joint_max, vm_scale_max, tail_pipe_max, ml_fq_min, fq_min_g1, msm_lds_sort_min, msm_chunk_min};
         refresh_switches();
@@ -368,7 +378,7 @@
         if (aux) { aux->destroy(); delete aux; aux = nullptr; }
         for (Engine* p : peers) { (void)hipSetDevice(p->device); p->destroy(); delete p; }
         if (!peers.empty()) { peers.clear(); (void)hipSetDevice(device); }
-        for (DevBuf* b : {&lines, &partA, &partB, &jacG1, &jacG2, &tmpA, &tmpB, &tmpR, &affG1, &affG2, &qtab, &vm_flag, &scale_tab, &fold_tab1, &fold_mult, &fold_tab, &fold_jac1, &fold_jac2, &fix_flags, &scale_flags}) b->release();
+        for (DevBuf* b : {&lines, &partA, &partB, &jacG1, &jacG2, &tmpA, &tmpB, &tmpR, &affG1, &affG2, &qtab, &vm_flag, &scale_tab, &fold_tab1, &fold_mult, &fold_tab, &fold_jac1, &fold_jac2, &fix_flags, &scale_flags, &lad_jac1, &lad_aff1, &lad_jac2, &lad_aff2, &lad_parts1, &lad_parts2, &lad_flags}) b->release();
         msm_scratch[0].release(); msm_scratch[1].release(); kzg_q[0].release(); kzg_q[1].release(); kzg_bases[0].release(); kzg_bases[1].release(); job_cache.release(); pc_release();
         if (stream3) (void)hipStreamDestroy(stream3);
         if (stream4) (void)hipStreamDestroy(stream4); if (ev_join4) (void)hipEventDestroy(ev_join4);
@@ -382,6 +392,7 @@
         if (stream2) (void)hipStreamDestroy(stream2);
         if (ev_fork) (void)hipEventDestroy(ev_fork); if (ev_join) (void)hipEventDestroy(ev_join); if (ev_join3) (void)hipEventDestroy(ev_join3);
         if (ev_t0) (void)hipEventDestroy(ev_t0); if (ev_t1) (void)hipEventDestroy(ev_t1);
+        if (ev_lad) (void)hipEventDestroy(ev_lad); if (ev_lad1) (void)hipEventDestroy(ev_lad1); if (ev_lad2) (void)hipEventDestroy(ev_lad2);
         if (ev_quiet) (void)hipEventDestroy(ev_quiet);
     }
     int32_t ensure_pinned_rows(size_t rows) {
@@ -743,6 +754,7 @@
     for (DevBuf* b : {&e->lines, &e->partA, &e->partB, &e->qtab, &e->scale_tab, &e->jacG1, &e->jacG2, &e->affG1, &e->affG2, &e->tmpA, &e->tmpB, &e->tmpR}) if (b->p && b->epoch != now) b->release();
     for (DevBuf* b : {&e->fold_tab1, &e->fold_mult, &e->fold_tab, &e->fold_jac1, &e->fold_jac2}) if (b->p && b->epoch != now) { b->release(); tables = true; }
     if (tables) { e->tab_owner = nullptr; e->g2tab_hi = nullptr; }
+    for (DevBuf* b : {&e->lad_jac1, &e->lad_aff1, &e->lad_jac2, &e->lad_aff2, &e->lad_parts1, &e->lad_parts2, &e->lad_flags}) if (b->p && b->epoch != now) b->release();
     for (int k = 0; k < 2; ++k) {
         MsmScratch& ms = e->msm_scratch[k];
         for (DevBuf* b : {&ms.digits, &ms.hist, &ms.offs, &ms.cursor, &ms.slotoffs, &ms.spw, &ms.sorted, &ms.slots, &ms.buckets, &ms.seg, &ms.seg2, &ms.win, &ms.ext, &ms.flags}) if (b->p && b->epoch != now) b->release();
@@ -855,6 +867,28 @@
     const int l1 = naf_recode(&c.l[0], 2, g.d1, 131), l2 = naf_recode(&c.l[2], 2, g.d2, 131);
     g.len = l1 > l2 ? l1 : l2;
     return g;
+}
+LadderTerms ladder_terms_g1(const Fr& s_mont) {
+    LadderTerms tm; std::memset(&tm, 0, sizeof tm);
+    const Fr c = from_mont(s_mont);
+    if ((c.l[4] | c.l[5] | c.l[6] | c.l[7]) != 0) { tm.n = -1; return tm; }
+    const NafDigits nd = naf_digits(s_mont);
+    for (int k = 0; k < nd.len; ++k) {
+        if (nd.d[k] == 0) continue;
+        if (k >= LADDER_ROWS_G1 || tm.n >= LADDER_MAX_TERMS) { tm.n = -1; return tm; }
+        tm.t[tm.n++] = (uint16_t)(k | (nd.d[k] < 0 ? 1 << 10 : 0));
+    }
+    return tm;
+}
+LadderTerms ladder_terms_g2(const Fr& s_mont) {
+    LadderTerms tm; std::memset(&tm, 0, sizeof tm);
+    const GlsDigits g = gls_digits(s_mont);
+    for (int j = 0; j < 4; ++j) for (int k = 0; k < g.len; ++k) {
+        if (g.d[j][k] == 0) continue;
+        if (k >= LADDER_ROWS_G2 || tm.n >= LADDER_MAX_TERMS) { tm.n = -1; return tm; }
+        tm.t[tm.n++] = (uint16_t)(k | (j << 8) | (g.d[j][k] < 0 ? 1 << 10 : 0));
+    }
+    return tm;
 }
 bool fits_128(const Fr& s_mont) { const Fr c = from_mont(s_mont); return (c.l[4] | c.l[5] | c.l[6] | c.l[7]) == 0; }
 Gls8Digits gls8_digits(const Fr& s_mont) {
@@ -1003,6 +1037,7 @@
     std::atomic<uint64_t> hash_done{0}; uint64_t hash_total = 0; double hash_t0 = 0;
     bool no_window = false;
     size_t hash_n = 0;
+    bool lad_ready = false, lad_on_lo = false; size_t lad_half = 0;
     DevBuf a_pow_h, b_pow_h, parts1, parts2; bool pre_vm_ready = false, pre_vm_side = false;
     PinBuf tp_rows[2]; size_t tp_round[2] = {~(size_t)0, ~(size_t)0};
     std::vector<G1A> ha; std::vector<G2A> hb; std::vector<Fr> hr;
@@ -1036,7 +1071,7 @@
     float ms = 0; (void)hipEventElapsedTime(&ms, t0, t1); e->stats.scale_ms += ms;
     j->len = n; j->seeded = false; j->world = j->world0;
     j->bs = Fr::one(); j->bs_on = false;
-    j->pre_vm_ready = false; j->pre_vm_side = false; j->pre_ready = false; j->look.clear(); j->tp_round[0] = j->tp_round[1] = ~(size_t)0;
+    j->pre_vm_ready = false; j->pre_vm_side = false; j->pre_ready = false; j->lad_ready = false; j->look.clear(); j->tp_round[0] = j->tp_round[1] = ~(size_t)0;
     return RIPP_OK;
 }
 
@@ -1063,7 +1098,7 @@
 }
 int32_t job_precompute_vm(Engine* e, ripp_sipp_job* j, bool side = false) {
     const size_t half = j->len / 2;
-    if (half == 0 || half > e->vm_fold_max || e->sw.no_vm || e->sw.no_precompute) return RIPP_OK;
+    if (half == 0 || half > e->vm_fold_max || e->sw.no_vm || e->sw.no_precompute || j->lad_ready) return RIPP_OK;
     int32_t rc;
     if ((rc = j->a_pow_h.reserve(half * sizeof(G1J))) || (rc = j->b_pow_h.reserve(half * sizeof(G2J))) || (rc = j->parts1.reserve(2 * half * sizeof(G1J))) || (rc = j->parts2.reserve(8 * half * sizeof(G2J)))) return rc;
     hipLaunchKernelGGL(HIP_KERNEL_NAME(k_vm_pow2<Fp>), dim3(nblk(half, 4 * VM_EPW)), dim3(256), 4 * VM_EPW * VmCurve<Fp>::SLOTS * sizeof(VmSlot), e->stream2, j->a.as<G1A>() + half, (uint32_t)half, 64, j->a_pow_h.as<G1J>());
@@ -1203,12 +1238,81 @@
     return RIPP_OK;
 }
 
+bool fold_ladder_pays(const Engine* e, size_t half) {
+#if defined(RIPP_BLS12_377)
+    (void)e; (void)half; return false;
+#else
+    return !e->sw.no_fold_ladder && !e->sw.no_fq && !e->sw.no_endo && !e->sw.no_precompute && half >= 1 && half >= e->fold_ladder_min && half <= e->fold_ladder_max;
+#endif
+}
+size_t fold_ladder_bytes(const Engine* e, size_t half, bool g1, bool g2) {
+    const size_t L = (size_t)e->fold_ladder_L;
+    return (g1 ? half * ((size_t)LADDER_ROWS_G1 * (sizeof(G1J) + sizeof(G1A)) + L * sizeof(G1J)) : 0) +
+           (g2 ? half * ((size_t)LADDER_ROWS_G2 * (sizeof(G2J) + sizeof(G2A)) + L * sizeof(G2J) + L) + 64 : 0);
+}
+bool fold_ladder_fits(const Engine* e, size_t half, bool g1, bool g2) {
+    const size_t held = (g1 ? e->lad_jac1.cap + e->lad_aff1.cap + e->lad_parts1.cap : 0) + (g2 ? e->lad_jac2.cap + e->lad_aff2.cap + e->lad_parts2.cap + e->lad_flags.cap : 0);
+    return e->mem_fits(fold_ladder_bytes(e, half, g1, g2), held);
+}
+int32_t fold_ladder_reserve(Engine* e, size_t half, bool g1, bool g2) {
+    const size_t L = (size_t)e->fold_ladder_L;
+    int32_t rc;
+    if (g1 && ((rc = e->lad_jac1.reserve((size_t)LADDER_ROWS_G1 * half * sizeof(G1J))) || (rc = e->lad_aff1.reserve((size_t)LADDER_ROWS_G1 * half * sizeof(G1A))) || (rc = e->lad_parts1.reserve(L * half * sizeof(G1J))))) return rc;
+    if (g2 && ((rc = e->lad_jac2.reserve((size_t)LADDER_ROWS_G2 * half * sizeof(G2J))) || (rc = e->lad_aff2.reserve((size_t)LADDER_ROWS_G2 * half * sizeof(G2A))) || (rc = e->lad_parts2.reserve(L * half * sizeof(G2J))) ||
+               (rc = e->lad_flags.reserve(L * half + 64)))) return rc;
+    return RIPP_OK;
+}
+int32_t fold_ladder_build_g1(Engine* e, hipStream_t st, const G1A* hi, size_t half) {
+    hipLaunchKernelGGL(k_ladder_g1_q, dim3(nblk(half, 64)), dim3(64), 0, st, hi, (uint32_t)half, LADDER_ROWS_G1, e->lad_jac1.as<G1J>());
+    HIPCHK(hipGetLastError());
+    return e->normalize_dev<Fp>(e->lad_jac1.as<G1J>(), (size_t)LADDER_ROWS_G1 * half, e->lad_aff1.as<G1A>(), st);
+}
+int32_t fold_ladder_build_g2(Engine* e, hipStream_t st, const G2A* hi, size_t half) {
+    hipLaunchKernelGGL(k_ladder_g2_q, dim3(nblk(half, 64)), dim3(64), 0, st, hi, (uint32_t)half, LADDER_ROWS_G2, e->lad_jac2.as<G2J>());
+    HIPCHK(hipGetLastError());
+    return e->normalize_dev<Fp2>(e->lad_jac2.as<G2J>(), (size_t)LADDER_ROWS_G2 * half, e->lad_aff2.as<G2A>(), st);
+}
+int32_t fold_ladder_g1(Engine* e, hipStream_t st, const G1A* lo, size_t half, const LadderTerms& tm, G1J* out) {
+    const int L = e->fold_ladder_L;
+    hipLaunchKernelGGL(k_fold_g1_ladder_q, dim3(nblk(half, 64), L), dim3(64), 0, st, e->lad_aff1.as<G1A>(), (uint32_t)half, tm, L, e->lad_parts1.as<G1J>());
+    hipLaunchKernelGGL(HIP_KERNEL_NAME(k_fold_combine_n<Fp>), dim3(nblk(half, 64)), dim3(64), 0, st, e->lad_parts1.as<G1J>(), L, lo, (uint32_t)half, out);
+    HIPCHK(hipGetLastError());
+    return RIPP_OK;
+}
+int32_t fold_ladder_g2(Engine* e, hipStream_t st, const G2A* lo, size_t half, const LadderTerms& tm, G2J* out) {
+    const int L = e->fold_ladder_L;
+    hipLaunchKernelGGL(k_fold_g2_ladder_q, dim3(nblk(half, 64), L), dim3(64), 0, st, e->lad_aff2.as<G2A>(), (uint32_t)half, tm, L, e->lad_parts2.as<G2J>(), e->lad_flags.as<uint8_t>());
+    hipLaunchKernelGGL(k_fold_g2_ladder_fix, dim3(FIX_GRID), dim3(64), 0, st, e->lad_aff2.as<G2A>(), (uint32_t)half, tm, L, e->lad_parts2.as<G2J>(), e->lad_flags.as<uint8_t>());
+    hipLaunchKernelGGL(HIP_KERNEL_NAME(k_fold_combine_n<Fp2>), dim3(nblk(half, 64)), dim3(64), 0, st, e->lad_parts2.as<G2J>(), L, lo, (uint32_t)half, out);
+    HIPCHK(hipGetLastError());
+    return RIPP_OK;
+}
+int32_t job_ladder_enqueue(Engine* e, ripp_sipp_job* j) {
+    const size_t half = j->len / 2;
+    j->lad_ready = false;
+    if (half == 0 || !fold_ladder_pays(e, half)) return RIPP_OK;
+    if (j->pre_ready || j->pre_vm_ready || (j->tab_ready && e->tab_owner == j) || (e->g2tab_hi && e->g2tab_half == half)) return RIPP_OK;
+    const bool xs = xscale_round(e, j, half);
+    if (j->bs_on && !xs) return RIPP_OK;
+    if (!fold_ladder_fits(e, half, true, true)) { e->mem_tier |= 32; return RIPP_OK; }
+    int32_t rc;
+    if ((rc = fold_ladder_reserve(e, half, true, true))) return rc;
+    HIPCHK(hipEventRecord(e->ev_lad, e->stream));
+    HIPCHK(hipStreamWaitEvent(e->stream2, e->ev_lad, 0)); HIPCHK(hipStreamWaitEvent(e->stream3, e->ev_lad, 0));
+    if ((rc = fold_ladder_build_g1(e, e->stream2, j->a.as<G1A>() + half, half))) return rc;
+    HIPCHK(hipEventRecord(e->ev_lad1, e->stream2));
+    if ((rc = fold_ladder_build_g2(e, e->stream3, xs ? j->b.as<G2A>() : j->b.as<G2A>() + half, half))) return rc;
+    HIPCHK(hipEventRecord(e->ev_lad2, e->stream3));
+    j->lad_ready = true; j->lad_half = half; j->lad_on_lo = xs;
+    return RIPP_OK;
+}
+
 int32_t job_prebuild_g2_tables(Engine* e, ripp_sipp_job* j) {
     const size_t half = j->len / 2;
     e->g2tab_hi = nullptr;
     if (e->sw.no_prebuild || e->sw.no_endo || half < 1) return RIPP_OK;
     const bool vm_form = (half <= e->vm_fold_max || half <= e->vm_joint_max) && !e->sw.no_vm;
-    if (vm_form || j->pre_ready || j->pre_vm_ready || (j->tab_ready && e->tab_owner == j) || !fold_g2_table_pays(e, half)) return RIPP_OK;
+    if (vm_form || j->pre_ready || j->pre_vm_ready || j->lad_ready || (j->tab_ready && e->tab_owner == j) || !fold_g2_table_pays(e, half)) return RIPP_OK;
     const bool xs = xscale_round(e, j, half);
     if (j->bs_on && !xs) return RIPP_OK;
     if (!fold_g2_table_fits(e, half)) return RIPP_OK;
@@ -1236,8 +1340,16 @@
     HIPCHK(hipStreamWaitEvent(e->stream2, e->ev_fork, 0));
     const bool tab = j->tab_ready && e->tab_owner == j && fits_128(x); j->tab_ready = false;
     const int tabW = tab_width(j->tab_M);
+    const bool xs_now = xscale_round(e, j, half) && fits_128(x) && (!tab || j->tab_on_lo);
+    LadderTerms lt1, lt2; lt1.n = lt2.n = -1;
+    if (j->lad_ready && j->lad_half == half && !tab && !pre && j->lad_on_lo == xs_now && !(j->bs_on && !xs_now)) { lt1 = ladder_terms_g1(x); lt2 = ladder_terms_g2(xs_now ? x : x_inv); }
+    const bool lad = lt1.n >= 0 && lt2.n >= 0; j->lad_ready = false;
     const G1A* tab1 = e->fold_tab1.as<G1A>() + (j->tab_fused ? half / 2 : 0);
-    if (tab && !e->sw.no_fq && half >= e->fq_min)
+    if (lad) {
+        HIPCHK(hipStreamWaitEvent(g1s, e->ev_lad1, 0));
+        if ((rc = fold_ladder_g1(e, g1s, a, half, lt1, j->jac1.as<G1J>()))) return rc;
+    }
+    else if (tab && !e->sw.no_fq && half >= e->fq_min)
         hipLaunchKernelGGL(k_fold_g1_tab_q, dim3(nblk(half, 256)), dim3(256), 0, g1s, tab1, j->tab_cnt, j->tab_M, a, (uint32_t)half, split32_wnaf(x, tabW), j->jac1.as<G1J>());
     else if (tab)
         hipLaunchKernelGGL(k_fold_g1_tab, dim3(nblk(half, 256)), dim3(256), 0, g1s, tab1, j->tab_cnt, j->tab_M, a, (uint32_t)half, split32_wnaf(x, tabW), j->jac1.as<G1J>());
@@ -1283,6 +1395,10 @@
         hipLaunchKernelGGL(k_fold_g2_combine8, dim3(nblk(half, 64)), dim3(64), 0, e->stream, e->qtab.as<G2J>(), (uint32_t)half, j->jac2.as<G2J>());
         }
         j->bs = Fr::one(); j->bs_on = false;
+    } else
+    if (lad) {
+        HIPCHK(hipStreamWaitEvent(e->stream, e->ev_lad2, 0));
+        if ((rc = fold_ladder_g2(e, e->stream, g2_lo, half, lt2, j->jac2.as<G2J>()))) return rc;
     } else
     if (pre_vm) {
         if (j->pre_vm_side) { HIPCHK(hipStreamWaitEvent(e->stream, e->ev_join3, 0)); j->pre_vm_side = false; }
@@ -1429,7 +1545,8 @@
     LOCK; if (!g_engine) return RIPP_OK;
     Engine* e = g_engine;
     if (hipSetDevice(e->device) != hipSuccess || hipDeviceSynchronize() != hipSuccess) { set_err("ripp_release_scratch: device synchronisation failed"); return RIPP_ERR_DEVICE; }
-    for (DevBuf* b : {&e->lines, &e->partA, &e->partB, &e->jacG1, &e->jacG2, &e->tmpA, &e->tmpB, &e->tmpR, &e->affG1, &e->affG2, &e->qtab, &e->scale_tab, &e->fold_tab1, &e->fold_mult, &e->fold_tab, &e->fold_jac1, &e->fold_jac2, &e->fix_flags, &e->scale_flags}) b->release();
+    for (DevBuf* b : {&e->lines, &e->partA, &e->partB, &e->jacG1, &e->jacG2, &e->tmpA, &e->tmpB, &e->tmpR, &e->affG1, &e->affG2, &e->qtab, &e->scale_tab, &e->fold_tab1, &e->fold_mult, &e->fold_tab, &e->fold_jac1, &e->fold_jac2, &e->fix_flags, &e->scale_flags,
+                     &e->lad_jac1, &e->lad_aff1, &e->lad_jac2, &e->lad_aff2, &e->lad_parts1, &e->lad_parts2, &e->lad_flags}) b->release();
     e->msm_scratch[0].release(); e->msm_scratch[1].release(); e->kzg_q[0].release(); e->kzg_q[1].release(); e->kzg_bases[0].release(); e->kzg_bases[1].release(); e->pc_release();
     for (PinBuf& pb : e->stage) pb.release();
     e->tab_owner = nullptr; e->g2tab_hi = nullptr; e->job_cache.release(); vec_caches_release();
@@ -1440,6 +1557,15 @@
 }
 
 API size_t ripp_device_bytes(void) { return g_dev_bytes.load(std::memory_order_relaxed); }
+API int32_t ripp_fold_ladder_terms(const ripp_fr* s, int32_t group, uint32_t* terms, size_t cap, int32_t* n_terms) {
+    if (!s || !n_terms || (group != 1 && group != 2) || (cap && !terms)) return RIPP_ERR_ARG;
+    Fr sm; std::memcpy(&sm, s, sizeof(Fr));
+    const LadderTerms tm = group == 1 ? ladder_terms_g1(sm) : ladder_terms_g2(sm);
+    *n_terms = tm.n;
+    if (tm.n > 0 && (size_t)tm.n > cap) return RIPP_ERR_LENGTH;
+    for (int t = 0; t < tm.n; ++t) terms[t] = tm.t[t];
+    return RIPP_OK;
+}
 
 API int32_t ripp_normalize_g1(const ripp_g1j* in, size_t n, ripp_g1a* out) {
     LOCK; ENGINE; if (n == 0) return RIPP_OK; if (!in || !out) return RIPP_ERR_ARG;
@@ -1489,6 +1615,15 @@
         Affine<F>*dh, *dl;
         if ((rc = upload<Affine<F>>(e, e->tmpA, hi, half, &dh))) return rc;
         if ((rc = upload<Affine<F>>(e, e->tmpB, lo, half, &dl))) return rc;
+        constexpr bool G1 = std::is_same<F, Fp>::value;
+        LadderTerms lt; lt.n = -1;
+        if (fold_ladder_pays(e, half) && fits_128(sm)) lt = G1 ? ladder_terms_g1(sm) : ladder_terms_g2(sm);
+        if (lt.n >= 0 && !fold_ladder_fits(e, half, G1, !G1)) { e->mem_tier |= 32; lt.n = -1; }
+        if (lt.n >= 0) {
+            if ((rc = fold_ladder_reserve(e, half, G1, !G1))) return rc;
+            if constexpr (G1) { if ((rc = fold_ladder_build_g1(e, e->stream, dh, half)) || (rc = fold_ladder_g1(e, e->stream, dl, half, lt, jac.as<G1J>()))) return rc; }
+            else { if ((rc = fold_ladder_build_g2(e, e->stream, dh, half)) || (rc = fold_ladder_g2(e, e->stream, dl, half, lt, jac.as<G2J>()))) return rc; }
+        } else
         if (std::is_same<F, Fp2>::value && !e->sw.no_endo) {
             const size_t qstride = (half + 63) & ~(size_t)63;
             if ((rc = e->qtab.reserve(4 * G2A_CHUNKS * qstride * sizeof(uint4)))) return rc;
@@ -2214,7 +2349,7 @@
     e->mem_tier = 0;
     struct Quiesce { Engine* e; ripp_sipp_job* j; ~Quiesce() {
         (void)hipStreamSynchronize(e->stream); (void)hipStreamSynchronize(e->stream2); (void)hipStreamSynchronize(e->stream3);
-        j->tp_round[0] = j->tp_round[1] = ~(size_t)0; j->pre_vm_ready = false; j->pre_vm_side = false; j->pre_ready = false; j->tab_ready = false; j->look.clear();
+        j->tp_round[0] = j->tp_round[1] = ~(size_t)0; j->pre_vm_ready = false; j->pre_vm_side = false; j->pre_ready = false; j->tab_ready = false; j->lad_ready = false; j->look.clear();
         e->g2tab_hi = nullptr;
         if (j->hash_thread.joinable()) j->hash_thread.join();
         j->ha_ext = nullptr; j->hb_ext = nullptr; j->hr_ext = nullptr; j->hash_prestarted = false; } } quiesce{e, j};
@@ -2285,7 +2420,7 @@
             HIPCHK(hipMemcpyAsync(j->b.p, hb, L * sizeof(G2A), hipMemcpyHostToDevice, e->stream));
             if ((rc = e->sync())) return rc;
             j->len = len = L; j->world = 1; sharded = false;
-            j->pre_vm_ready = false;
+            j->pre_vm_ready = false; j->lad_ready = false;
             continue;
         }
         Fp12 rows[2 * N_LINES];
@@ -2319,6 +2454,7 @@
                 if ((rc = e->step_products(as, bs, 1, half - start[sd], rows + sd * N_LINES))) return rc;
                 e->stats.miller_products_ms += now_ms() - tp;
             }
+            if (!j->lad_ready && !fuse_pending && !(!sharded && j->len == 2) && (rc = job_ladder_enqueue(e, j))) return rc;
             if (round >= 1 && !fuse_pending && !tp_round && (rc = job_prebuild_g2_tables(e, j))) return rc;
             const bool plan_fuse = look_forced ? look_items >= 16 : look_items >= 12;
             if (round == 0 && !j->seeded && (rc = job_precompute_round0(e, j, (plan_fuse || e->sw.fuse_tables) && j->len >= 4))) return rc;
@@ -2391,6 +2527,7 @@
             else if (!lrc && round == 0 && known && j->tab_ready && j->tab_fused && e->tab_owner == j && !j->bs_on) { fuse_pending = true; x0_saved = x; }
             else
             if (!lrc) lrc = job_fold(e, j, x, true, pipelined || known);
+            if (!lrc && !fuse_pending && !(!sharded && j->len == 2)) lrc = job_ladder_enqueue(e, j);
             if (!lrc && pipelined) {
                 if (!j->pre_vm_ready) lrc = job_precompute_vm(e, j, true);
                 if (!lrc && tail_pipe_ok(e, j)) lrc = job_tail_enqueue(e, j, round + 2);
diff --git a/ripp_amd/csrc/fq_curve.hpp b/ripp_amd/csrc/fq_curve.hpp
--- a/ripp_amd/csrc/fq_curve.hpp
+++ b/ripp_amd/csrc/fq_curve.hpp
@@ -280,4 +280,68 @@
 #endif
 }
 
-}
+constexpr int LADDER_ROWS_G1 = 129;
+constexpr int LADDER_ROWS_G2 = 65;
+constexpr int LADDER_MAX_TERMS = 136;
+struct LadderTerms { uint16_t t[LADDER_MAX_TERMS]; int n; };
+__global__ void __launch_bounds__(64, 2) k_ladder_g1_q(const G1A* __restrict__ in, uint32_t n, int rows, G1J* __restrict__ out ) {
+    const uint32_t i = blockIdx.x * blockDim.x + threadIdx.x;
+    if (i >= n) return;
+#if defined(__HIP_DEVICE_COMPILE__)
+    const G1A p = in[i];
+    if (is_inf(p)) {
+#pragma unroll 1
+        for (int k = 0; k < rows; ++k) out[(size_t)k * n + i] = jac_inf<Fp>();
+        return;
+    }
+    out[i] = to_jac(p);
+    const AffQ q = affq_from(p);
+    JacQ acc; jq_set(acc, q.x, q.y, fq_one());
+#pragma unroll 1
+    for (int k = 1; k < rows; ++k) { jdbl_q(acc); out[(size_t)k * n + i] = jacq_to_g1j(acc); }
+#endif
+}
+__global__ void __launch_bounds__(64, 2) k_fold_g1_ladder_q(const G1A* __restrict__ rows, uint32_t half, LadderTerms tm, int L, G1J* __restrict__ parts ) {
+    const uint32_t i = blockIdx.x * blockDim.x + threadIdx.x;
+    if (i >= half) return;
+    const int g = blockIdx.y;
+#if defined(__HIP_DEVICE_COMPILE__)
+    constexpr uint32_t betaw[12] = RIPP_GLV_BETA; constexpr fq28::Limbs BETA = fq28::from_mont384(betaw);
+    JacQ acc; jq_set_identity(acc);
+    bool inf = true, bad = false;
+#pragma unroll 1
+    for (int t = g; t < tm.n; t += L) {
+        const uint32_t w = tm.t[t];
+        const G1A qa = rows[(size_t)(w & 255u) * half + i];
+        bad |= is_inf(qa);
+        AffQ p = affq_from(qa);
+        if ((w >> 8) & 3u) p.x = fq_mul(p.x, fq_const<FQ_LN, 1>(BETA));
+        if (w >> 10) p.y = fq_reduce(fq_neg(p.y));
+        if (inf) { jq_set(acc, p.x, p.y, fq_one()); inf = false; }
+        else bad |= jmadd_q(acc, p.x, p.y);
+    }
+    G1J r = jac_inf<Fp>();
+    if (bad) {
+#pragma unroll 1
+        for (int t = g; t < tm.n; t += L) {
+            const uint32_t w = tm.t[t];
+            G1A q = rows[(size_t)(w & 255u) * half + i];
+            if ((w >> 8) & 3u) q.x = fmul(q.x, fp_const(RIPP_GLV_BETA));
+            if (w >> 10) q.y = neg(q.y);
+            r = add_mixed(r, q);
+        }
+    } else if (!inf) r = jacq_to_g1j(acc);
+    parts[(size_t)g * half + i] = r;
+#endif
+}
+template <class F>
+__global__ void __launch_bounds__(64) k_fold_combine_n(const Jac<F>* __restrict__ parts, int L, const Affine<F>* __restrict__ lo, uint32_t half, Jac<F>* __restrict__ out) {
+    const uint32_t i = blockIdx.x * blockDim.x + threadIdx.x;
+    if (i >= half) return;
+    Jac<F> acc = parts[i];
+#pragma unroll 1
+    for (int t = 1; t < L; ++t) acc = add(acc, parts[(size_t)t * half + i]);
+    out[i] = add_mixed(acc, lo[i]);
+}
+
+}
diff --git a/ripp_amd/csrc/fq_curve2.hpp b/ripp_amd/csrc/fq_curve2.hpp
--- a/ripp_amd/csrc/fq_curve2.hpp
+++ b/ripp_amd/csrc/fq_curve2.hpp
@@ -426,4 +426,81 @@
 #endif
 }
 
-}
+__global__ void __launch_bounds__(64, 2) k_ladder_g2_q(const G2A* __restrict__ in, uint32_t n, int rows, G2J* __restrict__ out ) {
+    const uint32_t i = blockIdx.x * blockDim.x + threadIdx.x;
+    if (i >= n) return;
+#if defined(__HIP_DEVICE_COMPILE__)
+    const G2A* bp = in + i;
+    bool inf; { const G2A b = *bp; inf = is_inf(b); }
+    if (inf) {
+#pragma unroll 1
+        for (int k = 0; k < rows; ++k) out[(size_t)k * n + i] = jac_inf<Fp2>();
+        return;
+    }
+    out[i] = to_jac(*opaque(bp));
+    JacQ2 d; j2_set(d, f2_from(opaque(bp)->x), f2_from(opaque(bp)->y), Fq2n{fq_one(), fq_zero()});
+    f2_pin(d.z);
+#pragma unroll 1
+    for (int k = 1; k < rows; ++k) { jdbl2_q(d); out[(size_t)k * n + i] = G2J{f2_to(d.x), f2_to(d.y), f2_to(d.z)}; }
+#endif
+}
+__device__ __noinline__ inline G2J fold_g2_ladder_complete(const G2A* __restrict__ rows, uint32_t half, uint32_t i, const LadderTerms& tm, int L, int g) {
+    G2J acc = jac_inf<Fp2>();
+#pragma unroll 1
+    for (int t = g; t < tm.n; t += L) {
+        const uint32_t w = tm.t[t];
+        G2A q = gls_image(rows[(size_t)(w & 255u) * half + i], (int)((w >> 8) & 3u));
+        if (w >> 10) q.y = neg(q.y);
+        acc = add_mixed(acc, q);
+    }
+    return acc;
+}
+__global__ void __launch_bounds__(64, 2) k_fold_g2_ladder_q(const G2A* __restrict__ rows, uint32_t half, LadderTerms tm, int L, G2J* __restrict__ parts , uint8_t* __restrict__ flag ) {
+    __shared__ uint4 park_[21 * 64];
+    const uint32_t i = blockIdx.x * blockDim.x + threadIdx.x;
+    if (i >= half) return;
+    const int g = blockIdx.y;
+#if defined(__HIP_DEVICE_COMPILE__)
+    uint4* park = park_ + threadIdx.x;
+    uint4* qpark = park + 7 * 64;
+    auto st7 = [](uint4* dst, const Fq2n& v) { uint32_t w[28];
+#pragma unroll
+        for (int k = 0; k < 14; ++k) { w[k] = v.c0.l[k]; w[14 + k] = v.c1.l[k]; }
+        const uint4* src = reinterpret_cast<const uint4*>(w);
+#pragma unroll
+        for (int k = 0; k < 7; ++k) dst[k * 64] = src[k]; };
+    auto ld7 = [](const uint4* src) { uint4 q[7];
+#pragma unroll
+        for (int k = 0; k < 7; ++k) q[k] = src[k * 64];
+        const uint32_t* w = reinterpret_cast<const uint32_t*>(q);
+        Fq2n v;
+#pragma unroll
+        for (int k = 0; k < 14; ++k) { v.c0.l[k] = w[k]; v.c1.l[k] = w[14 + k]; }
+        return v; };
+    JacQ2 acc; j2_set_identity(acc);
+    bool inf = true, bad = false;
+#pragma unroll 1
+    for (int t = g; t < tm.n; t += L) {
+        const uint32_t w = tm.t[t];
+        {
+            G2A q = gls_image(rows[(size_t)(w & 255u) * half + i], (int)((w >> 8) & 3u));
+            bad |= is_inf(q);
+            if (w >> 10) q.y = neg(q.y);
+            st7(qpark, f2_from(q.x)); st7(qpark + 7 * 64, f2_from(q.y));
+        }
+        auto loadx = [&]() { return ld7(qpark); };
+        auto loady = [&]() { return ld7(qpark + 7 * 64); };
+        if (inf) { j2_set(acc, loadx(), loady(), Fq2n{fq_one(), fq_zero()}); f2_pin(acc.z); inf = false; }
+        else bad |= jmadd2_q(acc, loadx, loady, park);
+    }
+    flag[(size_t)g * half + i] = bad;
+    if (bad) return;
+    if (inf) parts[(size_t)g * half + i] = jac_inf<Fp2>();
+    else parts[(size_t)g * half + i] = G2J{f2_to(acc.x), f2_to(acc.y), f2_to(acc.z)};
+#endif
+}
+__global__ void __launch_bounds__(64) k_fold_g2_ladder_fix(const G2A* __restrict__ rows, uint32_t half, LadderTerms tm, int L, G2J* __restrict__ parts, const uint8_t* __restrict__ flag) {
+    for_flagged(flag, (uint32_t)L * half, [&](uint32_t f) { const int g = (int)(f / half); const uint32_t i = f - (uint32_t)g * half; parts[f] = fold_g2_ladder_complete(rows, half, i, tm, L, g); });
+}
+
+}
diff --git a/rust/ripp-hip/src/ffi.rs b/rust/ripp-hip/src/ffi.rs
--- a/rust/ripp-hip/src/ffi.rs
+++ b/rust/ripp-hip/src/ffi.rs
@@ -106,6 +106,7 @@
     pub fn ripp_device_count() -> i32;
     pub fn ripp_release_scratch() -> i32;
     pub fn ripp_device_bytes() -> usize;
+    pub fn ripp_fold_ladder_terms(s: *const RippFr, group: i32, terms: *mut u32, cap: usize, n_terms: *mut i32) -> i32;
     pub fn ripp_last_error() -> *const core::ffi::c_char;
     pub fn ripp_config_default(cfg: *mut RippConfig) -> i32;
     pub fn ripp_configure(cfg: *const RippConfig) -> i32;
```

After: 2.602 million. 0.984x the previous value.
